# Senpai-sama06/real-time-audio-visual-zooming

Hardware: AMD Instinct MI355X
Metric: beamformed TF-bins/sec (2-ch, 1024-pt STFT) + SIR dB delta vs reference (higher is better)
Workload: dtype f32; 1 GPU; configs[1]: B=256 utterances/GPU, 2 interferers, oracle IBM, 1024-pt STFT hop 512 @16 kHz, 4.0 s utterances; batch_per_gpu=256, global_batch=256, samples=64000, n_fft=1024, hop=512, parallelism=utterance-sharded x1, RCCL metric all-reduce only, input_batches=2, tf_bins_per_utt=64638, mask=ibm, postfilter=ibm, normalize=peak

## Files before the change

include/avz.h:

```cpp
#ifndef AVZ_H_
#define AVZ_H_

#ifdef __cplusplus
extern "C" {
#endif

#define AVZ_OK 0
#define AVZ_ERR_ARG (-1)
#define AVZ_ERR_SHAPE (-2)
#define AVZ_ERR_HIP (-3)
#define AVZ_ERR_UNSUPPORTED (-4)
#define AVZ_ERR_ALIGN (-5)

#define AVZ_MASK_IBM 0
#define AVZ_MASK_IPD 1
#define AVZ_MASK_EXTERNAL 2
#define AVZ_MASK_ONES 3

#define AVZ_PF_NONE 0
#define AVZ_PF_IBM_TARGET 1
#define AVZ_PF_EXT_FLOOR 2
#define AVZ_PF_EXT_MUL 3
#define AVZ_PF_IRM 4

#define AVZ_FALLBACK_MIC0 0
#define AVZ_FALLBACK_MEAN 1
#define AVZ_FALLBACK_BATCH 2

#define AVZ_BF_MVDR 0
#define AVZ_BF_HYBRID_NULL 1

#define AVZ_NORM_NONE 0
#define AVZ_NORM_PEAK 1

typedef struct avz_config {
  int fs;
  int n_fft;
  int hop;
  double sigma;
  double angle_deg;
  double mic_d;
  double c_sound;
  double fmin_hz;
  int mask_mode;
  int postfilter;
  double pf_floor;
  double weight_eps;
  int normalize;
  double norm_eps;
  int max_batch;
  int max_samples;
  int beamformer;
  double bypass_hz;
  double cond_max;
  int singular_fallback;
  double ibm_kappa;
} avz_config;
#define AVZ_IBM_KAPPA 16.0

typedef struct avz_plan avz_plan;

typedef struct avz_batch_args {
  int batch;
  const int* len;
  int max_len;
  const float* mix;
  long long mix_stride;
  long long ch_stride;
  const float* ref_tgt;
  const float* ref_int;
  long long ref_stride;
  const float* ext_mask;
  long long mask_stride_b, mask_stride_f, mask_stride_t;
  float* out;
  long long out_stride;
  float* peak;
  double* cov_out;
  float* w_out;
  int mask_bins;
  int mask_frames;
  void* workspace;
  long long workspace_bytes;
} avz_batch_args;

int avz_plan_create(avz_plan** plan, const avz_config* cfg);
int avz_plan_destroy(avz_plan* plan);
int avz_plan_get_config(const avz_plan* plan, avz_config* cfg);
int avz_num_frames(const avz_plan* plan, int len);
int avz_mvdr_batch(const avz_plan* plan, const avz_batch_args* args, void* hip_stream);
long long avz_mvdr_workspace_bytes(const avz_plan* plan, int batch, int max_len);

int avz_mvdr_covariance(const avz_plan* plan, const avz_batch_args* args, void* hip_stream);
int avz_solve_covariance(const avz_plan* plan, int batch, const double* cov, float* w,
                         const double* steer, int* fallback, void* hip_stream);
int avz_apply_istft(const avz_plan* plan, const avz_batch_args* args, const float* w,
                    void* hip_stream);

typedef struct avz_spectral_args {
  int batch;
  int frames;
  const float* Y;
  long long y_stride_b, y_stride_m, y_stride_f;
  const float* mask;
  long long mask_stride_b, mask_stride_f;
  const double* steer;
  float* S;
  long long s_stride_b, s_stride_f;
  double* cov_out;
  float* w_out;
  int* fallback;
} avz_spectral_args;
int avz_beamform_spectral(const avz_plan* plan, const avz_spectral_args* args, void* hip_stream);

typedef struct avz_wpe_args {
  int batch, bins, frames;
  const int* frames_b;
  int taps, delay, iterations;
  const float* Y;
  long long y_stride_b, y_stride_m, y_stride_f;
  float* Z;
  long long z_stride_b, z_stride_m, z_stride_f;
  int* status;
} avz_wpe_args;
int avz_wpe_spectral(const avz_wpe_args* args, void* hip_stream);

int avz_istft(const avz_plan* plan, int batch, int frames, const float* S, long long s_stride_b,
              long long s_stride_f, float* out, long long out_stride, float* peak,
              void* workspace, long long workspace_bytes, void* hip_stream);

int avz_plan_set_timing(avz_plan* plan, int enable);
int avz_plan_set_timing_period(avz_plan* plan, int period);
int avz_plan_get_timing(avz_plan* plan, double* ms_avg , int* calls);
int avz_plan_set_ibm_stats(avz_plan* plan, unsigned long long* counts);
int avz_plan_set_diagnostics(avz_plan* plan, int synth_variant, int ipf_mode);
int avz_ibm_window(int n, float* out);

int avz_stft(const avz_plan* plan, int batch, int channels, const int* len, int max_len,
             const float* x, long long x_stride, long long ch_stride, float* Y,
             long long y_stride_b, long long y_stride_c, long long y_stride_f,
             void* hip_stream);

int avz_chunk_split(int n_items, int channels, int chunk, const int* item_utt,
                    const int* item_start, const int* len, const float* x, long long x_stride,
                    long long x_ch_stride, float* items, long long item_stride,
                    long long item_ch_stride, void* hip_stream);

int avz_chunk_merge(int batch, int max_len, int hop, int item_out_len, const int* len,
                    const int* item_base, const float* item_out, long long item_out_stride,
                    float* y, long long y_stride, float* peak, int normalize, double norm_eps,
                    void* hip_stream);

#define AVZ_FEAT_LOGMAG_IPD 1
#define AVZ_FEAT_TFLITE 2
int avz_mask_features(const avz_plan* plan, int layout, int batch, const int* len, int max_len,
                      const float* x, long long x_stride, long long ch_stride, float* feat,
                      long long s_b, long long s_c, long long s_f, long long s_t,
                      void* hip_stream);

int avz_mask_training_batch(const avz_plan* plan, int layout, int batch, const int* len,
                            int max_len, const float* mix, long long mix_stride,
                            long long ch_stride, const float* tgt, const float* itf,
                            long long ref_stride, float* feat, long long s_b, long long s_c,
                            long long s_f, long long s_t, float* label, long long l_b,
                            long long l_f, long long l_t, void* hip_stream);

int avz_srp_scan(const avz_plan* plan, int batch, const int* len, int max_len,
                 const float* mix, long long mix_stride, long long ch_stride, int n_angles,
                 double angle_lo, double angle_hi, double f_lo, double f_hi, double* power_db,
                 void* hip_stream);

int avz_projection_metrics(int batch, int max_len, const int* len, const float* est,
                           long long est_stride, const float* tgt, long long tgt_stride,
                           const float* itf, long long itf_stride, double* sums,
                           double* metrics, void* hip_stream);
int avz_projection_metrics_scaled(int batch, int max_len, const int* len, const float* est,
                                  long long est_stride, const float* est_peak, double est_eps,
                                  const float* tgt, long long tgt_stride, const float* itf,
                                  long long itf_stride, double* sums, double* metrics,
                                  void* hip_stream);

typedef struct avz_stoi_args {
  int batch, max_len;
  const int* len;
  double fs;
  const float* clean; long long clean_stride;
  const float* est;   long long est_stride;
  double* stoi;
  int* info;
  float* resampled;
  long long res_stride;
  double* tob;
  long long tob_stride;
  void* workspace; long long workspace_bytes;
} avz_stoi_args;
long long avz_stoi_workspace_bytes(int batch, int max_len, double fs);
int avz_stoi_batch(const avz_stoi_args* args, void* hip_stream);

long long avz_scene_workspace_bytes(int batch, int n_src, int n);
int avz_scene_mix(int batch, int n_src, int n, const float* src, const double* angles_deg,
                  const float* noise, double mic_d, double c_sound, double fs, double sir_db,
                  double snr_db, float* mix, long long mix_stride, long long ch_stride,
                  float* tgt, float* itf, long long ref_stride, void* workspace,
                  long long workspace_bytes, void* hip_stream);

long long avz_scene_generate_workspace_bytes(int batch, int n_interferers, int n);
int avz_scene_generate(int batch, long long start_idx, int n_interferers, int n, unsigned seed,
                       double mic_d, double c_sound, double fs, double sir_db, double snr_db,
                       float* mix, long long mix_stride, long long ch_stride, float* tgt,
                       float* itf, long long ref_stride, void* workspace,
                       long long workspace_bytes, void* hip_stream);

typedef struct avz_room {
  double dim[3];
  double absorption;
  int max_order;
  double mic[2][3];
  double c_sound, fs;
} avz_room;

int avz_room_rir_len(const avz_room* room);

int avz_room_rir(const avz_room* room, int batch, int n_src, const double* src_pos,
                 double* rir, void* hip_stream);

long long avz_scene_reverb_workspace_bytes(const avz_room* room, int batch, int n_src, int n);
int avz_scene_reverb_mix(const avz_room* room, int batch, int n_src, int n, const float* src,
                         const double* src_pos, const float* noise, double sir_db,
                         double snr_db, float* mix, long long mix_stride, long long ch_stride,
                         float* tgt, float* itf, long long ref_stride, void* workspace,
                         long long workspace_bytes, void* hip_stream);

long long avz_scene_reverb_generate_workspace_bytes(const avz_room* room, int batch,
                                                    int n_interferers, int n);
int avz_scene_reverb_generate(const avz_room* room, int batch, long long start_idx,
                              int n_interferers, int n, unsigned seed, const double* target_pos,
                              const double* interferer_pos, double sir_db, double snr_db,
                              float* mix, long long mix_stride, long long ch_stride, float* tgt,
                              float* itf, long long ref_stride, void* workspace,
                              long long workspace_bytes, void* hip_stream);

long long avz_stream_state_bytes(const avz_plan* plan, int streams);
int avz_stream_reset(const avz_plan* plan, void* state, long long state_bytes, int streams,
                     const int* select , void* hip_stream);
int avz_stream_steer(const avz_plan* plan, void* state, long long state_bytes, int streams,
                     const double* angle_deg ,
                     void* hip_stream);
typedef struct avz_stream_args {
  int streams, hops;
  double forget;
  const int* active;
  const int* adapt;
  const float* mix;  long long mix_stride, ch_stride;
  const float* ref_tgt; const float* ref_int; long long ref_stride;
  const float* ext_mask; long long mask_stride_b, mask_stride_f, mask_stride_t;
  float* out; long long out_stride;
  float* w_out;  double* cov_out;
  float* mask_out;
  void* state; long long state_bytes;
} avz_stream_args;
int avz_stream_push(const avz_plan* plan, const avz_stream_args* args, void* hip_stream);

long long avz_wpe_stream_state_bytes(const avz_plan* plan, int streams, int taps, int delay);
int avz_wpe_stream_reset(const avz_plan* plan, void* state, long long state_bytes, int streams,
                         int taps, int delay, double q_init,
                         const int* select ,
                         void* hip_stream);
typedef struct avz_wpe_stream_args {
  int streams, hops, taps, delay;
  double forget, power_floor;
  const int* active;
  const int* adapt;
  const float* mix; long long mix_stride, ch_stride;
  float* out;       long long out_stride, out_ch_stride;
  float* Y_out; float* Z_out;
  double* G_out;
  void* state; long long state_bytes;
} avz_wpe_stream_args;
int avz_wpe_stream_push(const avz_plan* plan, const avz_wpe_stream_args* args, void* hip_stream);

typedef struct avz_delay_mask_args {
  int batch; const int* len; int max_len;
  const float* mix; long long mix_stride, ch_stride;
  const double* angle_deg;
  int hist_bins, smooth, max_peaks;
  double rel_height, min_sep, f_lo_hz;
  float* mask; long long mask_stride_b, mask_stride_f, mask_stride_t;
// ... 39 lines not shown
```

real-time-audio-visual-zooming_amd/avz/_lib.py:

```python
from __future__ import annotations

import ctypes as ct
import os

import torch

_HERE = os.path.dirname(os.path.abspath(__file__))
LIB_PATH = os.environ.get("AVZ_LIB", os.path.join(_HERE, "libavz.so"))

AVZ_OK = 0
AVZ_ERR_ARG = -1
AVZ_ERR_SHAPE = -2
AVZ_ERR_HIP = -3
AVZ_ERR_UNSUPPORTED = -4
AVZ_ERR_ALIGN = -5

MASK_IBM, MASK_IPD, MASK_EXTERNAL, MASK_ONES = 0, 1, 2, 3
PF_NONE, PF_IBM_TARGET, PF_EXT_FLOOR, PF_EXT_MUL, PF_IRM = 0, 1, 2, 3, 4
FALLBACK_MIC0, FALLBACK_MEAN, FALLBACK_BATCH = 0, 1, 2
NORM_NONE, NORM_PEAK = 0, 1
BF_MVDR, BF_HYBRID_NULL = 0, 1
FEAT_LOGMAG_IPD, FEAT_TFLITE = 1, 2

EXPORTED = [
    "avz_plan_create", "avz_plan_destroy", "avz_plan_get_config", "avz_num_frames",
    "avz_mvdr_batch", "avz_plan_set_timing", "avz_plan_get_timing", "avz_stft",
    "avz_plan_set_timing_period",
    "avz_chunk_split", "avz_chunk_merge", "avz_mask_features", "avz_srp_scan",
    "avz_projection_metrics", "avz_scene_workspace_bytes", "avz_scene_mix", "avz_strerror",
    "avz_last_hip_error", "avz_version", "avz_mvdr_workspace_bytes",
    "avz_mvdr_covariance", "avz_solve_covariance", "avz_apply_istft", "avz_beamform_spectral",
    "avz_istft", "avz_scene_generate_workspace_bytes", "avz_scene_generate",
    "avz_projection_metrics_scaled", "avz_plan_set_ibm_stats", "avz_plan_set_diagnostics",
    "avz_ibm_window", "avz_wpe_spectral",
    "avz_room_rir_len", "avz_room_rir", "avz_scene_reverb_workspace_bytes",
    "avz_scene_reverb_mix", "avz_scene_reverb_generate_workspace_bytes",
    "avz_scene_reverb_generate",
    "avz_stoi_workspace_bytes", "avz_stoi_batch",
    "avz_mask_training_batch",
    "avz_stream_state_bytes", "avz_stream_reset", "avz_stream_steer", "avz_stream_push",
    "avz_wpe_stream_state_bytes", "avz_wpe_stream_reset", "avz_wpe_stream_push",
    "avz_delay_mask_workspace_bytes", "avz_delay_mask", "avz_delay_mask_check",
    "avz_delay_stream_state_bytes", "avz_delay_stream_reset", "avz_delay_stream_push",
    "avz_delay_stream_check",
]


class AvzConfig(ct.Structure):
    _fields_ = [
        ("fs", ct.c_int), ("n_fft", ct.c_int), ("hop", ct.c_int),
        ("sigma", ct.c_double), ("angle_deg", ct.c_double), ("mic_d", ct.c_double),
        ("c_sound", ct.c_double), ("fmin_hz", ct.c_double),
        ("mask_mode", ct.c_int), ("postfilter", ct.c_int),
        ("pf_floor", ct.c_double), ("weight_eps", ct.c_double),
        ("normalize", ct.c_int), ("norm_eps", ct.c_double),
        ("max_batch", ct.c_int), ("max_samples", ct.c_int),
        ("beamformer", ct.c_int), ("bypass_hz", ct.c_double), ("cond_max", ct.c_double),
        ("singular_fallback", ct.c_int), ("ibm_kappa", ct.c_double),
    ]


class AvzBatchArgs(ct.Structure):
    _fields_ = [
        ("batch", ct.c_int), ("len", ct.c_void_p), ("max_len", ct.c_int),
        ("mix", ct.c_void_p), ("mix_stride", ct.c_longlong), ("ch_stride", ct.c_longlong),
        ("ref_tgt", ct.c_void_p), ("ref_int", ct.c_void_p), ("ref_stride", ct.c_longlong),
        ("ext_mask", ct.c_void_p), ("mask_stride_b", ct.c_longlong),
        ("mask_stride_f", ct.c_longlong), ("mask_stride_t", ct.c_longlong),
        ("out", ct.c_void_p), ("out_stride", ct.c_longlong), ("peak", ct.c_void_p),
        ("cov_out", ct.c_void_p), ("w_out", ct.c_void_p),
        ("mask_bins", ct.c_int), ("mask_frames", ct.c_int),
        ("workspace", ct.c_void_p), ("workspace_bytes", ct.c_longlong),
    ]


class AvzSpectralArgs(ct.Structure):
    _fields_ = [
        ("batch", ct.c_int), ("frames", ct.c_int),
        ("Y", ct.c_void_p), ("y_stride_b", ct.c_longlong), ("y_stride_m", ct.c_longlong),
        ("y_stride_f", ct.c_longlong),
        ("mask", ct.c_void_p), ("mask_stride_b", ct.c_longlong), ("mask_stride_f", ct.c_longlong),
        ("steer", ct.c_void_p),
        ("S", ct.c_void_p), ("s_stride_b", ct.c_longlong), ("s_stride_f", ct.c_longlong),
        ("cov_out", ct.c_void_p), ("w_out", ct.c_void_p), ("fallback", ct.c_void_p),
    ]


class AvzWpeArgs(ct.Structure):
    _fields_ = [
        ("batch", ct.c_int), ("bins", ct.c_int), ("frames", ct.c_int),
        ("frames_b", ct.c_void_p),
        ("taps", ct.c_int), ("delay", ct.c_int), ("iterations", ct.c_int),
        ("Y", ct.c_void_p), ("y_stride_b", ct.c_longlong), ("y_stride_m", ct.c_longlong),
        ("y_stride_f", ct.c_longlong),
        ("Z", ct.c_void_p), ("z_stride_b", ct.c_longlong), ("z_stride_m", ct.c_longlong),
        ("z_stride_f", ct.c_longlong),
        ("status", ct.c_void_p),
    ]


class AvzStoiArgs(ct.Structure):
    _fields_ = [
        ("batch", ct.c_int), ("max_len", ct.c_int), ("len", ct.c_void_p), ("fs", ct.c_double),
        ("clean", ct.c_void_p), ("clean_stride", ct.c_longlong),
        ("est", ct.c_void_p), ("est_stride", ct.c_longlong),
        ("stoi", ct.c_void_p), ("info", ct.c_void_p),
        ("resampled", ct.c_void_p), ("res_stride", ct.c_longlong),
        ("tob", ct.c_void_p), ("tob_stride", ct.c_longlong),
        ("workspace", ct.c_void_p), ("workspace_bytes", ct.c_longlong),
    ]


class AvzStreamArgs(ct.Structure):
    _fields_ = [
        ("streams", ct.c_int), ("hops", ct.c_int), ("forget", ct.c_double),
        ("active", ct.c_void_p), ("adapt", ct.c_void_p),
        ("mix", ct.c_void_p), ("mix_stride", ct.c_longlong), ("ch_stride", ct.c_longlong),
        ("ref_tgt", ct.c_void_p), ("ref_int", ct.c_void_p), ("ref_stride", ct.c_longlong),
        ("ext_mask", ct.c_void_p), ("mask_stride_b", ct.c_longlong),
        ("mask_stride_f", ct.c_longlong), ("mask_stride_t", ct.c_longlong),
        ("out", ct.c_void_p), ("out_stride", ct.c_longlong),
        ("w_out", ct.c_void_p), ("cov_out", ct.c_void_p), ("mask_out", ct.c_void_p),
        ("state", ct.c_void_p), ("state_bytes", ct.c_longlong),
    ]


class AvzWpeStreamArgs(ct.Structure):
    _fields_ = [
        ("streams", ct.c_int), ("hops", ct.c_int), ("taps", ct.c_int), ("delay", ct.c_int),
        ("forget", ct.c_double), ("power_floor", ct.c_double),
        ("active", ct.c_void_p), ("adapt", ct.c_void_p),
        ("mix", ct.c_void_p), ("mix_stride", ct.c_longlong), ("ch_stride", ct.c_longlong),
        ("out", ct.c_void_p), ("out_stride", ct.c_longlong), ("out_ch_stride", ct.c_longlong),
        ("Y_out", ct.c_void_p), ("Z_out", ct.c_void_p), ("G_out", ct.c_void_p),
        ("state", ct.c_void_p), ("state_bytes", ct.c_longlong),
    ]


class AvzDelayMaskArgs(ct.Structure):
    _fields_ = [
        ("batch", ct.c_int), ("len", ct.c_void_p), ("max_len", ct.c_int),
        ("mix", ct.c_void_p), ("mix_stride", ct.c_longlong), ("ch_stride", ct.c_longlong),
        ("angle_deg", ct.c_void_p),
        ("hist_bins", ct.c_int), ("smooth", ct.c_int), ("max_peaks", ct.c_int),
        ("rel_height", ct.c_double), ("min_sep", ct.c_double), ("f_lo_hz", ct.c_double),
        ("mask", ct.c_void_p), ("mask_stride_b", ct.c_longlong),
        ("mask_stride_f", ct.c_longlong), ("mask_stride_t", ct.c_longlong),
        ("hist_out", ct.c_void_p), ("delays_out", ct.c_void_p), ("n_peaks", ct.c_void_p),
        ("workspace", ct.c_void_p), ("workspace_bytes", ct.c_longlong),
    ]


class AvzDelayStreamArgs(ct.Structure):
    _fields_ = [
        ("streams", ct.c_int), ("hops", ct.c_int), ("forget", ct.c_double),
        ("active", ct.c_void_p), ("adapt", ct.c_void_p),
        ("mix", ct.c_void_p), ("mix_stride", ct.c_longlong), ("ch_stride", ct.c_longlong),
        ("angle_deg", ct.c_void_p),
        ("hist_bins", ct.c_int), ("smooth", ct.c_int), ("max_peaks", ct.c_int),
        ("rel_height", ct.c_double), ("min_sep", ct.c_double), ("f_lo_hz", ct.c_double),
        ("mask", ct.c_void_p), ("mask_stride_b", ct.c_longlong),
        ("mask_stride_f", ct.c_longlong), ("mask_stride_t", ct.c_longlong),
        ("hist_out", ct.c_void_p), ("delays_out", ct.c_void_p), ("n_peaks", ct.c_void_p),
        ("state", ct.c_void_p), ("state_bytes", ct.c_longlong),
    ]


class AvzRoom(ct.Structure):
    _fields_ = [
        ("dim", ct.c_double * 3), ("absorption", ct.c_double), ("max_order", ct.c_int),
        ("mic", (ct.c_double * 3) * 2), ("c_sound", ct.c_double), ("fs", ct.c_double),
    ]


class AvzError(RuntimeError):
    pass


ABI_VERSION = 3


def hip_runtimes_mapped() -> list:
    paths = set()
    try:
        with open("/proc/self/maps") as fh:
            for line in fh:
                if "libamdhip64" in line:
                    paths.add(os.path.realpath(line.split()[-1]))
    except OSError:
        pass
    return sorted(paths)


def _load():
    if not os.path.exists(LIB_PATH):
        raise ImportError(f"libavz.so not found at {LIB_PATH}; run __graft_entry__.build() "
                          "(hipcc --offload-arch=gfx950). There is no CPU fallback.")
    lib = ct.CDLL(LIB_PATH)
    rts = hip_runtimes_mapped()
    if len(rts) > 1:
        raise ImportError(f"two HIP runtimes mapped into the process: {rts}")
    P = ct.c_void_p
    lib.avz_plan_create.argtypes = [ct.POINTER(P), ct.POINTER(AvzConfig)]
    lib.avz_plan_destroy.argtypes = [P]
    lib.avz_plan_get_config.argtypes = [P, ct.POINTER(AvzConfig)]
    lib.avz_num_frames.argtypes = [P, ct.c_int]
    lib.avz_mvdr_batch.argtypes = [P, ct.POINTER(AvzBatchArgs), P]
    lib.avz_mvdr_workspace_bytes.argtypes = [P, ct.c_int, ct.c_int]
    lib.avz_mvdr_workspace_bytes.restype = ct.c_longlong
    lib.avz_mvdr_covariance.argtypes = [P, ct.POINTER(AvzBatchArgs), P]
    lib.avz_solve_covariance.argtypes = [P, ct.c_int, P, P, P, P, P]
    lib.avz_apply_istft.argtypes = [P, ct.POINTER(AvzBatchArgs), P, P]
    lib.avz_beamform_spectral.argtypes = [P, ct.POINTER(AvzSpectralArgs), P]
    lib.avz_istft.argtypes = [P, ct.c_int, ct.c_int, P, ct.c_longlong, ct.c_longlong, P,
                              ct.c_longlong, P, P, ct.c_longlong, P]
    lib.avz_wpe_spectral.argtypes = [ct.POINTER(AvzWpeArgs), P]
    for name in ("avz_mvdr_covariance", "avz_solve_covariance", "avz_apply_istft",
                 "avz_beamform_spectral", "avz_istft", "avz_wpe_spectral"):
        getattr(lib, name).restype = ct.c_int
    lib.avz_stft.argtypes = [P, ct.c_int, ct.c_int, P, ct.c_int, P, ct.c_longlong, ct.c_longlong,
                             P, ct.c_longlong, ct.c_longlong, ct.c_longlong, P]
    I, LL = ct.c_int, ct.c_longlong
    lib.avz_plan_set_timing.argtypes = [P, I]
    lib.avz_plan_set_timing_period.argtypes = [P, I]
    lib.avz_plan_get_timing.argtypes = [P, ct.POINTER(ct.c_double), ct.POINTER(I)]
    lib.avz_plan_set_ibm_stats.argtypes = [P, P]
    lib.avz_plan_set_diagnostics.argtypes = [P, I, I]
    lib.avz_ibm_window.argtypes = [I, ct.POINTER(ct.c_float)]
    lib.avz_chunk_split.argtypes = [I, I, I, P, P, P, P, LL, LL, P, LL, LL, P]
    lib.avz_chunk_merge.argtypes = [I, I, I, I, P, P, P, LL, P, LL, P, I, ct.c_double, P]
    lib.avz_mask_features.argtypes = [P, I, I, P, I, P, LL, LL, P, LL, LL, LL, LL, P]
    D = ct.c_double
    lib.avz_srp_scan.argtypes = [P, I, P, I, P, LL, LL, I, D, D, D, D, P, P]
    lib.avz_projection_metrics.argtypes = [I, I, P, P, LL, P, LL, P, LL, P, P, P]
    lib.avz_projection_metrics_scaled.argtypes = [I, I, P, P, LL, P, D, P, LL, P, LL, P, P, P]
    lib.avz_scene_workspace_bytes.argtypes = [I, I, I]
    lib.avz_scene_workspace_bytes.restype = LL
    lib.avz_scene_mix.argtypes = [I, I, I, P, P, P, D, D, D, D, D, P, LL, LL, P, P, LL, P, LL, P]
    lib.avz_scene_generate_workspace_bytes.argtypes = [I, I, I]
    lib.avz_scene_generate_workspace_bytes.restype = LL
    lib.avz_scene_generate.argtypes = [I, LL, I, I, ct.c_uint, D, D, D, D, D, P, LL, LL, P, P, LL,
                                       P, LL, P]
    R = ct.POINTER(AvzRoom)
    DP = ct.POINTER(ct.c_double)
    lib.avz_room_rir_len.argtypes = [R]
    lib.avz_room_rir.argtypes = [R, I, I, P, P, P]
    lib.avz_scene_reverb_workspace_bytes.argtypes = [R, I, I, I]
    lib.avz_scene_reverb_workspace_bytes.restype = LL
    lib.avz_scene_reverb_mix.argtypes = [R, I, I, I, P, P, P, D, D, P, LL, LL, P, P, LL, P, LL, P]
    lib.avz_scene_reverb_generate_workspace_bytes.argtypes = [R, I, I, I]
    lib.avz_scene_reverb_generate_workspace_bytes.restype = LL
    lib.avz_scene_reverb_generate.argtypes = [R, I, LL, I, I, ct.c_uint, DP, DP, D, D, P, LL, LL,
                                              P, P, LL, P, LL, P]
    for name in ("avz_room_rir_len", "avz_room_rir", "avz_scene_reverb_mix",
                 "avz_scene_reverb_generate"):
        getattr(lib, name).restype = ct.c_int
    lib.avz_stoi_workspace_bytes.argtypes = [I, I, D]
    lib.avz_stoi_workspace_bytes.restype = LL
    lib.avz_stoi_batch.argtypes = [ct.POINTER(AvzStoiArgs), P]
    lib.avz_stoi_batch.restype = ct.c_int
    lib.avz_mask_training_batch.argtypes = [P, I, I, P, I, P, LL, LL, P, P, LL, P, LL, LL, LL, LL,
                                            P, LL, LL, LL, P]
    lib.avz_mask_training_batch.restype = ct.c_int
    SA = ct.POINTER(AvzStreamArgs)
    CP = ct.POINTER(AvzConfig)
    lib.avz_stream_state_bytes.argtypes = [P, I]
    lib.avz_stream_state_bytes.restype = LL
    lib.avz_stream_reset.argtypes = [P, P, LL, I, P, P]
    lib.avz_stream_steer.argtypes = [P, P, LL, I, P, P]
    lib.avz_stream_push.argtypes = [P, SA, P]
    lib.avz_stream_check_state_bytes.argtypes = [CP, I]
    lib.avz_stream_check_state_bytes.restype = LL
    lib.avz_stream_check_state.argtypes = [CP, P, LL, I, P, I]
    lib.avz_stream_check_push.argtypes = [CP, SA]
    for name in ("avz_stream_reset", "avz_stream_steer", "avz_stream_push",
                 "avz_stream_check_state", "avz_stream_check_push"):
        getattr(lib, name).restype = ct.c_int
    WA = ct.POINTER(AvzWpeStreamArgs)
    lib.avz_wpe_stream_state_bytes.argtypes = [P, I, I, I]
    lib.avz_wpe_stream_state_bytes.restype = LL
    lib.avz_wpe_stream_reset.argtypes = [P, P, LL, I, I, I, D, P, P]
    lib.avz_wpe_stream_push.argtypes = [P, WA, P]
    lib.avz_wpe_stream_check_state_bytes.argtypes = [CP, I, I, I]
    lib.avz_wpe_stream_check_state_bytes.restype = LL
    lib.avz_wpe_stream_check_reset.argtypes = [CP, P, LL, I, I, I, D]
    lib.avz_wpe_stream_check_push.argtypes = [CP, WA]
    for name in ("avz_wpe_stream_reset", "avz_wpe_stream_push", "avz_wpe_stream_check_reset",
                 "avz_wpe_stream_check_push"):
        getattr(lib, name).restype = ct.c_int
    DA = ct.POINTER(AvzDelayMaskArgs)
    lib.avz_delay_mask_workspace_bytes.argtypes = [P, I, I, I]
    lib.avz_delay_mask_workspace_bytes.restype = LL
    lib.avz_delay_mask.argtypes = [P, DA, P]
    lib.avz_delay_mask_check.argtypes = [CP, DA]
    lib.avz_delay_mask.restype = lib.avz_delay_mask_check.restype = ct.c_int
    DS = ct.POINTER(AvzDelayStreamArgs)
    lib.avz_delay_stream_state_bytes.argtypes = [P, I, I]
    lib.avz_delay_stream_state_bytes.restype = LL
    lib.avz_delay_stream_reset.argtypes = [P, P, LL, I, I, P, P]
    lib.avz_delay_stream_push.argtypes = [P, DS, P]
    lib.avz_delay_stream_check.argtypes = [CP, DS]
    for name in ("avz_delay_stream_reset", "avz_delay_stream_push", "avz_delay_stream_check"):
        getattr(lib, name).restype = ct.c_int
    lib.avz_stoi_taps.argtypes = [DP]
    lib.avz_stoi_taps.restype = ct.c_int
    lib.avz_strerror.argtypes = [ct.c_int]
    lib.avz_strerror.restype = ct.c_char_p
    lib.avz_last_hip_error.restype = ct.c_char_p
    for name in ("avz_plan_create", "avz_plan_destroy", "avz_plan_get_config", "avz_num_frames",
                 "avz_mvdr_batch", "avz_stft", "avz_chunk_split", "avz_chunk_merge",
                 "avz_plan_set_timing", "avz_plan_get_timing", "avz_mask_features",
                 "avz_plan_set_timing_period",
                 "avz_srp_scan", "avz_projection_metrics", "avz_scene_mix",
                 "avz_scene_generate", "avz_projection_metrics_scaled", "avz_version",
                 "avz_plan_set_ibm_stats", "avz_plan_set_diagnostics", "avz_ibm_window"):
        getattr(lib, name).restype = ct.c_int
    if lib.avz_version() != ABI_VERSION:
        raise ImportError(f"libavz ABI version {lib.avz_version()} != {ABI_VERSION} "
                          "(AvzBatchArgs / AvzSpectralArgs layouts); rebuild")
    return lib


lib = _load()


def check(rc: int, what: str) -> int:
    if rc < 0:
        msg = lib.avz_strerror(rc).decode()
        if rc == AVZ_ERR_HIP:
            msg += ": " + lib.avz_last_hip_error().decode()
        raise AvzError(f"{what} failed ({rc}): {msg}")
    return rc
```

real-time-audio-visual-zooming_amd/avz/engine.py:

```python
from __future__ import annotations

import ctypes as ct
from dataclasses import dataclass, field

import torch

from . import _lib
from ._lib import AvzBatchArgs, AvzConfig, AvzStreamArgs, check, lib

MASKS = {"ibm": _lib.MASK_IBM, "ipd": _lib.MASK_IPD, "external": _lib.MASK_EXTERNAL,
         "ones": _lib.MASK_ONES}
POSTFILTERS = {"none": _lib.PF_NONE, "ibm": _lib.PF_IBM_TARGET, "floor": _lib.PF_EXT_FLOOR,
               "mul": _lib.PF_EXT_MUL, "irm": _lib.PF_IRM}
FALLBACKS = {"mic0": _lib.FALLBACK_MIC0, "mean": _lib.FALLBACK_MEAN,
             "batch": _lib.FALLBACK_BATCH}
NORMS = {"none": _lib.NORM_NONE, "peak": _lib.NORM_PEAK}
BEAMFORMERS = {"mvdr": _lib.BF_MVDR, "hybrid_null": _lib.BF_HYBRID_NULL}


def n_frames(length: int, hop: int) -> int:
    return -(-length // hop) + 1


def out_length(length: int, hop: int) -> int:
    return (n_frames(length, hop) - 1) * hop


@dataclass
class PlanConfig:
    n_fft: int = 1024
    fs: int = 16000
    sigma: float = 1.0
    angle_deg: float = 90.0
    mic_d: float = 0.01
    c_sound: float = 343.0
    fmin_hz: float = 100.0
    mask: str = "ibm"
    postfilter: str = "ibm"
    pf_floor: float = 0.05
    weight_eps: float = 0.0
    normalize: str = "peak"
    norm_eps: float = 0.0
    max_batch: int = 1
    max_samples: int = 64000
    beamformer: str = "mvdr"
    bypass_hz: float = 200.0
    cond_max: float = 10.0
    singular_fallback: str = "mic0"
    ibm_kappa: float = 0.0
    extra: dict = field(default_factory=dict)


def _ptr(t):
    return None if t is None else ct.c_void_p(t.data_ptr())


def _stream_handle(stream):
    s = stream if stream is not None else torch.cuda.current_stream()
    return ct.c_void_p(s.cuda_stream)


class MVDRPlan:

    def __init__(self, cfg: PlanConfig | None = None, **kw):
        cfg = cfg or PlanConfig()
        for k, v in kw.items():
            if not hasattr(cfg, k):
                raise TypeError(f"unknown plan option {k!r}")
            setattr(cfg, k, v)
        self.cfg = cfg
        c = AvzConfig()
        c.fs, c.n_fft, c.hop = cfg.fs, cfg.n_fft, cfg.n_fft // 2
        c.sigma, c.angle_deg, c.mic_d = cfg.sigma, cfg.angle_deg, cfg.mic_d
        c.c_sound, c.fmin_hz = cfg.c_sound, cfg.fmin_hz
        c.mask_mode = MASKS[cfg.mask]
        c.postfilter = POSTFILTERS[cfg.postfilter]
        c.pf_floor, c.weight_eps = cfg.pf_floor, cfg.weight_eps
        c.normalize, c.norm_eps = NORMS[cfg.normalize], cfg.norm_eps
        c.max_batch, c.max_samples = cfg.max_batch, cfg.max_samples
        c.beamformer = BEAMFORMERS[cfg.beamformer]
        c.bypass_hz, c.cond_max = cfg.bypass_hz, cfg.cond_max
        c.singular_fallback = FALLBACKS[cfg.singular_fallback]
        c.ibm_kappa = cfg.ibm_kappa
        h = ct.c_void_p()
        check(lib.avz_plan_create(ct.byref(h), ct.byref(c)), "avz_plan_create")
        self._h = h
        self.hop = cfg.n_fft // 2
        self.F = cfg.n_fft // 2 + 1

    def __del__(self):
        h = getattr(self, "_h", None)
        if h is not None and h.value:
            lib.avz_plan_destroy(h)
            self._h = None

    KERNELS = ("analysis", "solve", "synthesis", "finalize")

    def set_timing(self, enable: bool = True, analysis_only: bool = False,
                   period: int = 1) -> None:
        mode = (2 if analysis_only else 1) if enable else 0
        check(lib.avz_plan_set_timing_period(self._h, int(period)), "avz_plan_set_timing_period")
        check(lib.avz_plan_set_timing(self._h, mode), "avz_plan_set_timing")

    def set_ibm_stats(self, counts) -> None:
        if counts is not None:
            assert counts.dtype == torch.int64 and counts.is_cuda and counts.numel() >= 2
        check(lib.avz_plan_set_ibm_stats(self._h, _ptr(counts)), "avz_plan_set_ibm_stats")
        self._ibm_stats = counts

    def set_diagnostics(self, synth_variant: int = 2, ipf_mode: int = 0) -> None:
        check(lib.avz_plan_set_diagnostics(self._h, int(synth_variant), int(ipf_mode)),
              "avz_plan_set_diagnostics")

    def timing(self) -> dict:
        ms = (ct.c_double * 4)()
        n = ct.c_int()
        check(lib.avz_plan_get_timing(self._h, ms, ct.byref(n)), "avz_plan_get_timing")
        return {"calls": n.value, **{k: ms[i] for i, k in enumerate(self.KERNELS)}}

    def frames(self, length: int) -> int:
        return check(lib.avz_num_frames(self._h, int(length)), "avz_num_frames")

    def out_len(self, length: int) -> int:
        return out_length(length, self.hop)

    def alloc_out(self, batch: int, max_len: int, device) -> torch.Tensor:
        n = self.out_len(max_len)
        return torch.empty((batch, (n + 3) // 4 * 4), dtype=torch.float32, device=device)

    def workspace_bytes(self, batch: int, max_len: int) -> int:
        return check(lib.avz_mvdr_workspace_bytes(self._h, int(batch), int(max_len)),
                     "avz_mvdr_workspace_bytes")

    def alloc_workspace(self, batch: int, max_len: int, device) -> torch.Tensor:
        n = self.workspace_bytes(batch, max_len)
        return torch.empty((max(n, 1) + 255) // 256 * 256, dtype=torch.uint8, device=device)

    def _batch_args(self, mix, lengths, max_len, ref_tgt, ref_int, ext_mask, out, peak,
                    cov_out, w_out, workspace, need_out=True):
        if not mix.is_cuda:
            raise ValueError("mix must be a device tensor")
        if mix.dtype != torch.float32 or mix.dim() != 3 or mix.shape[1] != 2:
            raise ValueError("mix must be float32 [B, 2, S]")
        if mix.stride(2) != 1:
            raise ValueError("mix must be contiguous along samples")
        B, _, S = mix.shape
        dev = mix.device
        if lengths is None:
            lengths = torch.full((B,), S, dtype=torch.int32, device=dev)
            max_len = S
        if lengths.dtype != torch.int32 or not lengths.is_cuda or lengths.dim() != 1 \
                or lengths.shape[0] < B:
            raise ValueError("lengths must be an int32 device tensor of >= B entries")
        if max_len is None:
            max_len = int(lengths[:B].max().item())
        if max_len > S:
            raise ValueError(f"max_len {max_len} exceeds the {S} samples of mix")
        T = self.frames(max_len)
        a = AvzBatchArgs()
        if need_out:
            if out is None:
                out = self.alloc_out(B, max_len, dev)
            if peak is None:
                peak = torch.empty((B,), dtype=torch.float32, device=dev)
            if out.dtype != torch.float32 or out.dim() != 2 or out.shape[0] < B or \
                    out.shape[1] < self.out_len(max_len) or out.stride(1) != 1:
                raise ValueError("out must be float32 [>= B, >= out_len(max_len)]")
            if peak.dtype != torch.float32 or peak.numel() < B or not peak.is_contiguous():
                raise ValueError("peak must be a contiguous float32 tensor of >= B entries")
            a.out = out.data_ptr()
            a.out_stride = out.stride(0)
            a.peak = peak.data_ptr()
        a.batch = B
        a.len = lengths.data_ptr()
        a.max_len = int(max_len)
        a.mix = mix.data_ptr()
        a.mix_stride = mix.stride(0)
        a.ch_stride = mix.stride(1)
        for r in (ref_tgt, ref_int):
            if r is not None and (r.dtype != torch.float32 or r.stride(-1) != 1 or not r.is_cuda
                                  or r.dim() != 2 or r.shape[0] < B or r.shape[1] < max_len):
                raise ValueError("references must be float32 device tensors [B, >= max_len]")
        if ref_tgt is not None:
            a.ref_tgt = ref_tgt.data_ptr()
            a.ref_stride = ref_tgt.stride(0)
        if ref_int is not None:
            a.ref_int = ref_int.data_ptr()
            if ref_tgt is not None and ref_int.stride(0) != ref_tgt.stride(0):
                raise ValueError("ref_tgt and ref_int must share a stride")
        if ext_mask is not None:
            if ext_mask.dtype != torch.float32 or not ext_mask.is_cuda or ext_mask.dim() != 3:
                raise ValueError("ext_mask must be float32 [B, F, T] on the device")
            if ext_mask.shape[0] < B or ext_mask.shape[1] < self.F or ext_mask.shape[2] < T:
                raise ValueError(f"ext_mask {tuple(ext_mask.shape)} does not cover "
                                 f"[B={B}, F={self.F}, T={T}]")
            a.ext_mask = ext_mask.data_ptr()
            a.mask_stride_b, a.mask_stride_f, a.mask_stride_t = ext_mask.stride()
            a.mask_bins, a.mask_frames = ext_mask.shape[1], ext_mask.shape[2]
        for name, t, last in (("cov_out", cov_out, 5), ("w_out", w_out, 4)):
            if t is not None and (not t.is_cuda or not t.is_contiguous() or t.numel() < B * self.F * last
                                  or t.dtype != (torch.float64 if last == 5 else torch.float32)):
                raise ValueError(f"{name} must be a contiguous device tensor of "
                                 f"[B, F, {last}] {'float64' if last == 5 else 'float32'}")
        a.cov_out = 0 if cov_out is None else cov_out.data_ptr()
        a.w_out = 0 if w_out is None else w_out.data_ptr()
        if workspace is not None:
            if workspace.dtype != torch.uint8 or not workspace.is_cuda:
                raise ValueError("workspace must be a uint8 device tensor")
            a.workspace = workspace.data_ptr()
            a.workspace_bytes = workspace.numel()
        return a, out, peak

    def run(self, mix: torch.Tensor, lengths: torch.Tensor | None = None, *,
            max_len: int | None = None, ref_tgt=None, ref_int=None, ext_mask=None,
            out: torch.Tensor | None = None, peak: torch.Tensor | None = None,
            cov_out=None, w_out=None, workspace: torch.Tensor | None = None, stream=None):
        a, out, peak = self._batch_args(mix, lengths, max_len, ref_tgt, ref_int, ext_mask, out,
                                        peak, cov_out, w_out, workspace)
        check(lib.avz_mvdr_batch(self._h, ct.byref(a), _stream_handle(stream)), "avz_mvdr_batch")
        return out, peak

    def covariance(self, mix, lengths=None, *, max_len=None, ref_tgt=None, ref_int=None,
                   ext_mask=None, cov_out=None, workspace=None, stream=None) -> torch.Tensor:
        B = mix.shape[0]
        if cov_out is None:
            cov_out = torch.empty((B, self.F, 5), dtype=torch.float64, device=mix.device)
        a, _, _ = self._batch_args(mix, lengths, max_len, ref_tgt, ref_int, ext_mask, None, None,
                                   cov_out, None, workspace, need_out=False)
        check(lib.avz_mvdr_covariance(self._h, ct.byref(a), _stream_handle(stream)),
              "avz_mvdr_covariance")
        return cov_out

    def solve_covariance(self, cov: torch.Tensor, *, steer=None, w=None, fallback=None,
                         stream=None) -> torch.Tensor:
        if cov.dtype != torch.float64 or cov.dim() != 3 or cov.shape[1:] != (self.F, 5) \
                or not cov.is_contiguous() or not cov.is_cuda:
            raise ValueError("cov must be a contiguous float64 [B, F, 5] device tensor")
        B = cov.shape[0]
        if w is None:
            w = torch.empty((B, self.F, 4), dtype=torch.float32, device=cov.device)
        st = self._steer_ptr(steer)
        fb = self._fallback_ptr(fallback, B)
        check(lib.avz_solve_covariance(self._h, B, ct.c_void_p(cov.data_ptr()),
                                       ct.c_void_p(w.data_ptr()), st, fb, _stream_handle(stream)),
              "avz_solve_covariance")
        return w

    def apply_istft(self, mix, w: torch.Tensor, lengths=None, *, max_len=None, gain=None,
                    out=None, peak=None, workspace=None, stream=None):
        if w.dtype != torch.float32 or not w.is_contiguous() or not w.is_cuda \
                or w.numel() < mix.shape[0] * self.F * 4:
            raise ValueError("w must be a contiguous float32 [B, F, 4] device tensor")
        a, out, peak = self._batch_args(mix, lengths, max_len, None, None, gain, out, peak, None,
                                        None, workspace)
        check(lib.avz_apply_istft(self._h, ct.byref(a), ct.c_void_p(w.data_ptr()),
                                  _stream_handle(stream)), "avz_apply_istft")
        return out, peak

    def _steer_ptr(self, steer):
        if steer is None:
            return None
# ... 447 lines not shown
```

real-time-audio-visual-zooming_amd/csrc/avz_capi.cpp:

```cpp
#include <hip/hip_runtime.h>

#include <algorithm>
#include <cmath>
#include <complex>
#include <limits>
#include <mutex>
#include <cstdlib>
#include <cstring>
#include <new>
#include <string>
#include <unordered_map>
#include <vector>

#include "../../include/avz.h"
#include "avz_internal.h"
#include "avz_delay_mask.hpp"
#include "avz_delay_stream.hpp"

struct Workspace {
  float* part;
  uint32_t* mwords;
  float* coef;
  float* heads;
  float* tails;
  uint32_t* peak_u;
  int* flag;
  float* pf_gain;
  float* tpart;
  int tail_slots;
  float* pheads;
  float* ptails;
  int seam_slots;
  avz::PieceState* pstate;
  uint32_t* xpend;
  uint32_t* xdfr;
  uint32_t* xunc;
  uint32_t* xst;
  size_t xst_bytes;
  long long xst_units;
  float* xres;
};

static int tail_slots(long long B, int nchunk) { return (int)std::min<long long>(B * nchunk * 8, 768); }
static int seam_slots(long long B, int nchunk) {
  return (int)(std::min<long long>(B, 256) * std::min(32, 2 * nchunk));
}

static size_t align256(size_t n) { return (n + 255) & ~size_t(255); }

static size_t ws_layout(const avz_config& c, long long batch, int nchunk, char* base, Workspace* w) {
  const int F = c.n_fft / 2 + 1, H = c.n_fft / 2, CF = avz_chunk_frames();
  const long long B = batch;
  const size_t sz_part = align256(sizeof(float) * B * nchunk * 5 * F);
  const size_t sz_mw = align256(sizeof(uint32_t) * B * nchunk * F);
  const size_t sz_coef = align256(sizeof(float) * B * F * 4);
  const size_t sz_ht = align256(sizeof(float) * B * nchunk * H);
  const size_t sz_b = align256(sizeof(uint32_t) * B);
  const size_t sz_gain =
      c.postfilter == AVZ_PF_IRM ? align256(sizeof(float) * B * nchunk * CF * F) : 0;
  const int ts = tail_slots(B, nchunk), ss = seam_slots(B, nchunk);
  const size_t sz_tpart = align256(sizeof(float) * (size_t)ts * 5 * F);
  const size_t sz_seam = align256(sizeof(float) * (size_t)ss * H);
  const long long units = c.mask_mode == AVZ_MASK_IBM ? B * nchunk + ts : 0;
  const size_t sz_xp = align256(sizeof(uint32_t) * 4 * units);
  const size_t sz_xd = align256(sizeof(uint32_t) * (size_t)F * units);
  const size_t sz_xu = align256(sizeof(uint32_t) * 32 * 32 * (size_t)units);
  const size_t sz_xs = align256(sizeof(uint32_t) * (2 * (size_t)units + (size_t)(units + 31) / 32));
  const size_t sz_xr = align256(sizeof(float) * avz::kXPieces * 5 * (size_t)F * units);

  if (base && w) {
    char* q = base;
    w->part = reinterpret_cast<float*>(q); q += sz_part;
    w->mwords = reinterpret_cast<uint32_t*>(q); q += sz_mw;
    w->coef = reinterpret_cast<float*>(q); q += sz_coef;
    w->heads = reinterpret_cast<float*>(q); q += sz_ht;
    w->tails = reinterpret_cast<float*>(q); q += sz_ht;
    w->peak_u = reinterpret_cast<uint32_t*>(q); q += sz_b;
    w->flag = reinterpret_cast<int*>(q); q += sz_b;
    w->pf_gain = sz_gain ? reinterpret_cast<float*>(q) : nullptr;
    q += sz_gain;
    w->tpart = reinterpret_cast<float*>(q); q += sz_tpart;
    w->tail_slots = ts;
    w->pheads = reinterpret_cast<float*>(q); q += sz_seam;
    w->ptails = reinterpret_cast<float*>(q); q += sz_seam;
    w->seam_slots = ss;
    w->pstate = reinterpret_cast<avz::PieceState*>(q); q += 4 * sz_b;
    w->xpend = units ? reinterpret_cast<uint32_t*>(q) : nullptr; q += sz_xp;
    w->xdfr = units ? reinterpret_cast<uint32_t*>(q) : nullptr; q += sz_xd;
    w->xunc = units ? reinterpret_cast<uint32_t*>(q) : nullptr; q += sz_xu;
    w->xst = units ? reinterpret_cast<uint32_t*>(q) : nullptr; q += sz_xs;
    w->xst_bytes = sz_xs;
    w->xst_units = units;
    w->xres = units ? reinterpret_cast<float*>(q) : nullptr; q += sz_xr;
  }
  return sz_part + sz_mw + sz_coef + 2 * sz_ht + 6 * sz_b + sz_gain + sz_tpart + 2 * sz_seam +
         sz_xp + sz_xd + sz_xu + sz_xs + sz_xr;
}

struct avz_plan {
  avz_config cfg;
  double tau1, tau2;
  int max_frames;
  int nchunk;
  void* arena;
  double* steer;
  double* xtw;
  float* xwin;
  float ibm_cert;
  uint32_t ibm_en_lo, ibm_en_span;
  unsigned long long* xstat;
  int synth_variant;
  int dbg_ipf;
  Workspace ws;
  bool timing;
  int n_k;
  hipEvent_t ev[2][8];
  bool ev_pending[2];
  int ev_kern[2];
  int ev_next;
  int period;
  long long seen;
  double ms_sum[4];
  int ms_calls;
};

static void timing_drain(avz_plan* p, int set) {
  if (!p->ev_pending[set]) return;
  p->ev_pending[set] = false;
  int last = 0;
  for (int i = 0; i < p->n_k; ++i)
    if ((p->ev_kern[set] >> i) & 1) last = i;
  if (hipEventSynchronize(p->ev[set][2 * last + 1]) != hipSuccess) return;
  for (int i = 0; i < p->n_k; ++i) {
    if (!((p->ev_kern[set] >> i) & 1)) continue;
    float ms = 0.f;
    if (hipEventElapsedTime(&ms, p->ev[set][2 * i], p->ev[set][2 * i + 1]) == hipSuccess)
      p->ms_sum[i] += ms;
  }
  p->ms_calls += 1;
}

static void timing_free(avz_plan* p) {
  if (!p->timing) return;
  for (int s = 0; s < 2; ++s)
    for (int i = 0; i < 8; ++i) (void)hipEventDestroy(p->ev[s][i]);
  p->timing = false;
}

static thread_local std::string g_last_hip;

static int hip_fail(hipError_t e) {
  g_last_hip = hipGetErrorString(e);
  return AVZ_ERR_HIP;
}

extern "C" int avz_version(void) { return 3; }

extern "C" const char* avz_last_hip_error(void) { return g_last_hip.c_str(); }

extern "C" const char* avz_strerror(int code) {
  switch (code) {
    case AVZ_OK: return "ok";
    case AVZ_ERR_ARG: return "invalid argument";
    case AVZ_ERR_SHAPE: return "length, stride or batch outside the plan";
    case AVZ_ERR_HIP: return "HIP runtime error";
    case AVZ_ERR_UNSUPPORTED: return "unsupported configuration";
    case AVZ_ERR_ALIGN: return "pointer or stride not aligned to its element / vector size";
    default: return "unknown error";
  }
}

static bool misaligned(const void* ptr, uintptr_t bytes) {
  return (reinterpret_cast<uintptr_t>(ptr) & (bytes - 1)) != 0;
}

static int frames_for(int len, int hop) { return (len + hop - 1) / hop + 1; }

#pragma clang fp contract(off)
static void ref_window_f32(int n, float* out) {
  const double start = -M_PI, step = (M_PI - start) / n;
  for (int i = 0; i < n; ++i) {
    double y = (double)i * step;
    y = y + start;
    const double c = std::cos(y);
    const double w = 0.5 + 0.5 * c;
    out[i] = (float)w;
  }
}
#pragma clang fp contract(on)

extern "C" int avz_ibm_window(int n, float* out) {
  if ((n != 512 && n != 1024) || !out) return AVZ_ERR_ARG;
  ref_window_f32(n, out);
  return AVZ_OK;
}

extern "C" int avz_plan_create(avz_plan** out, const avz_config* cfg) {
  if (!out || !cfg) return AVZ_ERR_ARG;
  *out = nullptr;
  const avz_config& c = *cfg;
  if (c.n_fft != 512 && c.n_fft != 1024) return AVZ_ERR_UNSUPPORTED;
  if (c.hop != c.n_fft / 2) return AVZ_ERR_UNSUPPORTED;
  if (c.fs <= 0 || c.c_sound <= 0 || !(c.sigma >= 0) || c.max_batch <= 0 ||
      c.max_samples < c.n_fft)
    return AVZ_ERR_ARG;
  if (c.mask_mode < AVZ_MASK_IBM || c.mask_mode > AVZ_MASK_ONES) return AVZ_ERR_ARG;
  if (c.postfilter < AVZ_PF_NONE || c.postfilter > AVZ_PF_IRM) return AVZ_ERR_ARG;
  if ((c.postfilter == AVZ_PF_IBM_TARGET || c.postfilter == AVZ_PF_IRM) &&
      c.mask_mode != AVZ_MASK_IBM)
    return AVZ_ERR_ARG;
  if (c.singular_fallback != AVZ_FALLBACK_MIC0 && c.singular_fallback != AVZ_FALLBACK_MEAN &&
      c.singular_fallback != AVZ_FALLBACK_BATCH)
    return AVZ_ERR_ARG;
  if ((c.postfilter == AVZ_PF_EXT_FLOOR || c.postfilter == AVZ_PF_EXT_MUL) &&
      c.mask_mode != AVZ_MASK_EXTERNAL)
    return AVZ_ERR_ARG;
  if (c.normalize != AVZ_NORM_NONE && c.normalize != AVZ_NORM_PEAK) return AVZ_ERR_ARG;
  if (c.beamformer != AVZ_BF_MVDR && c.beamformer != AVZ_BF_HYBRID_NULL) return AVZ_ERR_ARG;
  if (c.beamformer == AVZ_BF_HYBRID_NULL && !(c.cond_max >= 1.0)) return AVZ_ERR_ARG;

  avz_plan* p = new (std::nothrow) avz_plan();
  if (!p) return AVZ_ERR_ARG;
  p->cfg = c;
  const double theta = c.angle_deg * (M_PI / 180.0);
  p->tau1 = (c.mic_d / 2) * std::cos(0.0) * std::cos(theta - 0) / c.c_sound;
  p->tau2 = (c.mic_d / 2) * std::cos(0.0) * std::cos(theta - M_PI) / c.c_sound;
  p->max_frames = frames_for(c.max_samples, c.hop);
  const int F = c.n_fft / 2 + 1;
  {
    p->nchunk = (p->max_frames + avz_chunk_frames() - 1) / avz_chunk_frames();
    const int N = c.n_fft;
    const size_t sz_steer = align256(sizeof(double) * F * 4);
    const size_t sz_xtw = align256(sizeof(double) * N * 2), sz_xwin = align256(sizeof(float) * N);
    const size_t sz_tab = sz_steer + sz_xtw + sz_xwin;
    const size_t sz_ws = ws_layout(c, c.max_batch, p->nchunk, nullptr, nullptr);
    hipError_t e = hipMalloc(&p->arena, sz_tab + sz_ws);
    if (e != hipSuccess) {
      delete p;
      return hip_fail(e);
    }
    char* q = static_cast<char*>(p->arena);
    p->steer = reinterpret_cast<double*>(q);
    p->xtw = reinterpret_cast<double*>(q + sz_steer);
    p->xwin = reinterpret_cast<float*>(q + sz_steer + sz_xtw);
    ws_layout(c, c.max_batch, p->nchunk, q + sz_tab, &p->ws);
    if (p->ws.xst) {
      e = hipMemset(p->ws.xst, 0, p->ws.xst_bytes);
      if (e != hipSuccess) {
        (void)hipFree(p->arena);
        delete p;
        return hip_fail(e);
      }
    }
    const double kappa = c.ibm_kappa == 0.0 ? AVZ_IBM_KAPPA : c.ibm_kappa;
    p->ibm_cert = kappa > 0.0 ? (float)(kappa * 0x1p-24) : 0.0f;
    const bool refbits = c.n_fft == 1024 && c.postfilter != AVZ_PF_IRM;
    avz::ibm_level_range(refbits ? (double)p->ibm_cert * 2.0 / c.n_fft : (double)p->ibm_cert,
                         &p->ibm_en_lo, &p->ibm_en_span);
    p->xstat = nullptr;
    p->synth_variant = 2;
    p->dbg_ipf = 0;
    std::vector<double> xt((size_t)N * 2);
    for (int j = 0; j < N; ++j) {
      const long double a = -2.0L * 3.141592653589793238462643383279502884L * j / N;
      xt[2 * j] = (double)cosl(a);
      xt[2 * j + 1] = (double)sinl(a);
    }
    std::vector<float> xw((size_t)N);
    ref_window_f32(N, xw.data());
    std::vector<double> st((size_t)F * 4);
    const double df = 1.0 / (c.n_fft * (1.0 / c.fs));
    for (int k = 0; k < F; ++k) {
      const double omega = 2 * M_PI * (k * df);
      const std::complex<double> v0 = std::exp(std::complex<double>(0.0, -omega * p->tau1));
      const std::complex<double> v1 = std::exp(std::complex<double>(0.0, -omega * p->tau2));
      std::complex<double> d0 = v0, d1 = v1;
      if (c.beamformer == AVZ_BF_HYBRID_NULL) {
        const std::complex<double> den = v0 + 1e-10;
        d0 = v0 / den;
        d1 = v1 / den;
      }
      st[4 * k + 0] = d0.real();
      st[4 * k + 1] = d0.imag();
      st[4 * k + 2] = d1.real();
      st[4 * k + 3] = d1.imag();
    }
    e = hipMemcpy(p->steer, st.data(), sizeof(double) * st.size(), hipMemcpyHostToDevice);
    if (e == hipSuccess)
      e = hipMemcpy(p->xtw, xt.data(), sizeof(double) * xt.size(), hipMemcpyHostToDevice);
    if (e == hipSuccess)
      e = hipMemcpy(p->xwin, xw.data(), sizeof(float) * xw.size(), hipMemcpyHostToDevice);
    if (e != hipSuccess) {
      (void)hipFree(p->arena);
      delete p;
      return hip_fail(e);
    }
  }
  *out = p;
  return AVZ_OK;
}

extern "C" int avz_plan_destroy(avz_plan* p) {
  if (!p) return AVZ_ERR_ARG;
  timing_free(p);
  if (p->arena) (void)hipFree(p->arena);
  delete p;
  return AVZ_OK;
}

extern "C" int avz_plan_get_config(const avz_plan* p, avz_config* cfg) {
  if (!p || !cfg) return AVZ_ERR_ARG;
  *cfg = p->cfg;
  return AVZ_OK;
}

extern "C" int avz_num_frames(const avz_plan* p, int len) {
  if (!p || len < p->cfg.n_fft) return AVZ_ERR_SHAPE;
  return frames_for(len, p->cfg.hop);
}

static int chunks_for(int max_len, int hop) {
  return (frames_for(max_len, hop) + avz_chunk_frames() - 1) / avz_chunk_frames();
}

extern "C" long long avz_mvdr_workspace_bytes(const avz_plan* p, int batch, int max_len) {
  if (!p || batch < 0 || batch > p->cfg.max_batch) return AVZ_ERR_SHAPE;
  if (max_len < p->cfg.n_fft || max_len > p->cfg.max_samples) return AVZ_ERR_SHAPE;
  return (long long)ws_layout(p->cfg, batch, chunks_for(max_len, p->cfg.hop), nullptr, nullptr);
}

static void plan_params(const avz_plan* p, avz::ChainArgs& k) {
  const avz_config& c = p->cfg;
  k.fs = c.fs;
  k.sigma = c.sigma;
  k.tau1 = p->tau1;
  k.tau2 = p->tau2;
  k.mic_d = c.mic_d;
  k.c_sound = c.c_sound;
  k.fmin_hz = c.fmin_hz;
  k.weight_eps = (float)c.weight_eps;
  k.pf_floor = (float)c.pf_floor;
  k.norm_eps = (float)c.norm_eps;
  k.postfilter = c.postfilter;
  k.normalize = c.normalize;
  k.singular_fallback = c.singular_fallback;
  k.beamformer = c.beamformer;
  k.bypass_hz = c.bypass_hz;
  k.cond_max = c.cond_max;
  k.steer = p->steer;
  k.ibm_cert = p->ibm_cert;
  k.ibm_en_lo = p->ibm_en_lo;
  k.ibm_en_span = p->ibm_en_span;
  k.xwin = p->xwin;
  k.xtw = p->xtw;
  k.xstat = p->xstat;
  k.synth_variant = p->synth_variant;
  k.dbg_ipf = p->dbg_ipf;
}

enum { USE_CHAIN = 0, USE_COVARIANCE = 1, USE_APPLY = 2 };

static int prepare_chain(const avz_plan* p, const avz_batch_args* a, int use, avz::ChainArgs& k) {
  if (!p || !a) return AVZ_ERR_ARG;
  const avz_config& c = p->cfg;
  if (a->batch < 0 || a->batch > c.max_batch) return AVZ_ERR_SHAPE;
  if (!a->len || !a->mix || (use != USE_COVARIANCE && !a->out)) return AVZ_ERR_ARG;
  if (use == USE_COVARIANCE && !a->cov_out) return AVZ_ERR_ARG;
  if (a->max_len < c.n_fft || a->max_len > c.max_samples) return AVZ_ERR_SHAPE;
  if (a->ch_stride < a->max_len) return AVZ_ERR_SHAPE;
  if (a->batch > 1 && a->mix_stride < a->ch_stride + a->max_len) return AVZ_ERR_SHAPE;
  const int T = frames_for(a->max_len, c.hop);
  const int F = c.n_fft / 2 + 1;
  if (use != USE_COVARIANCE) {
    const long long out_len = (long long)(T - 1) * c.hop;
    if (a->batch > 1 && a->out_stride < out_len) return AVZ_ERR_SHAPE;
    if ((a->out_stride & 3) || (reinterpret_cast<uintptr_t>(a->out) & 15)) return AVZ_ERR_ALIGN;
  }
  if (use != USE_APPLY && c.mask_mode == AVZ_MASK_IBM) {
    if (!a->ref_tgt || !a->ref_int) return AVZ_ERR_ARG;
    if (a->batch > 1 && a->ref_stride < a->max_len) return AVZ_ERR_SHAPE;
  }
  const bool needs_mask = use == USE_APPLY ? a->ext_mask != nullptr
                                           : c.mask_mode == AVZ_MASK_EXTERNAL;
  if (use != USE_APPLY && c.mask_mode == AVZ_MASK_EXTERNAL && !a->ext_mask) return AVZ_ERR_ARG;
  if (needs_mask && (a->mask_bins < F || a->mask_frames < T)) return AVZ_ERR_SHAPE;
  Workspace ws = p->ws;
  int nchunk = p->nchunk;
  if (a->workspace) {
    nchunk = chunks_for(a->max_len, c.hop);
    if (reinterpret_cast<uintptr_t>(a->workspace) & 255) return AVZ_ERR_ALIGN;
    if (a->workspace_bytes < (long long)ws_layout(c, a->batch, nchunk, nullptr, nullptr))
      return AVZ_ERR_SHAPE;
    ws_layout(c, a->batch, nchunk, static_cast<char*>(a->workspace), &ws);
  }
  k = avz::ChainArgs{};
  k.xst_reset = (a->workspace && ws.xst) ? (long long)ws.xst_bytes : 0;
  plan_params(p, k);
  k.batch = a->batch;
  k.len = a->len;
  k.max_len = a->max_len;
  k.mix = a->mix;
  k.mix_stride = a->mix_stride;
  k.ch_stride = a->ch_stride;
  k.ref_tgt = a->ref_tgt;
  k.ref_int = a->ref_int;
  k.ref_stride = a->ref_stride;
  k.ext_mask = needs_mask ? a->ext_mask : nullptr;
  k.mask_sb = a->mask_stride_b;
  k.mask_sf = a->mask_stride_f;
  k.mask_st = a->mask_stride_t;
  k.out = a->out;
  k.out_stride = a->out_stride;
  k.peak = a->peak;
  k.cov_out = a->cov_out;
  k.w_out = a->w_out;
  k.max_frames = T;
  k.nchunk = nchunk;
  k.part = ws.part;
  k.mwords = ws.mwords;
  k.coef = ws.coef;
  k.heads = ws.heads;
  k.tails = ws.tails;
  k.peak_u = ws.peak_u;
  k.flag = ws.flag;
  k.pf_gain = ws.pf_gain;
  k.tpart = ws.tpart;
  k.tpart_slots = ws.tail_slots;
  k.pheads = ws.pheads;
  k.ptails = ws.ptails;
  k.pseam_slots = ws.seam_slots;
  k.pstate = ws.pstate;
  k.xpend = ws.xpend;
  k.xdfr = ws.xdfr;
  k.xunc = ws.xunc;
  k.xst = ws.xst;
  k.xres = ws.xres;
  k.xhint = ws.xst ? ws.xst + 2 * (ws.xst_units) : nullptr;
  if (use == USE_COVARIANCE) {
    k.out = nullptr;
    k.peak = nullptr;
    k.w_out = nullptr;
  }
  return AVZ_OK;
}

static int hip_rc(int rc) {
  if (rc == AVZ_ERR_HIP) g_last_hip = hipGetErrorString(hipGetLastError());
  return rc;
}

extern "C" int avz_mvdr_batch(const avz_plan* p, const avz_batch_args* a, void* stream) {
  if (p && a && a->batch == 0) return AVZ_OK;
  avz::ChainArgs k;
  const int e = prepare_chain(p, a, USE_CHAIN, k);
  if (e != AVZ_OK) return e;
  avz_plan* mp = const_cast<avz_plan*>(p);
  void* evs[8];
  int set = -1;
  if (mp->timing && (mp->seen++ % mp->period) == 0) {
    set = mp->ev_next;
    mp->ev_next ^= 1;
    timing_drain(mp, set);
    for (int i = 0; i < 8; ++i) evs[i] = mp->ev[set][i];
    k.events = evs;
    k.n_events = 2 * mp->n_k;
  }
  if (k.xst_reset && hipMemsetAsync(k.xst, 0, (size_t)k.xst_reset, (hipStream_t)stream) != hipSuccess)
    return hip_rc(AVZ_ERR_HIP);
  const int rc = hip_rc(avz_launch_chunked(p->cfg.n_fft, p->cfg.mask_mode, &k, stream));
  if (set >= 0 && rc == AVZ_OK) {
    mp->ev_pending[set] = true;
    mp->ev_kern[set] = avz_chain_kernels(p->cfg.n_fft, &k);
  }
  return rc;
}

extern "C" int avz_mvdr_covariance(const avz_plan* p, const avz_batch_args* a, void* stream) {
  if (p && a && a->batch == 0) return AVZ_OK;
  avz::ChainArgs k;
  const int e = prepare_chain(p, a, USE_COVARIANCE, k);
  if (e != AVZ_OK) return e;
  if (k.xst_reset && hipMemsetAsync(k.xst, 0, (size_t)k.xst_reset, (hipStream_t)stream) != hipSuccess)
    return hip_rc(AVZ_ERR_HIP);
  return hip_rc(avz_launch_covariance(p->cfg.n_fft, p->cfg.mask_mode, &k, stream));
}

extern "C" int avz_apply_istft(const avz_plan* p, const avz_batch_args* a, const float* w,
                               void* stream) {
  if (p && a && a->batch == 0) return AVZ_OK;
  if (!w || (reinterpret_cast<uintptr_t>(w) & 15)) return w ? AVZ_ERR_ALIGN : AVZ_ERR_ARG;
  avz::ChainArgs k;
  const int e = prepare_chain(p, a, USE_APPLY, k);
  if (e != AVZ_OK) return e;
  return hip_rc(avz_launch_apply_istft(p->cfg.n_fft, &k, w, stream));
}

extern "C" int avz_istft(const avz_plan* p, int batch, int frames, const float* S,
                         long long s_stride_b, long long s_stride_f, float* out,
                         long long out_stride, float* peak, void* workspace,
                         long long workspace_bytes, void* stream) {
  if (!p) return AVZ_ERR_ARG;
  const avz_config& c = p->cfg;
  if (batch < 0 || batch > c.max_batch || frames < 0) return AVZ_ERR_SHAPE;
  if (batch == 0) return AVZ_OK;
  if (!S || !out) return AVZ_ERR_ARG;
  if (misaligned(S, 8)) return AVZ_ERR_ALIGN;
  const long long len = (long long)(frames - 1) * c.hop;
  if (len < c.n_fft || len > c.max_samples) return AVZ_ERR_SHAPE;
  const int F = c.n_fft / 2 + 1;
  if (s_stride_f < frames || (batch > 1 && s_stride_b < (long long)F * s_stride_f))
    return AVZ_ERR_SHAPE;
  if (batch > 1 && out_stride < len) return AVZ_ERR_SHAPE;
  if ((out_stride & 3) || (reinterpret_cast<uintptr_t>(out) & 15)) return AVZ_ERR_ALIGN;
  Workspace ws = p->ws;
  int nchunk = p->nchunk;
  if (workspace) {
    nchunk = chunks_for((int)len, c.hop);
    if (reinterpret_cast<uintptr_t>(workspace) & 255) return AVZ_ERR_ALIGN;
    if (workspace_bytes < (long long)ws_layout(c, batch, nchunk, nullptr, nullptr))
      return AVZ_ERR_SHAPE;
    ws_layout(c, batch, nchunk, static_cast<char*>(workspace), &ws);
  }
  avz::ChainArgs k{};
  plan_params(p, k);
  k.postfilter = AVZ_PF_NONE;
  k.batch = batch;
  k.len = nullptr;
  k.max_len = (int)len;
  k.max_frames = frames;
  k.spec = S;
  k.spec_sb = s_stride_b;
  k.spec_sf = s_stride_f;
  k.spec_frames = frames;
  k.out = out;
  k.out_stride = out_stride;
  k.peak = peak;
  k.nchunk = nchunk;
  k.heads = ws.heads;
  k.tails = ws.tails;
  k.peak_u = ws.peak_u;
  return hip_rc(avz_launch_istft(c.n_fft, &k, stream));
}

extern "C" int avz_beamform_spectral(const avz_plan* p, const avz_spectral_args* a, void* stream) {
  if (!p || !a) return AVZ_ERR_ARG;
  const avz_config& c = p->cfg;
  if (a->batch < 0 || a->batch > c.max_batch || a->frames < 1) return AVZ_ERR_SHAPE;
  if (a->batch == 0) return AVZ_OK;
  if (!a->Y || !a->mask || !a->S) return AVZ_ERR_ARG;
  if (misaligned(a->Y, 8) || misaligned(a->S, 8) || misaligned(a->mask, 4))
    return AVZ_ERR_ALIGN;
  if (c.mask_mode != AVZ_MASK_EXTERNAL) return AVZ_ERR_ARG;
  const int F = c.n_fft / 2 + 1;
  if (a->y_stride_f < a->frames || a->y_stride_m < (long long)F * a->y_stride_f ||
      a->mask_stride_f < a->frames || a->s_stride_f < a->frames)
    return AVZ_ERR_SHAPE;
  if (a->batch > 1 && (a->y_stride_b < 2 * a->y_stride_m ||
                       a->mask_stride_b < (long long)F * a->mask_stride_f ||
                       a->s_stride_b < (long long)F * a->s_stride_f))
    return AVZ_ERR_SHAPE;
  avz::ChainArgs k{};
  plan_params(p, k);
  avz::SpecArgs s{};
  s.batch = a->batch;
  s.frames = a->frames;
  s.Y = a->Y;
  s.y_sb = a->y_stride_b;
  s.y_sm = a->y_stride_m;
  s.y_sf = a->y_stride_f;
  s.M = a->mask;
  s.m_sb = a->mask_stride_b;
  s.m_sf = a->mask_stride_f;
  s.steer = a->steer ? a->steer : p->steer;
  s.S = a->S;
  s.s_sb = a->s_stride_b;
  s.s_sf = a->s_stride_f;
  s.cov_out = a->cov_out;
  s.w_out = a->w_out;
  s.flag = a->fallback ? a->fallback : p->ws.flag;
  return hip_rc(avz_launch_spectral(c.n_fft, &s, &k, stream));
}

extern "C" int avz_wpe_spectral(const avz_wpe_args* a, void* stream) {
  if (!a) return AVZ_ERR_ARG;
  if (a->taps < 1 || a->taps > 16 || a->delay < 1 || a->iterations < 1 || a->iterations > 10)
    return AVZ_ERR_ARG;
  if (a->batch < 0 || a->bins < 0 || a->frames < 1 || a->frames > avz_wpe_max_frames())
    return AVZ_ERR_SHAPE;
  if (a->batch == 0 || a->bins == 0) return AVZ_OK;
// ... 16 lines not shown
  w.frames_b = a->frames_b;
  w.taps = a->taps;
  w.delay = a->delay;
  w.iterations = a->iterations;
  w.Y = a->Y;
  w.y_sb = a->y_stride_b;
  w.y_sm = a->y_stride_m;
  w.y_sf = a->y_stride_f;
  w.Z = a->Z;
  w.z_sb = a->z_stride_b;
  w.z_sm = a->z_stride_m;
  w.z_sf = a->z_stride_f;
  w.status = a->status;
  return hip_rc(avz_launch_wpe(&w, stream));
}

struct StoiShape {
  int resample;
  long long n10, nf, jmax;
  size_t sz_res, sz_e, sz_k, sz_i, sz_t;
  size_t bytes() const { return sz_res + sz_e + sz_k + sz_i + sz_t; }
};

static int stoi_shape(int batch, int max_len, double fs, StoiShape* s) {
  if (fs != 16000.0 && fs != 10000.0) return AVZ_ERR_UNSUPPORTED;
  if (batch < 0 || batch > 32767 || max_len < 0 || max_len > 0x3fffffff) return AVZ_ERR_SHAPE;
  s->resample = fs == 16000.0;
  s->n10 = s->resample ? (5LL * max_len + 7) / 8 : max_len;
  s->nf = s->n10 > 256 ? (s->n10 - 256 + 127) / 128 : 0;
  s->jmax = s->nf > 1 ? s->nf - 1 : 0;
  const size_t B = (size_t)batch;
  s->sz_res = s->resample ? align256(sizeof(float) * 2 * B * (size_t)s->n10) : 0;
  s->sz_e = align256(sizeof(double) * B * (size_t)s->nf);
  s->sz_k = align256(sizeof(int) * B * (size_t)s->nf);
  s->sz_i = align256(sizeof(int) * 4 * B);
  s->sz_t = align256(sizeof(double) * 2 * 15 * B * (size_t)s->jmax);
  return AVZ_OK;
}

extern "C" long long avz_stoi_workspace_bytes(int batch, int max_len, double fs) {
  StoiShape s;
  const int e = stoi_shape(batch, max_len, fs, &s);
  return e != AVZ_OK ? e : (long long)s.bytes();
}

extern "C" int avz_stoi_batch(const avz_stoi_args* a, void* stream) {
  if (!a) return AVZ_ERR_ARG;
  StoiShape s;
  const int e = stoi_shape(a->batch, a->max_len, a->fs, &s);
  if (e != AVZ_OK) return e;
  if (a->batch == 0) return AVZ_OK;
  if (!a->clean || !a->est || !a->stoi || !a->workspace) return AVZ_ERR_ARG;
  if (misaligned(a->clean, 4) || misaligned(a->est, 4) || misaligned(a->len, 4) ||
      misaligned(a->stoi, 8) || misaligned(a->info, 4) || misaligned(a->resampled, 4) ||
      misaligned(a->tob, 8) || misaligned(a->workspace, 256))
    return AVZ_ERR_ALIGN;
  if (a->workspace_bytes < (long long)s.bytes()) return AVZ_ERR_SHAPE;
  if (a->batch > 1 && (a->clean_stride < a->max_len || a->est_stride < a->max_len))
    return AVZ_ERR_SHAPE;
  if (a->resampled && a->res_stride < s.n10) return AVZ_ERR_SHAPE;
  if (a->tob && a->tob_stride < s.jmax) return AVZ_ERR_SHAPE;

  char* q = static_cast<char*>(a->workspace);
  float* ws_res = reinterpret_cast<float*>(q); q += s.sz_res;
  double* ws_e = reinterpret_cast<double*>(q); q += s.sz_e;
  int* ws_k = reinterpret_cast<int*>(q); q += s.sz_k;
  int* ws_i = reinterpret_cast<int*>(q); q += s.sz_i;
  double* ws_t = reinterpret_cast<double*>(q);

  avz::StoiArgs k{};
  k.batch = a->batch;
  k.max_len = a->max_len;
  k.len = a->len;
  k.resample = s.resample;
  k.n10_max = (int)s.n10;
  k.nf_max = (int)s.nf;
  k.clean = a->clean;
  k.est = a->est;
  k.clean_stride = a->clean_stride;
  k.est_stride = a->est_stride;
  if (a->resampled) {
    k.res = a->resampled;
    k.res_stride = a->res_stride;
  } else if (s.resample) {
    k.res = ws_res;
    k.res_stride = s.n10;
  }
  if (s.resample) {
    k.x10 = k.res;
    k.y10 = k.res + k.res_stride;
    k.x10_stride = k.y10_stride = 2 * k.res_stride;
  } else {
    k.x10 = a->clean;
    k.y10 = a->est;
    k.x10_stride = a->clean_stride;
    k.y10_stride = a->est_stride;
  }
  k.energy = ws_e;
  k.kept = ws_k;
  k.info = a->info ? a->info : ws_i;
  k.tob = a->tob ? a->tob : ws_t;
  k.tob_stride = a->tob ? a->tob_stride : s.jmax;
  k.stoi = a->stoi;
  return hip_rc(avz_launch_stoi(&k, stream));
}

extern "C" int avz_solve_covariance(const avz_plan* p, int batch, const double* cov, float* w,
                                    const double* steer, int* fallback, void* stream) {
  if (!p) return AVZ_ERR_ARG;
  if (batch < 0 || batch > p->cfg.max_batch) return AVZ_ERR_SHAPE;
  if (batch == 0) return AVZ_OK;
  if (!cov || !w) return AVZ_ERR_ARG;
  if (misaligned(cov, 8) || misaligned(w, 16) || misaligned(steer, 8)) return AVZ_ERR_ALIGN;
  avz::ChainArgs k{};
  plan_params(p, k);
  avz::SpecArgs s{};
  s.batch = batch;
  s.cov_in = cov;
  s.w_out = w;
  s.steer = steer ? steer : p->steer;
  s.flag = fallback ? fallback : p->ws.flag;
  return hip_rc(avz_launch_solve_cov(p->cfg.n_fft, &s, &k, stream));
}

extern "C" int avz_plan_set_timing(avz_plan* p, int enable) {
  if (!p) return AVZ_ERR_ARG;
  timing_free(p);
  p->ev_pending[0] = p->ev_pending[1] = false;
  p->ev_next = 0;
  p->ms_calls = 0;
  p->seen = 0;
  if (p->period < 1) p->period = 1;
  for (double& m : p->ms_sum) m = 0.0;
  if (!enable) return AVZ_OK;
  if (enable != 1 && enable != 2) return AVZ_ERR_ARG;
  p->n_k = enable == 2 ? 1 : 4;
  for (int s = 0; s < 2; ++s)
    for (int i = 0; i < 8; ++i) {
      const hipError_t e = hipEventCreateWithFlags(&p->ev[s][i], hipEventDisableSystemFence);
      if (e != hipSuccess) {
        for (int t = 0; t <= s; ++t)
          for (int j = 0; j < (t < s ? 8 : i); ++j) (void)hipEventDestroy(p->ev[t][j]);
        return hip_fail(e);
      }
    }
  p->timing = true;
  return AVZ_OK;
}

extern "C" int avz_plan_set_ibm_stats(avz_plan* p, unsigned long long* counts) {
  if (!p) return AVZ_ERR_ARG;
  if (misaligned(counts, 8)) return AVZ_ERR_ALIGN;
  p->xstat = counts;
  return AVZ_OK;
}

extern "C" int avz_plan_set_diagnostics(avz_plan* p, int synth_variant, int ipf_mode) {
  if (!p || synth_variant < 0 || synth_variant > 2 || ipf_mode < 0 || ipf_mode > 2)
    return AVZ_ERR_ARG;
  p->synth_variant = synth_variant;
  p->dbg_ipf = ipf_mode;
  return AVZ_OK;
}

extern "C" int avz_plan_set_timing_period(avz_plan* p, int period) {
  if (!p || period < 1) return AVZ_ERR_ARG;
  p->period = period;
  p->seen = 0;
  return AVZ_OK;
}

extern "C" int avz_plan_get_timing(avz_plan* p, double* ms_avg, int* calls) {
  if (!p || !ms_avg) return AVZ_ERR_ARG;
  if (!p->timing) return AVZ_ERR_ARG;
  timing_drain(p, p->ev_next);
  timing_drain(p, p->ev_next ^ 1);
  for (int i = 0; i < 4; ++i)
    ms_avg[i] = i >= p->n_k ? std::numeric_limits<double>::quiet_NaN()
                                 : (p->ms_calls ? p->ms_sum[i] / p->ms_calls : 0.0);
  if (calls) *calls = p->ms_calls;
  return AVZ_OK;
}

extern "C" int avz_stft(const avz_plan* p, int batch, int channels, const int* len, int max_len,
                        const float* x, long long x_stride, long long ch_stride, float* Y,
                        long long y_stride_b, long long y_stride_c, long long y_stride_f,
                        void* stream) {
  if (!p || !len || !x || !Y) return AVZ_ERR_ARG;
  if (channels != 1 && channels != 2) return AVZ_ERR_ARG;
  if (batch < 0) return AVZ_ERR_SHAPE;
  if (batch == 0) return AVZ_OK;
  if (max_len < p->cfg.n_fft) return AVZ_ERR_SHAPE;
  const int T = frames_for(max_len, p->cfg.hop);
  if (y_stride_f < T) return AVZ_ERR_SHAPE;
  avz::StftArgs s{};
  s.batch = batch;
  s.channels = channels;
  s.len = len;
  s.x = x;
  s.x_stride = x_stride;
  s.ch_stride = ch_stride;
  s.Y = Y;
  s.y_stride_b = y_stride_b;
  s.y_stride_c = y_stride_c;
  s.y_stride_f = y_stride_f;
  s.max_frames = T;
  s.max_len = max_len;
  const int rc = avz_launch_stft(p->cfg.n_fft, &s, stream);
  if (rc == AVZ_ERR_HIP) g_last_hip = hipGetErrorString(hipGetLastError());
  return rc;
}

extern "C" int avz_chunk_split(int n_items, int channels, int chunk, const int* item_utt,
                               const int* item_start, const int* len, const float* x,
                               long long x_stride, long long x_ch_stride, float* items,
                               long long item_stride, long long item_ch_stride, void* stream) {
  if (n_items < 0 || chunk <= 0 || (channels != 1 && channels != 2)) return AVZ_ERR_SHAPE;
  if (n_items == 0) return AVZ_OK;
  if (!item_utt || !item_start || !len || !x || !items) return AVZ_ERR_ARG;
  if (item_ch_stride < chunk && channels > 1) return AVZ_ERR_SHAPE;
  if (n_items > 1 && item_stride < (long long)channels * chunk) return AVZ_ERR_SHAPE;
  avz::ChunkSplitArgs s{};
  s.n_items = n_items;
  s.channels = channels;
  s.chunk = chunk;
  s.item_utt = item_utt;
  s.item_start = item_start;
  s.len = len;
  s.x = x;
  s.x_stride = x_stride;
  s.x_ch_stride = x_ch_stride;
  s.items = items;
  s.item_stride = item_stride;
  s.item_ch_stride = item_ch_stride;
  const int rc = avz_launch_chunk_split(&s, stream);
  if (rc == AVZ_ERR_HIP) g_last_hip = hipGetErrorString(hipGetLastError());
  return rc;
}

extern "C" int avz_chunk_merge(int batch, int max_len, int hop, int item_out_len, const int* len,
                               const int* item_base, const float* item_out,
                               long long item_out_stride, float* y, long long y_stride,
                               float* peak, int normalize, double norm_eps, void* stream) {
  if (batch < 0 || max_len < 0 || hop <= 0 || item_out_len <= 0) return AVZ_ERR_SHAPE;
  if (batch == 0 || max_len == 0) return AVZ_OK;
  if (!len || !item_base || !item_out || !y || !peak) return AVZ_ERR_ARG;
  if (item_out_stride < item_out_len || (batch > 1 && y_stride < max_len)) return AVZ_ERR_SHAPE;
  avz::ChunkMergeArgs m{};
  m.batch = batch;
  m.max_len = max_len;
  m.hop = hop;
  m.item_out_len = item_out_len;
  m.len = len;
  m.item_base = item_base;
  m.item_out = item_out;
  m.item_out_stride = item_out_stride;
  m.y = y;
  m.y_stride = y_stride;
  m.peak = peak;
  m.normalize = normalize != 0;
  m.norm_eps = (float)norm_eps;
  const int rc = avz_launch_chunk_merge(&m, stream);
  if (rc == AVZ_ERR_HIP) g_last_hip = hipGetErrorString(hipGetLastError());
  return rc;
}

extern "C" int avz_mask_features(const avz_plan* p, int layout, int batch, const int* len,
                                 int max_len, const float* x, long long x_stride,
                                 long long ch_stride, float* feat, long long s_b, long long s_c,
                                 long long s_f, long long s_t, void* stream) {
  if (!p || !len || !x || !feat) return AVZ_ERR_ARG;
  if (layout != AVZ_FEAT_LOGMAG_IPD && layout != AVZ_FEAT_TFLITE) return AVZ_ERR_ARG;
  if (batch < 0) return AVZ_ERR_SHAPE;
  if (batch == 0) return AVZ_OK;
  if (max_len < p->cfg.n_fft || max_len > p->cfg.max_samples) return AVZ_ERR_SHAPE;
  if (ch_stride < max_len) return AVZ_ERR_SHAPE;
  avz::StftArgs s{};
  s.batch = batch;
  s.channels = 2;
  s.len = len;
  s.x = x;
  s.x_stride = x_stride;
  s.ch_stride = ch_stride;
  s.max_frames = frames_for(max_len, p->cfg.hop);
  s.max_len = max_len;
  s.feat = layout;
  s.F_out = feat;
  s.f_sb = s_b;
  s.f_sc = s_c;
  s.f_sf = s_f;
  s.f_st = s_t;
  const int rc = avz_launch_stft(p->cfg.n_fft, &s, stream);
  if (rc == AVZ_ERR_HIP) g_last_hip = hipGetErrorString(hipGetLastError());
  return rc;
}

extern "C" int avz_mask_training_batch(const avz_plan* p, int layout, int batch, const int* len,
                                       int max_len, const float* mix, long long mix_stride,
                                       long long ch_stride, const float* tgt, const float* itf,
                                       long long ref_stride, float* feat, long long s_b,
                                       long long s_c, long long s_f, long long s_t, float* label,
                                       long long l_b, long long l_f, long long l_t, void* stream) {
  if (!p || !len || !mix || !tgt || !itf || !feat || !label) return AVZ_ERR_ARG;
  if (layout != AVZ_FEAT_LOGMAG_IPD && layout != AVZ_FEAT_TFLITE) return AVZ_ERR_ARG;
  const avz_config& c = p->cfg;
  if (batch < 0 || batch > c.max_batch) return AVZ_ERR_SHAPE;
// ... 843 lines not shown
```

real-time-audio-visual-zooming_amd/csrc/avz_chain_analysis.hpp:

```cpp
#pragma once
#include "avz_chain_common.hpp"
#include "avz_chain_exact.hpp"

namespace avz {
template <int N, int MASK, bool IRM, class TW>
__device__ __forceinline__ void analysis_item(const ChainArgs& A, unsigned char* lds, int c,
                                              int b, int p, int P, int slot, const TW& tw_reg,
                                              const LaneConst<N>& K, int seq) {
  using C = KCfg<N>;
  using G = CGeo<N>;
  constexpr int NT = G::NT, H = G::H, F = G::F, NSLOT = G::NSLOT, BPT = G::BPT, PPL = C::PPL;
  constexpr int FB = (MASK == MASK_IBM) ? NSLOT / 2 : NSLOT;
  static_assert(kChunk % FB == 0, "steps tile the chunk");
  constexpr bool REFBITS = N == 1024 && MASK == MASK_IBM && !IRM && !std::is_same<TW, NoTw>::value;
  constexpr bool SHARE = N == 1024 && MASK != MASK_IPD && !std::is_same<TW, NoTw>::value;
  constexpr bool DLT = MASK == MASK_IBM && !REFBITS;

  const int tid = threadIdx.x;
  const int wave = __builtin_amdgcn_readfirstlane(tid >> 6);
  const int lane = tid & 63;
  const int L = utt_len(A, b);
  const int T = (L + H - 1) / H + 1;
  const int nch = (T + kChunk - 1) / kChunk;
  if (L < N || c >= nch) return;
  if (c == 0 && p == 0 && tid == 0) {
    A.peak_u[b] = 0u;
    if (A.peak && A.normalize != NORM_PEAK) A.peak[b] = 0.0f;
  }
  const int t0 = c * kChunk;
  const int nframes = min(kChunk, T - t0);
  constexpr int SA = kChunk / FB;
  const int s_lo = p * SA / P;
  const int nstep = min((nframes + FB - 1) / FB, (p + 1) * SA / P);
  uint32_t* const pendw = reinterpret_cast<uint32_t*>(lds + G::MISC_OFF + 32 + 12 * (seq & 1));
  if (MASK == MASK_IBM && tid == 0) {
    int z = 0;
    opaque_i(z);
    pendw[0] = (uint32_t)z;
    pendw[1] = (uint32_t)z;
    pendw[2] = (uint32_t)z;
  }

  const typename C::Fft fft = K.fft;
  LaneMap<N> lm;
  {
    int ln = threadIdx.x & 63;
    opaque_i(ln);
    lm.init(ln);
  }
  const float cert_raw = A.ibm_cert * (2.0f / N);
  const WinCoef<N> wc = K.wc;
  const int my_slot = wave * C::FPW + lm.grp;
  cf* my_spec = slot_ptr<N>(lds, my_slot);
  const bool ref = (MASK == MASK_IBM) && (wave * C::FPW >= FB);
  const int my_frame = ref ? my_slot - FB : my_slot;
  const int wave_frame0 = ref ? wave * C::FPW - FB : wave * C::FPW;

  const float* mixb = A.mix + (long long)b * A.mix_stride;
  rsrc_t r_re = make_rsrc(mixb, L), r_im = make_rsrc(mixb + A.ch_stride, L);
  if constexpr (MASK == MASK_IBM) {
    if (ref) {
      r_re = make_rsrc(A.ref_tgt + (long long)b * A.ref_stride, L);
      r_im = make_rsrc(A.ref_int + (long long)b * A.ref_stride, L);
    }
  }
  cf v[PPL];
  auto issue_loads = [&](int step) {
    if constexpr (SHARE) {
      const int sp = (t0 + step * FB + wave_frame0) * H - N / 2 + lm.in0;
      if (t0 + step * FB + wave_frame0 >= 1)
        pair_loads<true>(v, r_re, r_im, sp, lm.grp);
      else
        pair_loads<false>(v, r_re, r_im, sp, lm.grp);
      return;
    }
    const int s0 = (t0 + step * FB + my_frame) * H - N / 2 + lm.in0;
    if (t0 + step * FB + wave_frame0 >= 1) {
      static_for<0, PPL>([&](auto r) {
        v[r].x = bload_nn(r_re, s0 + C::IN_STRIDE * r);
        v[r].y = bload_nn(r_im, s0 + C::IN_STRIDE * r);
      });
    } else {
      static_for<0, PPL>([&](auto r) {
        v[r].x = bload(r_re, s0 + C::IN_STRIDE * r);
        v[r].y = bload(r_im, s0 + C::IN_STRIDE * r);
      });
    }
  };

  constexpr bool IL_LOADS = N == 1024 && !std::is_same<TW, NoTw>::value;
  const rsrc_t r_none = make_rsrc(nullptr, 0);
  rsrc_t rn_re = r_none, rn_im = r_none;
  int sp_next = 0;
  auto load_reg = [&](auto kc) {
    constexpr int k = decltype(kc)::value;
    if constexpr (SHARE) {
      if constexpr (k < 16) {
        const int e = sp_next + 1024 * lm.grp + 32 * k;
        v[k].x = bload_nn(rn_re, e);
        v[k].y = bload_nn(rn_im, e);
      } else if constexpr ((k - 16) % 2 == 0) {
        const int e = sp_next + 512 + 32 * (k - 16) + 32 * lm.grp;
        v[k].x = bload_nn(rn_re, e);
        v[k].y = bload_nn(rn_im, e);
      }
    } else {
      v[k].x = bload_nn(rn_re, sp_next + C::IN_STRIDE * k);
      v[k].y = bload_nn(rn_im, sp_next + C::IN_STRIDE * k);
    }
  };

  Acc32 acc[BPT];
  uint32_t bits[BPT];
  uint32_t dfr[BPT];
  int ipd_clear_n[BPT];
#pragma unroll
  for (int j = 0; j < BPT; ++j) {
    acc[j].zero();
    bits[j] = 0u;
    dfr[j] = 0u;
    ipd_clear_n[j] = 0;
  }
  static_assert(!IRM || MASK == MASK_IBM, "IRM needs the references");
  float* const gain = IRM ? A.pf_gain + ((long long)b * A.nchunk + c) * kChunk * F : nullptr;
  const bool nyq_wave = (wave == G::NWAVE - 1);
  Acc32 an, adc;
  an.zero();
  adc.zero();
  uint32_t nyq_bits = 0u, nyq_dfr = 0u;
  float wone[BPT];
#pragma unroll
  for (int j = 0; j < BPT; ++j) wone[j] = (MASK == MASK_IPD && j == 0 && tid == 0) ? 0.0f : 1.0f;

  AVZ_STAMP_DECL();
  issue_loads(s_lo);
  lds_barrier();
  AVZ_STAMP_INIT();
  for (int step = s_lo; step < nstep; ++step) {
    const int f0 = t0 + step * FB;
    const bool live = f0 + wave_frame0 < T;
#ifdef AVZ_STAMPS
    asm volatile("s_waitcnt vmcnt(0)" ::: "memory");
    AVZ_STAMP(0);
#endif
    if (live) {
      if constexpr (SHARE) pair_finish(v);
      float eg0 = 0.0f, eg1 = eg0;
      if constexpr (REFBITS) {
        if (ref) {
          const float eg = group32_sum(frame_energy(v));
          int e0 = __builtin_amdgcn_readlane(__float_as_int(eg), 0);
          int e1 = __builtin_amdgcn_readlane(__float_as_int(eg), 32);
          const bool o0 = (uint32_t)e0 - A.ibm_en_lo > A.ibm_en_span;
          const bool o1 = (uint32_t)e1 - A.ibm_en_lo > A.ibm_en_span;
          if ((o0 || o1) && A.ibm_cert > 0.0f) {
            uint32_t nz = 0u;
            static_for<0, 32>([&](auto r) { nz |= __float_as_uint(v[r].x) | __float_as_uint(v[r].y); });
            const unsigned long long any = __ballot((nz << 1) != 0u);
            const bool f0 = o0 && (uint32_t)any != 0u, f1 = o1 && (any >> 32) != 0ull;
            if (f0 || f1) {
              const bool mine = lm.grp ? f1 : f0;
              static_for<0, 32>([&](auto r) {
                v[r].x = mine ? 0.0f : v[r].x;
                v[r].y = mine ? 0.0f : v[r].y;
              });
              e0 = f0 ? 0x7f800000 : e0;
              e1 = f1 ? 0x7f800000 : e1;
            }
          }
          eg0 = __int_as_float(e0);
          eg1 = __int_as_float(e1);
        }
      }
      if constexpr (MASK == MASK_IPD) {
        bool same = true;
        static_for<0, PPL>([&](auto r) {
          same &= __float_as_uint(v[r].x) == __float_as_uint(v[r].y);
        });
        const unsigned long long nb = __ballot(!same);
        const bool ident = (C::FPW == 1) ? nb == 0ull : ((nb >> (32 * lm.grp)) & 0xffffffffull) == 0ull;
        if ((lane & (64 / C::FPW - 1)) == 0) lds[G::MISC_OFF + my_slot] = ident ? 1 : 0;
      }
      if constexpr (IL_LOADS) {
        const bool more = step + 1 < nstep;
        rn_re = more ? r_re : r_none;
        rn_im = more ? r_im : r_none;
        sp_next = (t0 + (step + 1) * FB + (SHARE ? wave_frame0 : my_frame)) * H - N / 2 + lm.in0;
      }
      float en = 0.0f;
      if constexpr (!IL_LOADS) {
        window_fft<N>(v, wc, fft, my_spec, lm, NoAfter{}, (DLT && ref) ? &en : nullptr);
      } else if constexpr (REFBITS) {
        uint32_t um = 0u;
        if (step + 1 < nstep) {
          if (ref)
            um = window_fft_reg_ibm_bits(v, wc, fft, my_spec, tw_reg, lm, eg0, eg1, cert_raw, en,
                                         load_reg);
          else
            window_fft_reg(v, wc, fft, my_spec, tw_reg, lm, load_reg);
        } else {
          if (ref)
            um = window_fft_reg_ibm_bits(v, wc, fft, my_spec, tw_reg, lm, eg0, eg1, cert_raw, en);
          else
            window_fft_reg(v, wc, fft, my_spec, tw_reg, lm);
        }
        const unsigned long long ua = __ballot(um != 0u);
        if (ua != 0ull) {
          if ((ua >> (32 * lm.grp)) & 0xffffffffull) {
            KArgs& Ak = kernarg_chain_args();
            const int gxi = (Ak.max_frames + kChunk - 1) / kChunk;
            const int unit = slot < 0 ? b * gxi + c : gxi * Ak.batch + slot;
            Ak.xunc[((long long)unit * kChunk + step * FB + my_frame) * 32 + (lane & 31)] = um;
            int nu = __popc(um);
#pragma unroll
            for (int o = 1; o < 32; o <<= 1) nu += __shfl_xor(nu, o, 64);
            if ((lane & 31) == 0) {
              atomicOr(pendw, 1u << (step * FB + my_frame));
              atomicOr(pendw + 1, 1u << (step * FB + my_frame));
              if (nu >= kSparseMax) atomicOr(pendw + 2, 1u << (step * FB + my_frame));
            }
          }
        }
      } else {
        window_fft_reg(v, wc, fft, my_spec, tw_reg, lm, load_reg, (DLT && ref) ? &en : nullptr);
      }
      if constexpr (DLT) {
        static_assert(C::FPW == 2, "lane groups of 32");
        if (ref) {
          const bool o = ibm_level_out(en, A.ibm_en_lo, A.ibm_en_span);
          if (__ballot(o) != 0ull && A.ibm_cert > 0.0f) {
            const int sf = (t0 + step * FB + my_frame) * H - N / 2 + (lane & 31);
            uint32_t nz = 0u;
#pragma unroll 1
            for (int r = 0; r < N / 32; r += 4) {
#pragma unroll
              for (int q = 0; q < 4; ++q)
                nz |= __float_as_uint(bload(r_re, sf + 32 * (r + q))) |
                      __float_as_uint(bload(r_im, sf + 32 * (r + q)));
            }
            const unsigned long long any = __ballot((nz << 1) != 0u);
            if (o && ((any >> (32 * lm.grp)) & 0xffffffffull) != 0ull) en = __builtin_nanf("");
          }
        }
      }
      if (MASK == MASK_IBM && ref && (lane & 31) == 0)
        reinterpret_cast<float*>(lds + G::MISC_OFF + 16)[my_frame] = REFBITS ? en : A.ibm_cert * sqrtf(en);
    }
    AVZ_STAMP(3);
    if (!IL_LOADS && step + 1 < nstep) issue_loads(step + 1);
    AVZ_STAMP(11);
    lds_barrier();
    AVZ_STAMP(1);
    const int nvalid = min(FB, T - f0);
    uint32_t ipd_fix[BPT];
#pragma unroll
    for (int j = 0; j < BPT; ++j) ipd_fix[j] = 0u;
    const unsigned long long ident_w =
        (MASK == MASK_IPD) ? *reinterpret_cast<const unsigned long long*>(lds + G::MISC_OFF) : 0ull;
    const bool mask_vec = MASK == MASK_EXTERNAL && A.mask_st == 1 && (A.mask_sf & 3) == 0 &&
                          (A.mask_sb & 3) == 0 &&
                          ((reinterpret_cast<uintptr_t>(A.ext_mask) & 15) == 0) && (f0 & 3) == 0;
    float dlt[4] = {0.0f, 0.0f, 0.0f, 0.0f};
    if constexpr (DLT) {
      const float4 q = *reinterpret_cast<const float4*>(lds + G::MISC_OFF + 16);
      dlt[0] = q.x;
      dlt[1] = q.y;
      dlt[2] = q.z;
      dlt[3] = q.w;
    }
    auto bin_phase = [&](auto full, auto vec) {
      constexpr int G = FB < 4 ? FB : 4;
#pragma unroll
      for (int j = 0; j < BPT; ++j) {
        const int kb = tid + j * NT;
        const int kp = (N - kb) & (N - 1);
#pragma unroll
        for (int g0 = 0; g0 < FB; g0 += G) {
          float mv[MASK == MASK_EXTERNAL ? 4 : 1];
          if constexpr (MASK == MASK_EXTERNAL && G == 4 && decltype(vec)::value) {
            const float4 m4 = *reinterpret_cast<const float4*>(
                A.ext_mask + (long long)b * A.mask_sb + (long long)kb * A.mask_sf + f0 + g0);
            mv[0] = m4.x;
            mv[1] = m4.y;
            mv[2] = m4.z;
            mv[3] = m4.w;
          }
          cf zm[G], zmp[G], zr[G], zrp[G];
          uint32_t zw[G];
#pragma unroll
          for (int i = 0; i < G; ++i) {
            if (decltype(full)::value || g0 + i < nvalid) {
              const cf* Zm = slot_ptr<N>(lds, g0 + i);
              zm[i] = Zm[kb];
              zmp[i] = Zm[kp];
              if constexpr (REFBITS) {
                zw[i] = reinterpret_cast<const uint32_t*>(slot_ptr<N>(lds, FB + g0 + i))[kb & 31];
              } else if constexpr (MASK == MASK_IBM) {
                const cf* Zr = slot_ptr<N>(lds, FB + g0 + i);
                zr[i] = Zr[kb];
                zrp[i] = Zr[kp];
              }
            }
          }
#pragma unroll
          for (int i = 0; i < G; ++i) {
            if (decltype(full)::value || g0 + i < nvalid) {
              cf x0, x1;
              split_pair2(zm[i], zmp[i], x0, x1);
              if constexpr (MASK == MASK_IPD) {
                const float p0 = x0.x * x0.x + x0.y * x0.y;
                const float p1 = x1.x * x1.x + x1.y * x1.y;
                const float re = x0.x * x1.x + x0.y * x1.y;
                const float im = x0.y * x1.x - x0.x * x1.y;
                const bool clear = im * im > 1e-10f * (p0 * p1) &&
                                   !((ident_w >> (8 * (g0 + i))) & 1ull);
                ipd_fix[j] |= (clear ? 0u : 1u) << (g0 + i);
                acc[j].c00 = fmaf(wone[j], p0, acc[j].c00);
                acc[j].c11 = fmaf(wone[j], p1, acc[j].c11);
                acc[j].c01r = fmaf(wone[j], re, acc[j].c01r);
                acc[j].c01i = fmaf(wone[j], im, acc[j].c01i);
                continue;
              }
              if constexpr (MASK == MASK_IBM) {
                bool noise;
                if constexpr (REFBITS) {
                  noise = (zw[i] >> (kb >> 5)) & 1u;
                } else {
                  noise = ibm_noise(zr[i], zrp[i]);
                  if (ibm_uncertain(zr[i], zrp[i], dlt[g0 + i])) {
                    noise = false;
                    dfr[j] |= 1u << (step * FB + g0 + i);
                    atomicOr(pendw, 1u << (step * FB + g0 + i));
                  }
                }
                bits[j] |= (noise ? 1u : 0u) << (step * FB + g0 + i);
                acc[j].add_sel(x0, x1, noise);
                if constexpr (IRM) gain[(step * FB + g0 + i) * F + kb] = irm_gain(zr[i], zrp[i]);
                continue;
              }
              bool noise = false;
              float wgt;
              float m;
              if constexpr (MASK == MASK_EXTERNAL && G == 4 && decltype(vec)::value) {
                m = 1.0f - mv[i];
                wgt = m + A.weight_eps;
              } else {
                m = bin_mask<MASK>(A, b, x0, x1, zr[i], zrp[i], kb, f0 + g0 + i, noise, wgt);
              }
              bits[j] |= (noise ? 1u : 0u) << (step * FB + g0 + i);
              acc[j].add(x0, x1, wgt, m);
              if constexpr (IRM) gain[(step * FB + g0 + i) * F + kb] = irm_gain(zr[i], zrp[i]);
            }
          }
        }
      }
    };
    if (nvalid == FB) {
      if constexpr (MASK == MASK_EXTERNAL) {
        if (mask_vec)
          bin_phase(std::true_type{}, std::true_type{});
        else
          bin_phase(std::true_type{}, std::false_type{});
      } else {
        bin_phase(std::true_type{}, std::false_type{});
      }
    } else {
      bin_phase(std::false_type{}, std::false_type{});
    }
    if constexpr (MASK == MASK_IPD) {
#pragma unroll
      for (int j = 0; j < BPT; ++j) {
        const int kb = tid + j * NT;
        const int kp = (N - kb) & (N - 1);
        uint32_t f = ipd_fix[j];
        const bool dc = (j == 0 && tid == 0);
        if (dc) f = 0u;
        ipd_clear_n[j] += dc ? 0 : nvalid - __popc(f);
        while (f) {
          const int i = __builtin_ctz(f);
          f &= f - 1u;
          const cf* Zm = slot_ptr<N>(lds, i);
          cf x0, x1;
          split_pair2(Zm[kb], Zm[kp], x0, x1);
          const float w = ((ident_w >> (8 * i)) & 1ull) ? 0.01f : ipd_weight_exact(x0, x1);
          acc[j].add(x0, x1, w - 1.0f, w);
        }
      }
    }
    if (nyq_wave) {
      bool noise = false, nunc = false;
      if (lane < nvalid) {
        int ln = lane;
        opaque_i(ln);
        const cf* Zm = slot_ptr<N>(lds, ln);
        cf y0, y1, zr{0, 0};
        split_pair2(Zm[N / 2], Zm[N / 2], y0, y1);
        if constexpr (MASK == MASK_IBM) zr = slot_ptr<N>(lds, FB + ln)[N / 2];
        float wn;
        float mn = bin_mask<MASK>(A, b, y0, y1, zr, zr, N / 2, f0 + lane, noise, wn);
        if (MASK == MASK_IPD && ((ident_w >> (8 * lane)) & 1ull)) wn = mn = 0.01f;
        if (MASK == MASK_IBM &&
            ibm_uncertain(zr, zr, reinterpret_cast<const float*>(lds + G::MISC_OFF + 16)[lane])) {
          noise = false;
          wn = mn = 0.0f;
          nunc = true;
          atomicOr(pendw, 1u << (step * FB + lane));
        }
        an.add(y0, y1, wn, mn);
        if constexpr (MASK == MASK_IPD) {
          cf d0, d1;
          const cf z0 = Zm[0];
          split_pair2(z0, z0, d0, d1);
          const float wd = ((ident_w >> (8 * lane)) & 1ull) ? 0.01f : ipd_weight_exact(d0, d1);
          adc.add(d0, d1, wd, wd);
        }
        if constexpr (IRM) gain[(step * FB + lane) * F + N / 2] = irm_gain(zr, zr);
      }
      const unsigned long long bal = __ballot(noise);
      nyq_bits |= ((uint32_t)bal & ((1u << FB) - 1u)) << (step * FB);
      if constexpr (MASK == MASK_IBM)
        nyq_dfr |= ((uint32_t)__ballot(nunc) & ((1u << FB) - 1u)) << (step * FB);
    }
    AVZ_STAMP(12);
    lds_barrier();
    AVZ_STAMP(2);
  }

  if constexpr (MASK == MASK_IBM) {
    const uint32_t pend = pendw[0], full = pendw[1];
    const uint32_t big = REFBITS ? pendw[2] : pend;
    KArgs& Ak = kernarg_chain_args();
    const int gxi = (Ak.max_frames + kChunk - 1) / kChunk;
    const int unit = slot < 0 ? b * gxi + c : gxi * Ak.batch + slot;
    if (nyq_wave && lane == 0) {
      reinterpret_cast<uint4*>(Ak.xpend)[unit] = make_uint4(pend, full, nyq_dfr, big);
      if (pend) *reinterpret_cast<uint32_t*>(lds + G::MISC_OFF + 56) |= 1u << min(seq, 31);
    }
    if (DLT && pend != 0u) {
#pragma unroll
      for (int j = 0; j < BPT; ++j) Ak.xdfr[(long long)unit * F + tid + j * NT] = dfr[j];
    }
  }

  float* Pt = slot < 0 ? A.part + ((long long)b * A.nchunk + c) * 5 * F
                       : A.tpart + (long long)slot * 5 * F;
  uint32_t* MW = A.mwords + ((long long)b * A.nchunk + c) * F;
  const uint32_t rng = (P == 1) ? ~0u : ((1u << (kChunk / P)) - 1u) << (kChunk / P * p);
  auto put_word = [&](int k, uint32_t w) {
    if (slot < 0) {
      MW[k] = w;
    } else {
      atomicAnd(MW + k, ~rng);
      atomicOr(MW + k, w);
    }
  };
  constexpr bool DC_NYQ = MASK == MASK_IPD;
#pragma unroll
  for (int j = 0; j < BPT; ++j) {
    const int kb = tid + j * NT;
    if (DC_NYQ && kb == 0) continue;
    if constexpr (MASK == MASK_IBM) acc[j].cm = (float)__popc(bits[j]);
    if constexpr (MASK == MASK_IPD) acc[j].cm += (float)ipd_clear_n[j];
    Pt[0 * F + kb] = acc[j].c00;
    Pt[1 * F + kb] = acc[j].c11;
    Pt[2 * F + kb] = acc[j].c01r;
    Pt[3 * F + kb] = acc[j].c01i;
    Pt[4 * F + kb] = acc[j].cm;
    if constexpr (MASK == MASK_IBM) put_word(kb, bits[j]);
  }
  if (nyq_wave) {
    for (int o = 1; o < 64; o <<= 1) {
      an.c00 += __shfl_xor(an.c00, o, 64);
      an.c11 += __shfl_xor(an.c11, o, 64);
      an.c01r += __shfl_xor(an.c01r, o, 64);
      an.c01i += __shfl_xor(an.c01i, o, 64);
      an.cm += __shfl_xor(an.cm, o, 64);
      if constexpr (DC_NYQ) {
        adc.c00 += __shfl_xor(adc.c00, o, 64);
        adc.c11 += __shfl_xor(adc.c11, o, 64);
        adc.c01r += __shfl_xor(adc.c01r, o, 64);
        adc.c01i += __shfl_xor(adc.c01i, o, 64);
        adc.cm += __shfl_xor(adc.cm, o, 64);
      }
    }
    if (DC_NYQ && lane == 0) {
      Pt[0 * F] = adc.c00;
      Pt[1 * F] = adc.c11;
      Pt[2 * F] = adc.c01r;
      Pt[3 * F] = adc.c01i;
      Pt[4 * F] = adc.cm;
    }
    if (lane == 0) {
      Pt[0 * F + N / 2] = an.c00;
      Pt[1 * F + N / 2] = an.c11;
      Pt[2 * F + N / 2] = an.c01r;
      Pt[3 * F + N / 2] = an.c01i;
      Pt[4 * F + N / 2] = an.cm;
      if constexpr (MASK == MASK_IBM) put_word(N / 2, nyq_bits);
    }
  }

  if constexpr (MASK == MASK_IBM) {
    const uint32_t big = REFBITS ? pendw[2] : pendw[0];
    if (big != 0u) {
      AVZ_XT_BEGIN(tp);
      __syncthreads();
      if (tid == 0) {
        KArgs& Ak = kernarg_chain_args();
        const int gxi = (Ak.max_frames + kChunk - 1) / kChunk;
        const int unit = slot < 0 ? b * gxi + c : gxi * Ak.batch + slot;
        const XPieces q = x_pieces(pendw[0], big);
        Ak.xst[2 * unit + 1] = 0u;
        __builtin_amdgcn_fence(__ATOMIC_RELEASE, "agent");
        __hip_atomic_store(Ak.xst + 2 * unit, kXOpen | ((uint32_t)q.n << 16), __ATOMIC_RELAXED,
                           __HIP_MEMORY_SCOPE_AGENT);
        __hip_atomic_fetch_or(Ak.xhint + (unit >> 5), 1u << (unit & 31), __ATOMIC_RELAXED,
                              __HIP_MEMORY_SCOPE_AGENT);
#ifdef AVZ_XTRACE
        if (g_stamps) {
          g_stamps[blockIdx.x * 16 + 12] += __builtin_amdgcn_s_memrealtime() - tp;
          g_stamps[blockIdx.x * 16 + 13] += 1 + 256 * q.n;
        }
#endif
      }
    }
  }
}

template <int N, int MASK, bool IRM, bool SPLIT, class TW>
__device__ __forceinline__ void analysis_items(const ChainArgs& A, unsigned char* lds, int gx,
                                               int n_items, const TW& tw_reg,
                                               const LaneConst<N>& K) {
  const int P = SPLIT && A.a_pieces > 1 ? A.a_pieces : 1;
  const int n_whole = P > 1 ? A.a_whole : n_items;
  const int n_end = n_whole + (n_items - n_whole) * P;
  int seq = 0;
  for (int u = blockIdx.x; u < n_end; u += gridDim.x) {
    const bool whole = u < n_whole;
    const int q = u - n_whole, it = whole ? u : n_whole + q / P;
    analysis_item<N, MASK, IRM>(A, lds, it % gx, it / gx, whole ? 0 : q % P, whole ? 1 : P,
                                whole ? -1 : q, tw_reg, K, seq++);
  }
}

template <int N, int MASK, bool IRM, bool SPLIT = false>
__global__ void __launch_bounds__(kCThreads, KCfg<N>::BLOCKS_PER_CU) avz_analysis_kernel(ChainArgs A) {
  using G = CGeo<N>;
  extern __shared__ __align__(16) unsigned char lds[];
  AVZ_XT(0, __builtin_amdgcn_s_memrealtime());
  if (MASK == MASK_IBM && threadIdx.x == 0)
    *reinterpret_cast<uint32_t*>(lds + G::MISC_OFF + 56) = 0u;
  if (A.pstate)
    for (int b = blockIdx.x * kCThreads + threadIdx.x; b < A.batch; b += gridDim.x * kCThreads)
      A.pstate[b] = PieceState{};
  KCfg<N>::Fft::fill_twiddles(reinterpret_cast<cf*>(lds + G::TW_OFF), threadIdx.x, G::NT);
  const int gx = (A.max_frames + kChunk - 1) / kChunk;
  const int n_items = gx * A.batch;
  if constexpr (N == 1024) {
    __syncthreads();
    cf tw_reg[31];
    Fft1024x2 f;
    f.init(threadIdx.x & 63);
    f.load_twiddles(tw_reg, reinterpret_cast<const cf*>(lds + G::TW_OFF));
    if (MASK != MASK_IPD && (threadIdx.x & 32)) {
      static_for<0, 16>([&](auto i) { tw_reg[2 * i] = cf{-tw_reg[2 * i].x, -tw_reg[2 * i].y}; });
    }
    LaneConst<N> K;
    K.init(threadIdx.x);
    if (MASK != MASK_IPD && (threadIdx.x & 32)) {
      K.wc.ac = -K.wc.ac;
      K.wc.as = -K.wc.as;
    }
    analysis_items<N, MASK, IRM, SPLIT>(A, lds, gx, n_items, tw_reg, K);
    if constexpr (MASK == MASK_IBM) ibm_exact_units<N, MASK, IRM, SPLIT, Tw1024>(lds, gx, n_items);
  } else {
    LaneConst<N> K;
    K.init(threadIdx.x);
    analysis_items<N, MASK, IRM, SPLIT>(A, lds, gx, n_items, NoTw{}, K);
    if constexpr (MASK == MASK_IBM) ibm_exact_units<N, MASK, IRM, SPLIT, NoTw>(lds, gx, n_items);
  }
}
}
```

real-time-audio-visual-zooming_amd/csrc/avz_chain_common.hpp:

```cpp
#pragma once
#include <hip/hip_runtime.h>
#include <hip/hip_ext.h>
#include <stdint.h>

#include <algorithm>
#include <atomic>
#include <type_traits>

#include "avz_common.hpp"

namespace avz {

constexpr int kChunk = 32;
constexpr int kSC1 = 16;
typedef int v4i_t __attribute__((ext_vector_type(4)));
constexpr int kCThreads = 256;

template <int N>
struct CGeo {
  using C = KCfg<N>;
  static constexpr int NT = kCThreads;
  static constexpr int NWAVE = NT / 64;
  static constexpr int H = N / 2;
  static constexpr int F = N / 2 + 1;
  static constexpr int NSLOT = NWAVE * C::FPW;
  static constexpr int BPT = (N / 2) / NT;
  static constexpr int SLOT_LDS = NWAVE * C::WAVE_BYTES;
  static constexpr int TW_OFF = SLOT_LDS;
  static constexpr int MISC_OFF = TW_OFF + C::TW_BYTES;
  static constexpr int LDS_BYTES = MISC_OFF + 64;
  static_assert(BPT >= 1 && BPT * NT == N / 2, "bin mapping");
  static constexpr int BLOCKS = C::BLOCKS_PER_CU;
  static_assert(BLOCKS * LDS_BYTES <= 160 * 1024, "resident blocks per CU");
};

template <int N, int PF>
constexpr int kSynR = (N == 512 && (PF == PF_EXT_FLOOR || PF == PF_EXT_MUL)) ? 1 : KCfg<N>::SYN_R;

template <int N, int R_ = KCfg<N>::SYN_R>
struct SGeo {
  using C = KCfg<N>;
  static constexpr int NT = kCThreads;
  static constexpr int NWAVE = NT / 64;
  static constexpr int R = R_;
  static constexpr int H = N / 2;
  static constexpr int F = N / 2 + 1;
  static constexpr int NSLOT = NWAVE * C::FPW * R;
  static constexpr int BPT = (N / 2) / NT;
  static constexpr int SLOT_LDS = NWAVE * C::WAVE_BYTES * R;
  static constexpr int TW_OFF = SLOT_LDS;
  static constexpr int MISC_OFF = TW_OFF + C::TW_BYTES;
  static constexpr int LDS_BYTES = MISC_OFF + 64;
  static constexpr int BLOCKS = C::SYN_BLOCKS_PER_CU;
  static_assert(BLOCKS * LDS_BYTES <= 160 * 1024, "resident synthesis blocks per CU");
};

template <int N>
struct WinCoef {
  float a0, ac, as, s0, sc, ss;
  __device__ __forceinline__ void init(const LaneMap<N>& lm) {
    double s, c;
    sincospi(2.0 * lm.in0 / N, &s, &c);
    const double sca = 2.0 / N;
    a0 = (float)(0.5 * sca);
    ac = (float)(0.5 * sca * c);
    as = (float)(0.5 * sca * s);
    sincospi(2.0 * lm.out0 / N, &s, &c);
    s0 = 0.25f;
    sc = (float)(0.25 * c);
    ss = (float)(0.25 * s);
  }
};

template <int N>
__device__ __forceinline__ float inv_wsum(int m) {
  const float c1 = cospif(2.0f * (float)m / (float)N);
  const float wa = 0.5f - 0.5f * c1, wb = 0.5f + 0.5f * c1;
  return 1.0f / (wa * wa + wb * wb);
}

template <int N>
struct LaneConst {
  typename KCfg<N>::Fft fft;
  LaneMap<N> lm;
  WinCoef<N> wc;
  float inv[4];
  __device__ __forceinline__ void init(int tid) {
    const int lane = tid & 63;
    fft.init(lane);
    lm.init(lane);
    wc.init(lm);
    const int m0 = 4 * (tid % (N / 8));
#pragma unroll
    for (int i = 0; i < 4; ++i) inv[i] = inv_wsum<N>(m0 + i);
  }
};

template <int N = 1024, int PPL>
__device__ __forceinline__ void window_apply(cf (&v)[PPL], float a0, float ac, float as) {
  using C = KCfg<N>;
  static_assert(C::IN_STRIDE * (PPL / 2) == N / 2, "upper-half registers are N/2 later");
  const float a2 = a0 + a0;
  static_for<0, PPL / 2>([&](auto r) {
    constexpr int j = (C::IN_STRIDE * 32 / N) * r;
    constexpr float cr = W32::c[j % 32], sr = -W32::s[j % 32];
    const float w = fmaf(as, sr, fmaf(-ac, cr, a0));
    v[r] = c_scale(v[r], w);
    v[r + PPL / 2] = c_scale(v[r + PPL / 2], a2 - w);
  });
}

__device__ __forceinline__ bool ibm_noise(cf zr, cf zrp) {
  return fmaf(zr.x, zrp.x, -(zr.y * zrp.y)) < 0.0f;
}

__device__ __forceinline__ float group32_sum(float e) {
  e += __int_as_float(__builtin_amdgcn_mov_dpp(__float_as_int(e), 0xB1, 0xF, 0xF, false));
  e += __int_as_float(__builtin_amdgcn_mov_dpp(__float_as_int(e), 0x4E, 0xF, 0xF, false));
  e += __int_as_float(__builtin_amdgcn_mov_dpp(__float_as_int(e), 0x141, 0xF, 0xF, false));
  e += __int_as_float(__builtin_amdgcn_mov_dpp(__float_as_int(e), 0x140, 0xF, 0xF, false));
  float lo, hi;
  xhalf<16>(e, lo, hi);
  return lo + hi;
}
__device__ __forceinline__ float frame_energy(const cf (&v)[32]) {
  float e = 0.0f;
  static_for<0, 32>([&](auto r) {
    e = fmaf(v[r].x, v[r].x, e);
    e = fmaf(v[r].y, v[r].y, e);
  });
  return e;
}
struct NoAfter {
  template <class K>
  __device__ __forceinline__ void operator()(K) const {}
};
template <class After = NoAfter>
__device__ __forceinline__ void window_fft_reg(cf (&v)[32], const WinCoef<1024>& wc,
                                               const Fft1024x2& fft, cf* spec,
                                               const cf (&tw_reg)[31], const LaneMap<1024>& lm,
                                               After&& after = After{}, float* en = nullptr) {
  window_apply(v, wc.a0, wc.ac, wc.as);
  if (en) *en = group32_sum(frame_energy(v));
  fft.stage1_reg_st(v, spec, tw_reg);
  fft.transpose_read(v, spec);
  fft.stage2_emit(v, [&](auto k, cf x) {
    spec[lm.out0 + 32 * k] = x;
    after(k);
  });
}

__device__ __forceinline__ bool ibm_uncertain(cf zr, cf zrp, float dl) {
  const float d = fmaf(zr.x, zrp.x, -(zr.y * zrp.y));
  const float m = fmaxf(fmaxf(fabsf(zr.x), fabsf(zr.y)), fmaxf(fmaxf(fabsf(zrp.x), fabsf(zrp.y)), dl));
  return !(fabsf(d) >= 3.9f * dl * m);
}
__device__ __forceinline__ bool ibm_level_out(float en, uint32_t lo, uint32_t span) {
  return __float_as_uint(en) - lo > span;
}
template <class After = NoAfter>
__device__ __forceinline__ uint32_t window_fft_reg_ibm_bits(cf (&v)[32], const WinCoef<1024>& wc,
                                                        const Fft1024x2& fft, cf* spec,
                                                        const cf (&tw_reg)[31],
                                                        const LaneMap<1024>& lm, float eg0,
                                                        float eg1, float cert, float& dl,
                                                        After&& after = After{}) {
  constexpr int N = 1024;
  window_apply(v, wc.a0, wc.ac, wc.as);
  const int l = lm.out0;
  fft.stage1_reg_st(v, spec, tw_reg);
  fft.transpose_read(v, spec);
  fft.stage2_emit(v, [&](auto k, cf x) {
    if constexpr (decltype(k)::value >= 16) {
      spec[l + 32 * k] = x;
      after(k);
    }
  });
  dl = cert * sqrtf(lm.grp ? eg1 : eg0);
  __builtin_amdgcn_wave_barrier();
  uint32_t w = 0u;
  float slack = __builtin_inff();
  const float dl39 = 3.9f * dl;
  static_for<0, 16>([&](auto kk) {
    constexpr int k = 15 - decltype(kk)::value;
    const int m = l + 32 * k;
    cf zp = spec[(N - m) & (N - 1)];
    if (k == 0 && l == 0) zp = v[0];
    w = (w << 1) | (ibm_noise(v[k], zp) ? 1u : 0u);
    const float d = fmaf(v[k].x, zp.x, -(v[k].y * zp.y));
    const float mm = fmaxf(fmaxf(fabsf(v[k].x), fabsf(v[k].y)),
                           fmaxf(fmaxf(fabsf(zp.x), fabsf(zp.y)), dl));
    slack = fminf(slack, fmaf(-dl39, mm, fabsf(d)));
  });
  const bool unc = slack < 0.0f;
  uint32_t um = 0u;
  if (__ballot(unc) != 0ull) {
    static_for<0, 16>([&](auto kk) {
      constexpr int k = 15 - decltype(kk)::value;
      const int m = l + 32 * k;
      cf zp = spec[(N - m) & (N - 1)];
      if (k == 0 && l == 0) zp = v[0];
      const float d = fmaf(v[k].x, zp.x, -(v[k].y * zp.y));
      const float mm = fmaxf(fmaxf(fabsf(v[k].x), fabsf(v[k].y)),
                             fmaxf(fmaxf(fabsf(zp.x), fabsf(zp.y)), dl));
      um = (um << 1) | (fmaf(-dl39, mm, fabsf(d)) < 0.0f ? 1u : 0u);
    });
    w &= ~um;
  }
  reinterpret_cast<uint32_t*>(spec)[l] = w;
  static_for<0, 16>([&](auto k) { after(k); });
  return um;
}

template <int N, bool IL512 = false, class After = NoAfter>
__device__ __forceinline__ void window_fft(cf (&v)[KCfg<N>::PPL], const WinCoef<N>& wc,
                                           const typename KCfg<N>::Fft& fft, cf* spec,
                                           const LaneMap<N>& lm, After&& after = After{},
                                           float* en = nullptr) {
  using C = KCfg<N>;
  float a0 = wc.a0, ac = wc.ac, as = wc.as;
  opaque(a0);
  opaque(ac);
  opaque(as);
  window_apply<N>(v, a0, ac, as);
  if (en) {
    float e = 0.0f;
    static_for<0, C::PPL>([&](auto r) {
      e = fmaf(v[r].x, v[r].x, e);
      e = fmaf(v[r].y, v[r].y, e);
    });
    *en = group32_sum(e);
  }
  if constexpr (N == 1024) {
    fft.stage1_ab_st(v, spec);
    fft.transpose_read(v, spec);
    fft.stage2_emit(v, [&](auto k, cf x) {
      spec[lm.out0 + C::OUT_STRIDE * k] = x;
      after(k);
    });
  } else if constexpr (IL512) {
    fft.forward_emit(v, spec, [&](auto k, cf x) {
      spec[lm.out0 + C::OUT_STRIDE * k] = x;
      after(k);
    });
  } else {
    fft.forward(v, spec);
    static_for<0, C::PPL>([&](auto k) { spec[lm.out0 + C::OUT_STRIDE * k] = v[k]; });
  }
}

template <bool NONNEG>
__device__ __forceinline__ void pair_loads(cf (&v)[32], rsrc_t r0, rsrc_t r1, int sp, int g) {
  static_for<0, 16>([&](auto j) {
    const int e = sp + 1024 * g + 32 * j;
    v[j].x = NONNEG ? bload_nn(r0, e) : bload(r0, e);
    v[j].y = NONNEG ? bload_nn(r1, e) : bload(r1, e);
  });
  static_for<0, 8>([&](auto i) {
    const int e = sp + 512 + 32 * (2 * i) + 32 * g;
    v[16 + 2 * i].x = NONNEG ? bload_nn(r0, e) : bload(r0, e);
    v[16 + 2 * i].y = NONNEG ? bload_nn(r1, e) : bload(r1, e);
  });
}
__device__ __forceinline__ void pair_finish(cf (&v)[32]) {
  static_for<0, 8>([&](auto i) {
    const auto rx = __builtin_amdgcn_permlane32_swap(__float_as_uint(v[16 + 2 * i].x),
                                                     __float_as_uint(v[16 + 2 * i].x), false, false);
    const auto ry = __builtin_amdgcn_permlane32_swap(__float_as_uint(v[16 + 2 * i].y),
                                                     __float_as_uint(v[16 + 2 * i].y), false, false);
    v[16 + 2 * i] = cf{__uint_as_float(rx[0]), __uint_as_float(ry[0])};
    v[17 + 2 * i] = cf{__uint_as_float(rx[1]), __uint_as_float(ry[1])};
  });
}

__device__ __forceinline__ void store_through(float* row, int n, int i, float4 v) {
  const v4i_t d = {__float_as_int(v.x), __float_as_int(v.y), __float_as_int(v.z),
                   __float_as_int(v.w)};
  __builtin_amdgcn_raw_buffer_store_b128(d, make_rsrc(row, n), 4 * i, 0, kSC1);
}

template <class CA>
__device__ __forceinline__ int utt_len(CA& A, int b) {
  if (!A.len) return A.max_len;
  const __attribute__((address_space(4))) int* lc =
      (const __attribute__((address_space(4))) int*)(A.len);
  return min(lc[b], A.max_len);
}

template <int MASK>
__device__ __forceinline__ float bin_mask(const ChainArgs& A, int b, cf x0, cf x1, cf zr,
                                          cf zrp, int k, int t, bool& noise, float& wgt) {
  if constexpr (MASK == MASK_IBM) {
    noise = ibm_noise(zr, zrp);
    wgt = noise ? 1.0f : 0.0f;
    return wgt;
  } else if constexpr (MASK == MASK_IPD) {
    wgt = ipd_weight(x0, x1);
    return wgt;
  } else if constexpr (MASK == MASK_ONES) {
    wgt = 1.0f;
    return 1.0f;
  } else {
    const float M =
        A.ext_mask[(long long)b * A.mask_sb + (long long)k * A.mask_sf + (long long)t * A.mask_st];
    const float m = 1.0f - M;
    wgt = m + A.weight_eps;
    return m;
  }
}

__device__ __forceinline__ float irm_gain(cf zr, cf zrp) {
  const float tr = zr.x + zrp.x, ti = zr.y - zrp.y;
  const float ir = zr.y + zrp.y, ii = zr.x - zrp.x;
  const float pt = tr * tr + ti * ti, pi = ir * ir + ii * ii;
  return sqrtf(pt / (pt + pi + 4e-10f));
}

using KArgs = const __attribute__((address_space(4))) ChainArgs;
__device__ __forceinline__ KArgs& kernarg_chain_args() {
  uintptr_t u = (uintptr_t)__builtin_amdgcn_kernarg_segment_ptr();
  asm volatile("" : "+s"(u));
  return *(KArgs*)u;
}
struct NoTw {};
using Tw1024 = cf[31];

template <int F, class CA>
__device__ __forceinline__ float* unit_item(CA& A, int u, int gx, int n_items, int n_whole, int P,
                                            int& b, int& c) {
  if (u < n_items) {
    b = u / gx;
    c = u % gx;
    return A.part + ((long long)b * A.nchunk + c) * 5 * F;
  }
  const int q = u - n_items, it = n_whole + q / P;
  b = it / gx;
  c = it % gx;
  return A.tpart + (long long)q * 5 * F;
}
}
```

real-time-audio-visual-zooming_amd/csrc/avz_chain_exact.hpp:

```cpp
#pragma once
#include "avz_chain_common.hpp"
#include "avz_ibm_exact.hpp"

namespace avz {
__device__ __forceinline__ int pick(uint32_t packed, int i) {
  return (int)(signed char)(packed >> (8 * i));
}
template <int N>
struct XLds {
  using C = KCfg<N>;
  using X = XGeo<N>;
  static constexpr int FR = 4;
  static constexpr int MP = N / 2 + 4;
  static constexpr int MIC_BYTES = FR / C::FPW * C::WAVE_BYTES;
  static constexpr int MAG_OFF = (4 * X::SCRATCH > MIC_BYTES) ? 4 * X::SCRATCH : MIC_BYTES;
  static constexpr int TWL_OFF = MAG_OFF + 2 * FR * MP * 4;
  static constexpr int WIN_OFF = TWL_OFF + (N / 2) * 16;
  static constexpr int SLOT_OFF = WIN_OFF + N * 4;
  static constexpr int SCAN_OFF = SLOT_OFF + FR * 32;
  static constexpr int SCAN_INTS = 256;
  static constexpr int WL = 32;
  static constexpr int WL_OFF = SCAN_OFF + 256 * 4;
  static constexpr int CTL_OFF = WL_OFF + WL * 16;
  static constexpr int END = CTL_OFF + 32;
  static_assert(C::FPW == 2 && END <= CGeo<N>::SLOT_LDS, "exact phase LDS");
};

struct XSlot {
  int unit, f, e, b, L, c, flags, pad;
};
__device__ __forceinline__ XSlot slot_u(const XSlot* sl, int g) {
  const XSlot v = sl[g];
  XSlot s;
  s.unit = __builtin_amdgcn_readfirstlane(v.unit);
  s.f = __builtin_amdgcn_readfirstlane(v.f);
  s.e = 0;
  s.b = __builtin_amdgcn_readfirstlane(v.b);
  s.L = __builtin_amdgcn_readfirstlane(v.L);
  s.c = __builtin_amdgcn_readfirstlane(v.c);
  s.flags = __builtin_amdgcn_readfirstlane(v.flags);
  s.pad = 0;
  return s;
}

template <int N, bool PER_BIN>
__device__ __forceinline__ void exact_round(KArgs& A, unsigned char* lds, const XSlot* sl, int ns,
                                            Acc32 (&pacc)[CGeo<N>::BPT + 1],
                                            uint32_t (&pbits)[CGeo<N>::BPT + 1]) {
  using C = KCfg<N>;
  using G = CGeo<N>;
  using X = XGeo<N>;
  using XL = XLds<N>;
  constexpr int NT = G::NT, H = G::H, F = G::F, BPT = G::BPT, PPL = C::PPL, MP = XL::MP;
  const int tid = threadIdx.x, lane = tid & 63;
  const int wave = __builtin_amdgcn_readfirstlane(tid >> 6);
  float* const mag = reinterpret_cast<float*>(lds + XL::MAG_OFF);
  const cd* const twl = reinterpret_cast<const cd*>(lds + XL::TWL_OFF);
  const float* const win = reinterpret_cast<const float*>(lds + XL::WIN_OFF);
  cd* const buf = reinterpret_cast<cd*>(lds + wave * X::SCRATCH);
  AVZ_STAMP_DECL();
  AVZ_STAMP_INIT();
  AVZ_XT_LAP_BEGIN(xr_prev);
  int lane_o = lane;
  opaque_i(lane_o);
  const int ga = wave >> 1, gb = (wave >> 1) + 2;
  const float* const refp = (wave & 1) ? A.ref_int : A.ref_tgt;
  float xa[N / 64], xb[N / 64];
  if (ga < ns) {
    const XSlot s = slot_u(sl, ga);
    ref_frame_load<N>(make_rsrc(refp + (long long)s.b * A.ref_stride, s.L),
                      (s.c * kChunk + s.f) * H - N / 2, lane_o, xa);
  }
  if (gb < ns) {
    const XSlot s = slot_u(sl, gb);
    ref_frame_load<N>(make_rsrc(refp + (long long)s.b * A.ref_stride, s.L),
                      (s.c * kChunk + s.f) * H - N / 2, lane_o, xb);
  }
  if (ga < ns) ref_spectrum_exact<N>(xa, twl, win, buf, mag + (2 * ga + (wave & 1)) * MP, lane_o);
  AVZ_STAMP(4);
  AVZ_XT_LAP(8, xr_prev);
  cf v[PPL];
  LaneMap<N> lm;
  lm.init(lane_o);
  const int gm = C::FPW * wave + lm.grp;
  if (wave < XL::FR / C::FPW) {
    const XSlot s = slot_u(sl, 0);
    const float* mixb = A.mix + (long long)s.b * A.mix_stride;
    const rsrc_t r_m0 = make_rsrc(mixb, s.L), r_m1 = make_rsrc(mixb + A.ch_stride, s.L);
    const bool on = gm < ns;
    const int fm = sl[on ? gm : 0].f;
    const int s0 = (s.c * kChunk + fm) * H - N / 2 + lm.in0;
#pragma unroll
    for (int r = 0; r < PPL; ++r) {
      v[r].x = on ? bload(r_m0, s0 + C::IN_STRIDE * r) : 0.0f;
      v[r].y = on ? bload(r_m1, s0 + C::IN_STRIDE * r) : 0.0f;
    }
  }
  if (gb < ns) {
    int lane_b = lane;
    opaque_i(lane_b);
    ref_spectrum_exact<N>(xb, twl, win, buf, mag + (2 * gb + (wave & 1)) * MP, lane_b);
  }
  AVZ_STAMP(5);
  lds_barrier();
  AVZ_STAMP(6);
  AVZ_XT_LAP(9, xr_prev);
  if (wave < XL::FR / C::FPW) {
    WinCoef<N> wc;
    wc.init(lm);
    cf* const spec = slot_ptr<N>(lds, gm);
    if constexpr (N == 1024) {
      Fft1024x2 f;
      f.l = lm.out0;
      window_apply(v, wc.a0, wc.ac, wc.as);
      f.forward(v, spec, reinterpret_cast<const cf*>(lds + G::TW_OFF));
      static_for<0, 32>([&](auto k) { spec[lm.out0 + 32 * k] = v[k]; });
    } else {
      Fft512x2 f;
      f.init(lane_o);
      window_fft<N>(v, wc, f, spec, lm);
    }
  }
  AVZ_STAMP(7);
  lds_barrier();
  AVZ_STAMP(8);
  AVZ_XT_LAP(10, xr_prev);
  unsigned long long n_exact = 0;
  for (int g = 0; g < ns; ++g) {
    const XSlot s = slot_u(sl, g);
    const cf* Zm = slot_ptr<N>(lds, g);
    auto put = [&](int j, int k, const Acc32& a, bool dfr, bool noise) {
      if (dfr) {
        pacc[j].c00 += a.c00;
        pacc[j].c11 += a.c11;
        pacc[j].c01r += a.c01r;
        pacc[j].c01i += a.c01i;
        pacc[j].cm += a.cm;
        pbits[j] |= (noise ? 1u : 0u) << s.f;
      }
    };
#pragma unroll
    for (int j = 0; j < BPT; ++j) {
      const int kb = tid + j * NT;
      const int kp = (N - kb) & (N - 1);
      const bool dfr =
          PER_BIN ? ((A.xdfr[(long long)s.unit * F + kb] >> s.f) & 1u)
                  : ((s.flags & 1) &&
                     ((A.xunc[((long long)s.unit * kChunk + s.f) * 32 + (kb & 31)] >> (kb >> 5)) & 1u));
      Acc32 a;
      a.zero();
      bool noise = false;
      if (dfr) {
        noise = mag[(2 * g + 1) * MP + kb] > mag[(2 * g) * MP + kb];
        cf x0, x1;
        split_pair2(Zm[kb], Zm[kp], x0, x1);
        a.add_sel(x0, x1, noise);
        a.cm = noise ? 1.0f : 0.0f;
        n_exact += 1;
      }
      put(j, kb, a, dfr, noise);
    }
    if (tid == NT - 1) {
      const bool dfr = (s.flags >> 1) & 1;
      Acc32 a;
      a.zero();
      bool noise = false;
      if (dfr) {
        noise = mag[(2 * g + 1) * MP + N / 2] > mag[(2 * g) * MP + N / 2];
        cf y0, y1;
        split_pair2(Zm[N / 2], Zm[N / 2], y0, y1);
        const float wn = noise ? 1.0f : 0.0f;
        a.add(y0, y1, wn, wn);
        n_exact += 1;
      }
      put(BPT, N / 2, a, dfr, noise);
    }
  }
  if (A.xstat && n_exact) atomicAdd(A.xstat + 1, n_exact);
  AVZ_STAMP(9);
  lds_barrier();
  AVZ_STAMP(10);
  AVZ_XT_LAP(11, xr_prev);
}

constexpr int kSparseMax = 12;

constexpr uint32_t kXOpen = 0x80000000u;
constexpr int kXRound = 2;
struct XPieces {
  uint32_t sp;
  int n_sp, nr, npr, n;
};
__device__ __forceinline__ XPieces x_pieces(uint32_t pend, uint32_t big) {
  XPieces q;
  q.sp = pend & ~big;
  q.n_sp = q.sp ? 1 : 0;
  q.nr = (__popc(big) + kXRound - 1) / kXRound;
  q.npr = min(q.nr, kXPieces - q.n_sp);
  q.n = q.n_sp + q.npr;
  return q;
}
__device__ __forceinline__ bool x_has_piece(uint32_t v) {
  return (v & kXOpen) && (v & 0xffffu) < ((v >> 16) & 0xffu);
}

template <int N>
__device__ __forceinline__ void exact_sparse(KArgs& A, unsigned char* lds, int b, int L, int c,
                                             const int* items, int n,
                                             Acc32 (&pacc)[CGeo<N>::BPT + 1],
                                             uint32_t (&pbits)[CGeo<N>::BPT + 1]) {
  using G = CGeo<N>;
  using XL = XLds<N>;
  constexpr int H = N / 2, NT = G::NT, BPT = G::BPT;
  const int tid = threadIdx.x, lane = tid & 63;
  const int wave = __builtin_amdgcn_readfirstlane(tid >> 6);
  const cd* const twl = reinterpret_cast<const cd*>(lds + XL::TWL_OFF);
  const float* const win = reinterpret_cast<const float*>(lds + XL::WIN_OFF);
  float* const res = reinterpret_cast<float*>(lds);
  const rsrc_t rt = make_rsrc(A.ref_tgt + (long long)b * A.ref_stride, L);
  const rsrc_t ri = make_rsrc(A.ref_int + (long long)b * A.ref_stride, L);
  const float* mixb = A.mix + (long long)b * A.mix_stride;
  const rsrc_t rm0 = make_rsrc(mixb, L), rm1 = make_rsrc(mixb + A.ch_stride, L);
  for (int it = wave; it < n; it += NT / 64) {
    const int item = __builtin_amdgcn_readfirstlane(items[it]);
    const int f = item >> 16, k = item & 0xffff;
    const int s0 = (c * kChunk + f) * H - N / 2;
    float st[N / 64], si[N / 64], sm0[N / 64], sm1[N / 64];
#pragma unroll
    for (int r = 0; r < N / 64; ++r) {
      const int m = lane + 64 * r;
      st[r] = bload(rt, s0 + m);
      si[r] = bload(ri, s0 + m);
      sm0[r] = bload(rm0, s0 + m);
      sm1[r] = bload(rm1, s0 + m);
    }
    double tr = 0.0, ti = 0.0, ir = 0.0, ii = 0.0, ac = 0.0, bs = 0.0, as = 0.0, bc = 0.0;
#pragma unroll
    for (int r = 0; r < N / 64; ++r) {
      const int m = lane + 64 * r;
      const double w = (double)win[m];
      const double xt = w * (double)st[r], xi = w * (double)si[r];
      const double a = w * (double)sm0[r], bb = w * (double)sm1[r];
      const cd tw = xtw_at<N>(twl, (k * m) & (N - 1));
      tr = fma(xt, tw.x, tr);
      ti = fma(xt, tw.y, ti);
      ir = fma(xi, tw.x, ir);
      ii = fma(xi, tw.y, ii);
      ac = fma(a, tw.x, ac);
      bs = fma(bb, tw.y, bs);
      as = fma(a, tw.y, as);
      bc = fma(bb, tw.x, bc);
    }
#pragma unroll
    for (int o = 32; o > 0; o >>= 1) {
      tr += __shfl_xor(tr, o, 64);
      ti += __shfl_xor(ti, o, 64);
      ir += __shfl_xor(ir, o, 64);
      ii += __shfl_xor(ii, o, 64);
      ac += __shfl_xor(ac, o, 64);
      bs += __shfl_xor(bs, o, 64);
      as += __shfl_xor(as, o, 64);
      bc += __shfl_xor(bc, o, 64);
    }
    if (lane == 0) {
      const bool noise = np_abs_c64((float)ir, (float)ii) > np_abs_c64((float)tr, (float)ti);
      constexpr double sc = 2.0 / N;
      const cf zk = {(float)(sc * (ac - bs)), (float)(sc * (as + bc))};
      const cf zp = {(float)(sc * (ac + bs)), (float)(sc * (bc - as))};
      Acc32 t;
      t.zero();
      cf x0, x1;
      split_pair2(zk, zp, x0, x1);
      if (k == N / 2) {
        const float wn = noise ? 1.0f : 0.0f;
        t.add(x0, x1, wn, wn);
      } else {
        t.add_sel(x0, x1, noise);
        t.cm = noise ? 1.0f : 0.0f;
      }
      float* q = res + 6 * it;
      q[0] = noise ? 1.0f : 0.0f;
      q[1] = t.c00;
      q[2] = t.c11;
      q[3] = t.c01r;
      q[4] = t.c01i;
      q[5] = t.cm;
    }
  }
  __syncthreads();
  for (int it = 0; it < n; ++it) {
    const int item = items[it];
    const int f = item >> 16, k = item & 0xffff;
    const int j = k == N / 2 ? BPT : k / NT;
    if (k == N / 2 ? tid == NT - 1 : (k % NT) == tid) {
      const float* q = res + 6 * it;
#pragma unroll
      for (int jj = 0; jj <= BPT; ++jj) {
        if (jj != j) continue;
        pacc[jj].c00 += q[1];
        pacc[jj].c11 += q[2];
        pacc[jj].c01r += q[3];
        pacc[jj].c01i += q[4];
        pacc[jj].cm += q[5];
        pbits[jj] |= (q[0] != 0.0f ? 1u : 0u) << f;
      }
    }
  }
  if (A.xstat && tid == 0) atomicAdd(A.xstat + 1, (unsigned long long)n);
  __syncthreads();
}

template <int N, bool PER_BIN, class CA>
__device__ __forceinline__ void exact_set_slot(CA& A, XSlot* sl, int g, int u, int f, int gx,
                                               int n_items, int n_whole, int P) {
  constexpr int F = N / 2 + 1;
  XSlot s;
  s.unit = u;
  s.f = f;
  s.e = -1;
  unit_item<F>(A, u, gx, n_items, n_whole, P, s.b, s.c);
  s.L = utt_len(A, s.b);
  const uint4 r = reinterpret_cast<const uint4*>(A.xpend)[u];
  s.flags = (PER_BIN ? 0 : (int)((r.y >> f) & 1u)) | (int)(((r.z >> f) & 1u) << 1);
  s.pad = 0;
  sl[g] = s;
}

template <int N, bool PER_BIN>
__device__ __forceinline__ void exact_unit(KArgs& A, unsigned char* lds, int u, int gx, int n_items,
                                           int n_whole, int P) {
  using G = CGeo<N>;
  using XL = XLds<N>;
  constexpr int F = N / 2 + 1, NT = G::NT, BPT = G::BPT, FR = XL::FR;
  const int tid = threadIdx.x;
  XSlot* const sl = reinterpret_cast<XSlot*>(lds + XL::SLOT_OFF);
  const uint4 rec = reinterpret_cast<const uint4*>(A.xpend)[u];
  const uint32_t pend = rec.x;
  if (pend == 0u || rec.w != 0u) return;
  int b, c;
  float* const Pt = unit_item<F>(A, u, gx, n_items, n_whole, P, b, c);
  if (A.xstat && tid == 0) atomicAdd(A.xstat, (unsigned long long)__popc(pend));
  Acc32 pacc[BPT + 1];
  uint32_t pbits[BPT + 1];
#pragma unroll
  for (int j = 0; j <= BPT; ++j) {
    const int kk = j < BPT ? tid + j * NT : N / 2;
    pbits[j] = 0u;
    if (j < BPT || tid == NT - 1) {
      pacc[j].c00 = Pt[0 * F + kk];
      pacc[j].c11 = Pt[1 * F + kk];
      pacc[j].c01r = Pt[2 * F + kk];
      pacc[j].c01i = Pt[3 * F + kk];
      pacc[j].cm = Pt[4 * F + kk];
    } else {
      pacc[j].zero();
    }
  }
  uint32_t rest = pend;
  if constexpr (!PER_BIN) {
    int* const items = reinterpret_cast<int*>(lds + XL::SCAN_OFF);
    int* const ctl = reinterpret_cast<int*>(lds + XL::CTL_OFF);
    uint32_t* const wsm = reinterpret_cast<uint32_t*>(lds + 16384);
    const uint32_t has_words = reinterpret_cast<const uint4*>(A.xpend)[u].y;
#pragma unroll
    for (int i = 0; i < kChunk / (G::NT / 32); ++i) {
      const int f = (tid >> 5) + (G::NT / 32) * i;
      if ((pend >> f) & 1u)
        wsm[f * 32 + (tid & 31)] =
            ((has_words >> f) & 1u) ? A.xunc[((long long)u * kChunk + f) * 32 + (tid & 31)] : 0u;
    }
    __syncthreads();
    if (tid < 64) {
      const uint32_t nyq = reinterpret_cast<const uint4*>(A.xpend)[u].z;
      int base = 0;
      uint32_t sparse = 0u;
      for (uint32_t todo = pend; todo != 0u; todo &= todo - 1u) {
        const int f = __builtin_ctz(todo);
        const uint32_t w = tid < 32 ? wsm[f * 32 + tid] : 0u;
        int inc = __popc(w);
#pragma unroll
        for (int o = 1; o < 32; o <<= 1) {
          const int y = __shfl_up(inc, o, 64);
          if ((tid & 63) >= o) inc += y;
        }
        const int tot = __shfl(inc, 31, 64), ny = (nyq >> f) & 1u;
        if (tot + ny <= kSparseMax && base + tot + ny <= XL::SCAN_INTS) {
          int at = base + inc - __popc(w);
          for (uint32_t x = w; x != 0u; x &= x - 1u) items[at++] = (f << 16) | (tid + 32 * __builtin_ctz(x));
          if (ny && tid == 0) items[base + tot] = (f << 16) | (N / 2);
          base += tot + ny;
          sparse |= 1u << f;
        }
      }
      if (tid == 0) {
        ctl[0] = base;
        ctl[1] = (int)sparse;
      }
    }
    __syncthreads();
    const int n_sp = ctl[0];
    rest &= ~(uint32_t)ctl[1];
    if (n_sp > 0) exact_sparse<N>(A, lds, b, utt_len(A, b), c, items, n_sp, pacc, pbits);
  }
  while (rest != 0u) {
    if (tid < FR) {
      uint32_t x = rest;
      for (int i = 0; i < tid && x; ++i) x &= x - 1u;
      if (x) exact_set_slot<N, PER_BIN>(A, sl, tid, u, __builtin_ctz(x), gx, n_items, n_whole, P);
    }
    const int ns = min(FR, __popc(rest));
    for (int i = 0; i < ns; ++i) rest &= rest - 1u;
    __syncthreads();
    exact_round<N, PER_BIN>(A, lds, sl, ns, pacc, pbits);
  }
  uint32_t* const MW = A.mwords + ((long long)b * A.nchunk + c) * F;
#pragma unroll
  for (int j = 0; j <= BPT; ++j) {
    const int kk = j < BPT ? tid + j * NT : N / 2;
    if (j < BPT || tid == NT - 1) {
      Pt[0 * F + kk] = pacc[j].c00;
      Pt[1 * F + kk] = pacc[j].c11;
      Pt[2 * F + kk] = pacc[j].c01r;
      Pt[3 * F + kk] = pacc[j].c01i;
      Pt[4 * F + kk] = pacc[j].cm;
      if (pbits[j]) atomicOr(MW + kk, pbits[j]);
    }
  }
}

template <int N>
__device__ __forceinline__ void exact_sparse_frames(KArgs& A, unsigned char* lds, int u, int b,
                                                    int c, uint32_t frames,
                                                    Acc32 (&pacc)[CGeo<N>::BPT + 1],
                                                    uint32_t (&pbits)[CGeo<N>::BPT + 1]) {
  using G = CGeo<N>;
  using XL = XLds<N>;
  const int tid = threadIdx.x;
  int* const items = reinterpret_cast<int*>(lds + XL::SCAN_OFF);
  int* const ctl = reinterpret_cast<int*>(lds + XL::CTL_OFF);
  uint32_t* const wsm = reinterpret_cast<uint32_t*>(lds + 16384);
  const uint4 rec = reinterpret_cast<const uint4*>(A.xpend)[u];
#pragma unroll
  for (int i = 0; i < kChunk / (G::NT / 32); ++i) {
    const int f = (tid >> 5) + (G::NT / 32) * i;
    if ((frames >> f) & 1u)
      wsm[f * 32 + (tid & 31)] =
          ((rec.y >> f) & 1u) ? A.xunc[((long long)u * kChunk + f) * 32 + (tid & 31)] : 0u;
  }
  __syncthreads();
  uint32_t todo = frames;
  while (todo != 0u) {
    if (tid < 64) {
      int base = 0;
      uint32_t took = 0u;
      for (uint32_t t = todo; t != 0u; t &= t - 1u) {
        const int f = __builtin_ctz(t);
        const uint32_t w = tid < 32 ? wsm[f * 32 + tid] : 0u;
        int inc = __popc(w);
#pragma unroll
        for (int o = 1; o < 32; o <<= 1) {
          const int y = __shfl_up(inc, o, 64);
          if ((tid & 63) >= o) inc += y;
        }
        const int tot = __shfl(inc, 31, 64), ny = (rec.z >> f) & 1u;
        if (base + tot + ny > XL::SCAN_INTS) break;
        int at = base + inc - __popc(w);
        for (uint32_t x = w; x != 0u; x &= x - 1u) items[at++] = (f << 16) | (tid + 32 * __builtin_ctz(x));
        if (ny && tid == 0) items[base + tot] = (f << 16) | (N / 2);
        base += tot + ny;
        took |= 1u << f;
      }
      if (tid == 0) {
        ctl[0] = base;
        ctl[1] = (int)took;
      }
    }
    __syncthreads();
    const int n = ctl[0];
    todo &= ~(uint32_t)ctl[1];
    exact_sparse<N>(A, lds, b, utt_len(A, b), c, items, n, pacc, pbits);
  }
}

template <int N, bool PER_BIN>
__device__ __forceinline__ void exact_piece(KArgs& A, unsigned char* lds, int u, int p, int gx,
                                            int n_items, int n_whole, int P) {
  using G = CGeo<N>;
  using XL = XLds<N>;
  constexpr int F = N / 2 + 1, NT = G::NT, BPT = G::BPT, FR = XL::FR;
  const int tid = threadIdx.x;
  XSlot* const sl = reinterpret_cast<XSlot*>(lds + XL::SLOT_OFF);
  int* const ctl = reinterpret_cast<int*>(lds + XL::CTL_OFF);
  const uint4 rec = reinterpret_cast<const uint4*>(A.xpend)[u];
  const XPieces q = x_pieces(rec.x, rec.w);
  int b, c;
  float* const Pt = unit_item<F>(A, u, gx, n_items, n_whole, P, b, c);
  Acc32 pacc[BPT + 1];
  uint32_t pbits[BPT + 1];
#pragma unroll
  for (int j = 0; j <= BPT; ++j) {
    pacc[j].zero();
    pbits[j] = 0u;
  }
  if (p < q.n_sp) {
    if (A.xstat && tid == 0) atomicAdd(A.xstat, (unsigned long long)__popc(q.sp));
    if constexpr (!PER_BIN) exact_sparse_frames<N>(A, lds, u, b, c, q.sp, pacc, pbits);
  } else {
    constexpr int R = kXRound;
    static_assert(R <= FR, "round frames");
    const int g = p - q.n_sp, r0 = g * q.nr / q.npr, r1 = (g + 1) * q.nr / q.npr;
    if (A.xstat && tid == 0)
      atomicAdd(A.xstat, (unsigned long long)(min(R * r1, __popc(rec.w)) - R * r0));
    const int L = utt_len(A, b);
    uint32_t rest = rec.w;
    for (int i = 0; i < r0 * R; ++i) rest &= rest - 1u;
    for (int r = r0; r < r1; ++r) {
      if (tid < R) {
        uint32_t x = rest;
        for (int i = 0; i < tid && x; ++i) x &= x - 1u;
        if (x) {
          const int f = __builtin_ctz(x);
          XSlot s;
          s.unit = u;
          s.f = f;
          s.e = -1;
          s.b = b;
          s.L = L;
          s.c = c;
          s.flags = (PER_BIN ? 0 : (int)((rec.y >> f) & 1u)) | (int)(((rec.z >> f) & 1u) << 1);
          s.pad = 0;
          sl[tid] = s;
        }
      }
      const int ns = min(R, __popc(rest));
      for (int i = 0; i < ns; ++i) rest &= rest - 1u;
      __syncthreads();
      exact_round<N, PER_BIN>(A, lds, sl, ns, pacc, pbits);
    }
  }
  uint32_t* const MW = A.mwords + ((long long)b * A.nchunk + c) * F;
  float* const R = A.xres + ((long long)u * kXPieces + p) * 5 * F;
#pragma unroll
  for (int j = 0; j <= BPT; ++j) {
    const int kk = j < BPT ? tid + j * NT : N / 2;
    if (j < BPT || tid == NT - 1) {
      if (pbits[j]) atomicOr(MW + kk, pbits[j]);
      if (q.n == 1) {
        Pt[0 * F + kk] = Pt[0 * F + kk] + pacc[j].c00;
        Pt[1 * F + kk] = Pt[1 * F + kk] + pacc[j].c11;
        Pt[2 * F + kk] = Pt[2 * F + kk] + pacc[j].c01r;
        Pt[3 * F + kk] = Pt[3 * F + kk] + pacc[j].c01i;
        Pt[4 * F + kk] = Pt[4 * F + kk] + pacc[j].cm;
      } else {
        R[0 * F + kk] = pacc[j].c00;
        R[1 * F + kk] = pacc[j].c11;
        R[2 * F + kk] = pacc[j].c01r;
        R[3 * F + kk] = pacc[j].c01i;
        R[4 * F + kk] = pacc[j].cm;
      }
    }
  }
#ifdef AVZ_XTRACE
  const unsigned long long tf = __builtin_amdgcn_s_memrealtime();
#endif
  __syncthreads();
  if (tid == 0) {
    bool last = true;
    if (q.n > 1) {
      __builtin_amdgcn_fence(__ATOMIC_RELEASE, "agent");
      const uint32_t arrived =
          __hip_atomic_fetch_add(A.xst + 2 * u + 1, 1u, __ATOMIC_RELAXED, __HIP_MEMORY_SCOPE_AGENT) + 1u;
      last = arrived == (uint32_t)q.n;
      if (last) __builtin_amdgcn_fence(__ATOMIC_ACQUIRE, "agent");
    }
    ctl[4] = last ? 1 : 0;
  }
  __syncthreads();
#ifdef AVZ_XTRACE
  const unsigned long long tm = __builtin_amdgcn_s_memrealtime();
  if (tid == 0 && g_stamps) g_stamps[blockIdx.x * 16 + 6] += tm - tf;
#endif
  if (ctl[4]) {
    if (q.n > 1) {
      const float* const R0 = A.xres + (long long)u * kXPieces * 5 * F;
      constexpr int M = (5 * F + NT - 1) / NT;
      float v[M];
#pragma unroll
      for (int m = 0; m < M; ++m) v[m] = tid + m * NT < 5 * F ? Pt[tid + m * NT] : 0.0f;
      for (int pp = 0; pp < q.n; ++pp) {
        float t[M];
#pragma unroll
        for (int m = 0; m < M; ++m)
          t[m] = tid + m * NT < 5 * F ? R0[(long long)pp * 5 * F + tid + m * NT] : 0.0f;
#pragma unroll
        for (int m = 0; m < M; ++m) v[m] += t[m];
      }
#pragma unroll
      for (int m = 0; m < M; ++m)
        if (tid + m * NT < 5 * F) Pt[tid + m * NT] = v[m];
    }
    if (tid == 0) {
      __hip_atomic_store(A.xst + 2 * u + 1, 0u, __ATOMIC_RELAXED, __HIP_MEMORY_SCOPE_AGENT);
      __hip_atomic_store(A.xst + 2 * u, 0u, __ATOMIC_RELAXED, __HIP_MEMORY_SCOPE_AGENT);
      __hip_atomic_fetch_and(A.xhint + (u >> 5), ~(1u << (u & 31)), __ATOMIC_RELAXED,
                             __HIP_MEMORY_SCOPE_AGENT);
    }
  }
  __syncthreads();
#ifdef AVZ_XTRACE
  if (tid == 0 && g_stamps) g_stamps[blockIdx.x * 16 + 7] += __builtin_amdgcn_s_memrealtime() - tm;
#endif
}

__device__ __forceinline__ int exact_claim(KArgs& A, int n_units, int* cand) {
  const int lane = threadIdx.x & 63;
  const int nw = (n_units + 31) >> 5;
  const int w_start = (int)(((long long)blockIdx.x * nw) / gridDim.x);
  for (;;) {
    int count = 0;
    for (int w0 = 0; w0 < nw && count < 64; w0 += 64) {
      const int wi = w0 + lane;
      int wid = w_start + wi;
      if (wid >= nw) wid -= nw;
      const uint32_t bits =
          wi < nw ? __hip_atomic_load(A.xhint + wid, __ATOMIC_RELAXED, __HIP_MEMORY_SCOPE_AGENT) : 0u;
      const int cnt = __popc(bits);
      int pre = cnt;
#pragma unroll
      for (int o = 1; o < 64; o <<= 1) {
        const int y = __shfl_up(pre, o, 64);
        if (lane >= o) pre += y;
      }
      const int tot = __shfl(pre, 63, 64);
      int pos = count + pre - cnt;
      for (uint32_t x = bits; x != 0u && pos < 64; x &= x - 1u) cand[pos++] = wid * 32 + __builtin_ctz(x);
      count += tot;
    }
    count = min(count, 64);
    if (count == 0) return -1;
    __builtin_amdgcn_fence(__ATOMIC_RELEASE, "wavefront");
    __builtin_amdgcn_wave_barrier();
    __builtin_amdgcn_fence(__ATOMIC_ACQUIRE, "wavefront");
    const int uid = lane < count ? cand[lane] : -1;
    const uint32_t v =
        uid >= 0 ? __hip_atomic_load(A.xst + 2 * uid, __ATOMIC_RELAXED, __HIP_MEMORY_SCOPE_AGENT) : 0u;
    const unsigned long long m = __ballot(x_has_piece(v));
    if (m == 0ull) return -1;
    int k = (int)(blockIdx.x % (unsigned)__popcll(m));
    unsigned long long mm = m;
    for (; k > 0; --k) mm &= mm - 1ull;
    const int src = __builtin_ctzll(mm);
    int res = -1;
    if (lane == src) {
      const uint32_t old =
          __hip_atomic_fetch_add(A.xst + 2 * uid, 1u, __ATOMIC_RELAXED, __HIP_MEMORY_SCOPE_AGENT);
      if (x_has_piece(old)) {
        __builtin_amdgcn_fence(__ATOMIC_ACQUIRE, "agent");
        res = (uid << 8) | (int)(old & 0xffu);
      }
    }
    res = __shfl(res, src, 64);
    if (res >= 0) return res;
    __builtin_amdgcn_wave_barrier();
  }
}

template <int N, int MASK, bool IRM, bool SPLIT, class TW>
__device__ __forceinline__ void ibm_exact_units(unsigned char* lds, int gx, int n_items) {
  KArgs& A = kernarg_chain_args();
  using G = CGeo<N>;
  using XL = XLds<N>;
  constexpr bool SHARE = N == 1024 && !std::is_same<TW, NoTw>::value;
  constexpr bool PER_BIN = !(N == 1024 && !IRM && SHARE);
  AVZ_XT(1, __builtin_amdgcn_s_memrealtime());
  if (A.ibm_cert <= 0.0f) return;
  const int tid = threadIdx.x;
  const int P = SPLIT && A.a_pieces > 1 ? A.a_pieces : 1;
  const int n_whole = P > 1 ? A.a_whole : n_items;
  __syncthreads();
  const uint32_t mine = *reinterpret_cast<const uint32_t*>(lds + G::MISC_OFF + 56);
  auto tables = [&]() {
    int t = threadIdx.x;
    opaque_i(t);
    xtab_fill<N>(A.xtw, A.xwin, reinterpret_cast<cd*>(lds + XL::TWL_OFF),
                 reinterpret_cast<float*>(lds + XL::WIN_OFF), t, G::NT);
    __syncthreads();
  };
  bool have_tables = false;
  int seq = 0;
  auto one = [&](int u) {
    const int k = seq++;
    if (!((mine >> min(k, 31)) & 1u)) return;
    const uint4 rec = reinterpret_cast<const uint4*>(A.xpend)[u];
    if (rec.x == 0u || rec.w != 0u) return;
    if (k >= 31) {
      int b, c;
      unit_item<G::F>(A, u, gx, n_items, n_whole, P, b, c);
      const int L = utt_len(A, b);
      if (L < N || c >= ((L + G::H - 1) / G::H + 1 + kChunk - 1) / kChunk) return;
    }
    if (!have_tables) {
      tables();
      have_tables = true;
    }
    exact_unit<N, PER_BIN>(A, lds, u, gx, n_items, n_whole, P);
  };
  const int n_end = n_whole + (n_items - n_whole) * P;
  for (int u = blockIdx.x; u < n_end; u += gridDim.x) one(u < n_whole ? u : n_items + u - n_whole);
  AVZ_XT(2, __builtin_amdgcn_s_memrealtime());
  {
    const int n_units = n_items + (n_end - n_whole);
    int* const ctl = reinterpret_cast<int*>(lds + XLds<N>::CTL_OFF);
    for (;;) {
      AVZ_XT_BEGIN(tc);
      if (tid < 64) {
        const int got = exact_claim(A, n_units, reinterpret_cast<int*>(lds + XLds<N>::SCAN_OFF));
        if (tid == 0) ctl[2] = got;
      }
      AVZ_XT_END(14, tc);
      __syncthreads();
      const int got = ctl[2];
      __syncthreads();
      if (got < 0) break;
      if (!have_tables) {
        AVZ_XT_BEGIN(tt);
        tables();
        have_tables = true;
        AVZ_XT_END(15, tt);
      }
      AVZ_XT_BEGIN(t0x);
      exact_piece<N, PER_BIN>(A, lds, got >> 8, got & 0xff, gx, n_items, n_whole, P);
#ifdef AVZ_XTRACE
      if (tid == 0 && g_stamps) {
        unsigned long long* st = g_stamps + blockIdx.x * 16;
        st[4] += 1;
        st[5] += __builtin_amdgcn_s_memrealtime() - t0x;
      }
#endif
    }
  }
  AVZ_XT(3, __builtin_amdgcn_s_memrealtime());
}
}
```

real-time-audio-visual-zooming_amd/csrc/avz_internal.h:

```cpp
#pragma once
#include <stdint.h>
#include <string.h>

namespace avz {

enum : int { MASK_IBM = 0, MASK_IPD = 1, MASK_EXTERNAL = 2, MASK_ONES = 3 };
enum : int { PF_NONE = 0, PF_IBM_TARGET = 1, PF_EXT_FLOOR = 2, PF_EXT_MUL = 3, PF_IRM = 4 };
enum : int { NORM_NONE = 0, NORM_PEAK = 1 };

enum : int { BF_MVDR = 0, BF_HYBRID_NULL = 1 };

struct PieceState {
  uint32_t cnt, fin;
  unsigned long long st;
};
static_assert(sizeof(PieceState) == 16, "one 16-B store resets it");

constexpr int kXPieces = 8;

inline void ibm_level_range(double c, uint32_t* lo_bits, uint32_t* span) {
  auto bits = [](double x) {
    const float f = (float)x;
    uint32_t u;
    memcpy(&u, &f, 4);
    return u;
  };
  auto value = [](uint32_t u) {
    float f;
    memcpy(&f, &u, 4);
    return (double)f;
  };
  double lo = 0x1p-100, hi = 0x1p100;
  if (c > 0.0) {
    if (0x1p-114 / (c * c) > lo) lo = 0x1p-114 / (c * c);
    const double m = c > 64.0 ? c : 64.0;
    if (0x1p124 / (c * m) < hi) hi = 0x1p124 / (c * m);
  }
  if (!(lo <= hi) || !(lo >= 0x1p-126) || !(hi <= 0x1p127)) lo = hi = 1.0;
  uint32_t a = bits(lo), b = bits(hi);
  if (value(a) < lo) ++a;
  if (value(b) > hi) --b;
  if (a > b) a = b = bits(1.0);
  *lo_bits = a;
  *span = b - a;
}

struct ChainArgs {
  int batch;
  const int* len;
  int max_len;
  const float* mix;
  long long mix_stride;
  long long ch_stride;
  const float* ref_tgt;
  const float* ref_int;
  long long ref_stride;
  const float* ext_mask;
  long long mask_sb, mask_sf, mask_st;
  float* out;
  long long out_stride;
  float* peak;
  double* cov_out;
  float* w_out;
  double fs, sigma, tau1, tau2, fmin_hz;
  double mic_d, c_sound;
  float weight_eps, pf_floor, norm_eps;
  int postfilter, normalize;
  int beamformer;
  double bypass_hz, cond_max;
  int max_frames;
  int nchunk;
  float* part;
  uint32_t* mwords;
  const double* steer;
  float* coef;
  float* heads;
  float* tails;
  uint32_t* peak_u;
  float* pf_gain;
  int singular_fallback;
  const float* spec;
  long long spec_sb, spec_sf;
  int spec_frames;
  int cov_only;
  int* flag;
  int a_whole, a_pieces;
  float* tpart;
  int tpart_slots;
  int s_whole, s_pieces, s_steps;
  float* pheads;
  float* ptails;
  int pseam_slots;
  int b_lo;
  int s_ipf;
  PieceState* pstate;
  int dbg_ipf;
  float ibm_cert;
  uint32_t ibm_en_lo, ibm_en_span;
  const float* xwin;
  const double* xtw;
  unsigned long long* xstat;
  uint32_t* xpend;
  uint32_t* xdfr;
  uint32_t* xunc;
  uint32_t* xst;
  float* xres;
  uint32_t* xhint;
  long long xst_reset;
  int synth_variant;
  void* const* events;
  int n_events;
};

struct SpecArgs {
  int batch, frames;
  const float* Y;
  long long y_sb, y_sm, y_sf;
  const float* M;
  long long m_sb, m_sf;
  const double* steer;
  float* S;
  long long s_sb, s_sf;
  double* cov_out;
  float* w_out;
  const double* cov_in;
  int* flag;
};

struct WpeArgs {
  int batch, bins, frames;
  const int* frames_b;
  int taps, delay, iterations;
  const float* Y;
  long long y_sb, y_sm, y_sf;
  float* Z;
  long long z_sb, z_sm, z_sf;
  int* status;
};

struct StoiArgs {
  int batch, max_len;
  const int* len;
  int resample;
  int n10_max, nf_max;
  const float* clean;
  const float* est;
  long long clean_stride, est_stride;
  float* res;
  long long res_stride;
  const float* x10;
  const float* y10;
  long long x10_stride, y10_stride;
  double* energy;
  int* kept;
  int* info;
  double* tob;
  long long tob_stride;
  double* stoi;
};

struct StftArgs {
  int batch, channels;
  const int* len;
  int max_len;
  const float* x;
  long long x_stride, ch_stride;
  float* Y;
  long long y_stride_b, y_stride_c, y_stride_f;
  int max_frames;
  int feat;
  float* F_out;
  long long f_sb, f_sc, f_sf, f_st;
};
enum : int { FEAT_NONE = 0, FEAT_LOGMAG_IPD = 1, FEAT_TFLITE = 2 };

struct TrainArgs {
  StftArgs s;
  const float* tgt;
  const float* itf;
  long long ref_stride;
  float* label;
  long long l_sb, l_sf, l_st;
};

struct StreamArgs {
  int streams, hops;
  double forget;
  const int* active;
  const int* adapt;
  const float* mix;
  long long mix_stride, ch_stride;
  const float* ref_tgt;
  const float* ref_int;
  long long ref_stride;
  const float* ext_mask;
  long long mask_sb, mask_sf, mask_st;
  float* out;
  long long out_stride;
  float* w_out;
  double* cov_out;
  float* mask_out;
  unsigned char* state;
  long long state_stride;
  const int* select;
  const double* angle_deg;
};

struct StreamLayout {
  long long prev_off = 0, tail_off = 0, cov_off = 0, steer_off = 0, stride = 0;
  constexpr explicit StreamLayout(int n_fft) {
    const long long H = n_fft / 2, F = H + 1;
    prev_off = 64;
    tail_off = prev_off + 4 * H * 4;
    cov_off = tail_off + H * 4;
    steer_off = cov_off + F * 5 * 8;
    stride = (steer_off + F * 4 * 8 + 255) & ~255LL;
  }
};

struct WpeStreamArgs {
  int streams, hops, taps, delay;
  double forget, inv_forget, power_floor, q_init;
  const int* active;
  const int* adapt;
  const float* mix;
  long long mix_stride, ch_stride;
  float* out;
  long long out_stride, out_ch_stride;
  float* Y_out;
  float* Z_out;
  double* G_out;
  unsigned char* state;
  long long state_stride;
  const int* select;
  int j0, nf;
};

constexpr int kWpeStreamRound = 8;

struct WpeStreamLayout {
  long long prev_off = 0, tail_off = 0, ring_off = 0, zr_off = 0, g_off = 0, q_off = 0, stride = 0;
  int n = 0, W = 0, R = 0, tri = 0;
  constexpr WpeStreamLayout(int n_fft, int taps, int delay) {
    const long long H = n_fft / 2, F = H + 1;
    auto up = [](long long v) { return (v + 255) & ~255LL; };
    n = 2 * taps;
    W = taps + delay + 1;
    R = W + kWpeStreamRound;
    tri = n * (n + 1) / 2;
    prev_off = 256;
    tail_off = up(prev_off + 2 * H * 4);
    ring_off = up(tail_off + 2 * H * 4);
    zr_off = up(ring_off + F * R * 16);
    g_off = up(zr_off + kWpeStreamRound * F * 16);
    q_off = up(g_off + F * n * 32);
    stride = up(q_off + F * tri * 16);
  }
};

struct SrpArgs {
// ... 114 lines not shown
```

Baseline: 79.64 billion TF-bins/s.

## Speculate IBM polarity for dense uncertain frames and verify exactly in parallel

For frames with many uncertain IBM bins, the analysis pass now guesses the mask polarity from the summed sign of the difference, applies it immediately, and records the frame as speculative instead of pending. The exact path gains verify pieces that recheck speculative bins and a fix-up pass that subtracts wrong contributions and re-adds corrected ones, plus flips the stored mask words. The aim is to take dense uncertain frames off the critical exact-recompute path and spread verification over more pieces. Exact-path twiddle and window tables are also prefetched into registers before the claim. This adds complexity, extra workspace, and a sign-cancellation fix-up path whose correctness is delicate.

```diff
diff --git a/include/avz.h b/include/avz.h
--- a/include/avz.h
+++ b/include/avz.h
@@ -132,6 +132,8 @@
 int avz_plan_set_timing_period(avz_plan* plan, int period);
 int avz_plan_get_timing(avz_plan* plan, double* ms_avg , int* calls);
 int avz_plan_set_ibm_stats(avz_plan* plan, unsigned long long* counts);
+int avz_plan_set_ibm_speculation(avz_plan* plan, unsigned long long* counts, int invert_polarity,
+                                 double bound_factor);
 int avz_plan_set_diagnostics(avz_plan* plan, int synth_variant, int ipf_mode);
 int avz_ibm_window(int n, float* out);
 
diff --git a/real-time-audio-visual-zooming_amd/avz/_lib.py b/real-time-audio-visual-zooming_amd/avz/_lib.py
--- a/real-time-audio-visual-zooming_amd/avz/_lib.py
+++ b/real-time-audio-visual-zooming_amd/avz/_lib.py
@@ -32,7 +32,7 @@
     "avz_mvdr_covariance", "avz_solve_covariance", "avz_apply_istft", "avz_beamform_spectral",
     "avz_istft", "avz_scene_generate_workspace_bytes", "avz_scene_generate",
     "avz_projection_metrics_scaled", "avz_plan_set_ibm_stats", "avz_plan_set_diagnostics",
-    "avz_ibm_window", "avz_wpe_spectral",
+    "avz_ibm_window", "avz_wpe_spectral", "avz_plan_set_ibm_speculation",
     "avz_room_rir_len", "avz_room_rir", "avz_scene_reverb_workspace_bytes",
     "avz_scene_reverb_mix", "avz_scene_reverb_generate_workspace_bytes",
     "avz_scene_reverb_generate",
@@ -226,6 +226,8 @@
     lib.avz_plan_get_timing.argtypes = [P, ct.POINTER(ct.c_double), ct.POINTER(I)]
     lib.avz_plan_set_ibm_stats.argtypes = [P, P]
     lib.avz_plan_set_diagnostics.argtypes = [P, I, I]
+    lib.avz_plan_set_ibm_speculation.argtypes = [P, P, I, ct.c_double]
+    lib.avz_plan_set_ibm_speculation.restype = ct.c_int
     lib.avz_ibm_window.argtypes = [I, ct.POINTER(ct.c_float)]
     lib.avz_chunk_split.argtypes = [I, I, I, P, P, P, P, LL, LL, P, LL, LL, P]
     lib.avz_chunk_merge.argtypes = [I, I, I, I, P, P, P, LL, P, LL, P, I, ct.c_double, P]
diff --git a/real-time-audio-visual-zooming_amd/avz/engine.py b/real-time-audio-visual-zooming_amd/avz/engine.py
--- a/real-time-audio-visual-zooming_amd/avz/engine.py
+++ b/real-time-audio-visual-zooming_amd/avz/engine.py
@@ -107,6 +107,15 @@
             assert counts.dtype == torch.int64 and counts.is_cuda and counts.numel() >= 2
         check(lib.avz_plan_set_ibm_stats(self._h, _ptr(counts)), "avz_plan_set_ibm_stats")
         self._ibm_stats = counts
+
+    def set_ibm_speculation(self, counts=None, invert_polarity: bool = False,
+                            bound_factor: float = 1.0) -> None:
+        if counts is not None:
+            assert counts.dtype == torch.int64 and counts.is_cuda and counts.numel() >= 4
+        check(lib.avz_plan_set_ibm_speculation(self._h, _ptr(counts), int(bool(invert_polarity)),
+                                               float(bound_factor)),
+              "avz_plan_set_ibm_speculation")
+        self._ibm_spec_stats = counts
 
     def set_diagnostics(self, synth_variant: int = 2, ipf_mode: int = 0) -> None:
         check(lib.avz_plan_set_diagnostics(self._h, int(synth_variant), int(ipf_mode)),
diff --git a/real-time-audio-visual-zooming_amd/csrc/avz_capi.cpp b/real-time-audio-visual-zooming_amd/csrc/avz_capi.cpp
--- a/real-time-audio-visual-zooming_amd/csrc/avz_capi.cpp
+++ b/real-time-audio-visual-zooming_amd/csrc/avz_capi.cpp
@@ -39,6 +39,7 @@
   size_t xst_bytes;
   long long xst_units;
   float* xres;
+  uint32_t* xspec;
 };
 
 static int tail_slots(long long B, int nchunk) { return (int)std::min<long long>(B * nchunk * 8, 768); }
@@ -67,6 +68,7 @@
   const size_t sz_xu = align256(sizeof(uint32_t) * 32 * 32 * (size_t)units);
   const size_t sz_xs = align256(sizeof(uint32_t) * (2 * (size_t)units + (size_t)(units + 31) / 32));
   const size_t sz_xr = align256(sizeof(float) * avz::kXPieces * 5 * (size_t)F * units);
+  const size_t sz_xc = align256(sizeof(uint32_t) * 4 * units);
 
   if (base && w) {
     char* q = base;
@@ -92,9 +94,10 @@
     w->xst_bytes = sz_xs;
     w->xst_units = units;
     w->xres = units ? reinterpret_cast<float*>(q) : nullptr; q += sz_xr;
+    w->xspec = units ? reinterpret_cast<uint32_t*>(q) : nullptr; q += sz_xc;
   }
   return sz_part + sz_mw + sz_coef + 2 * sz_ht + 6 * sz_b + sz_gain + sz_tpart + 2 * sz_seam +
-         sz_xp + sz_xd + sz_xu + sz_xs + sz_xr;
+         sz_xp + sz_xd + sz_xu + sz_xs + sz_xr + sz_xc;
 }
 
 struct avz_plan {
@@ -109,6 +112,9 @@
   float ibm_cert;
   uint32_t ibm_en_lo, ibm_en_span;
   unsigned long long* xstat;
+  unsigned long long* xspstat;
+  int ibm_spec_flip;
+  double ibm_bq_scale;
   int synth_variant;
   int dbg_ipf;
   Workspace ws;
@@ -258,6 +264,9 @@
     avz::ibm_level_range(refbits ? (double)p->ibm_cert * 2.0 / c.n_fft : (double)p->ibm_cert,
                          &p->ibm_en_lo, &p->ibm_en_span);
     p->xstat = nullptr;
+    p->xspstat = nullptr;
+    p->ibm_spec_flip = 0;
+    p->ibm_bq_scale = 1.0;
     p->synth_variant = 2;
     p->dbg_ipf = 0;
     std::vector<double> xt((size_t)N * 2);
@@ -354,6 +363,9 @@
   k.xwin = p->xwin;
   k.xtw = p->xtw;
   k.xstat = p->xstat;
+  k.xspstat = p->xspstat;
+  k.ibm_spec_flip = p->ibm_spec_flip;
+  k.ibm_bq_scale = p->ibm_bq_scale;
   k.synth_variant = p->synth_variant;
   k.dbg_ipf = p->dbg_ipf;
 }
@@ -435,6 +447,7 @@
   k.xunc = ws.xunc;
   k.xst = ws.xst;
   k.xres = ws.xres;
+  k.xspec = ws.xspec;
   k.xhint = ws.xst ? ws.xst + 2 * (ws.xst_units) : nullptr;
   if (use == USE_COVARIANCE) {
     k.out = nullptr;
@@ -757,6 +770,18 @@
   if (!p) return AVZ_ERR_ARG;
   if (misaligned(counts, 8)) return AVZ_ERR_ALIGN;
   p->xstat = counts;
+  return AVZ_OK;
+}
+
+extern "C" int avz_plan_set_ibm_speculation(avz_plan* p, unsigned long long* counts,
+                                            int invert_polarity, double bound_factor) {
+  if (!p || invert_polarity < 0 || invert_polarity > 1 || !(bound_factor > 0.0) ||
+      !std::isfinite(bound_factor))
+    return AVZ_ERR_ARG;
+  if (misaligned(counts, 8)) return AVZ_ERR_ALIGN;
+  p->xspstat = counts;
+  p->ibm_spec_flip = invert_polarity;
+  p->ibm_bq_scale = bound_factor;
   return AVZ_OK;
 }
 
diff --git a/real-time-audio-visual-zooming_amd/csrc/avz_chain_analysis.hpp b/real-time-audio-visual-zooming_amd/csrc/avz_chain_analysis.hpp
--- a/real-time-audio-visual-zooming_amd/csrc/avz_chain_analysis.hpp
+++ b/real-time-audio-visual-zooming_amd/csrc/avz_chain_analysis.hpp
@@ -33,12 +33,17 @@
   const int s_lo = p * SA / P;
   const int nstep = min((nframes + FB - 1) / FB, (p + 1) * SA / P);
   uint32_t* const pendw = reinterpret_cast<uint32_t*>(lds + G::MISC_OFF + 32 + 12 * (seq & 1));
+  uint32_t* const specw = reinterpret_cast<uint32_t*>(lds + G::MISC_OFF + 8 * (seq & 1));
   if (MASK == MASK_IBM && tid == 0) {
     int z = 0;
     opaque_i(z);
     pendw[0] = (uint32_t)z;
     pendw[1] = (uint32_t)z;
     pendw[2] = (uint32_t)z;
+    if constexpr (REFBITS) {
+      specw[0] = (uint32_t)z;
+      specw[1] = (uint32_t)z;
+    }
   }
 
   const typename C::Fft fft = K.fft;
@@ -210,14 +215,20 @@
             KArgs& Ak = kernarg_chain_args();
             const int gxi = (Ak.max_frames + kChunk - 1) / kChunk;
             const int unit = slot < 0 ? b * gxi + c : gxi * Ak.batch + slot;
-            Ak.xunc[((long long)unit * kChunk + step * FB + my_frame) * 32 + (lane & 31)] = um;
-            int nu = __popc(um);
+            Ak.xunc[((long long)unit * kChunk + step * FB + my_frame) * 32 + (lane & 31)] =
+                um & 0xffffu;
+            int nu = __popc(um & 0xffffu);
 #pragma unroll
             for (int o = 1; o < 32; o <<= 1) nu += __shfl_xor(nu, o, 64);
             if ((lane & 31) == 0) {
-              atomicOr(pendw, 1u << (step * FB + my_frame));
-              atomicOr(pendw + 1, 1u << (step * FB + my_frame));
-              if (nu >= kSparseMax) atomicOr(pendw + 2, 1u << (step * FB + my_frame));
+              if (um & 0x10000u) {
+                atomicOr(specw, 1u << (step * FB + my_frame));
+                if (um & 0x20000u) atomicOr(specw + 1, 1u << (step * FB + my_frame));
+              } else {
+                atomicOr(pendw, 1u << (step * FB + my_frame));
+                atomicOr(pendw + 1, 1u << (step * FB + my_frame));
+                if (nu >= kSparseMax) atomicOr(pendw + 2, 1u << (step * FB + my_frame));
+              }
             }
           }
         }
@@ -401,10 +412,15 @@
         if (MASK == MASK_IPD && ((ident_w >> (8 * lane)) & 1ull)) wn = mn = 0.01f;
         if (MASK == MASK_IBM &&
             ibm_uncertain(zr, zr, reinterpret_cast<const float*>(lds + G::MISC_OFF + 16)[lane])) {
-          noise = false;
-          wn = mn = 0.0f;
           nunc = true;
-          atomicOr(pendw, 1u << (step * FB + lane));
+          if (REFBITS && ((specw[0] >> (step * FB + lane)) & 1u)) {
+            noise = (specw[1] >> (step * FB + lane)) & 1u;
+            wn = mn = noise ? 1.0f : 0.0f;
+          } else {
+            noise = false;
+            wn = mn = 0.0f;
+            atomicOr(pendw, 1u << (step * FB + lane));
+          }
         }
         an.add(y0, y1, wn, mn);
         if constexpr (MASK == MASK_IPD) {
@@ -428,13 +444,16 @@
 
   if constexpr (MASK == MASK_IBM) {
     const uint32_t pend = pendw[0], full = pendw[1];
+    const uint32_t spec = REFBITS ? specw[0] : 0u;
     const uint32_t big = REFBITS ? pendw[2] : pend;
     KArgs& Ak = kernarg_chain_args();
     const int gxi = (Ak.max_frames + kChunk - 1) / kChunk;
     const int unit = slot < 0 ? b * gxi + c : gxi * Ak.batch + slot;
     if (nyq_wave && lane == 0) {
       reinterpret_cast<uint4*>(Ak.xpend)[unit] = make_uint4(pend, full, nyq_dfr, big);
-      if (pend) *reinterpret_cast<uint32_t*>(lds + G::MISC_OFF + 56) |= 1u << min(seq, 31);
+      if constexpr (REFBITS)
+        reinterpret_cast<uint4*>(Ak.xspec)[unit] = make_uint4(spec, specw[1], 0u, 0u);
+      if (pend | spec) *reinterpret_cast<uint32_t*>(lds + G::MISC_OFF + 56) |= 1u << min(seq, 31);
     }
     if (DLT && pend != 0u) {
 #pragma unroll
@@ -502,14 +521,15 @@
 
   if constexpr (MASK == MASK_IBM) {
     const uint32_t big = REFBITS ? pendw[2] : pendw[0];
-    if (big != 0u) {
+    const uint32_t spec = REFBITS ? specw[0] : 0u;
+    if (x_published(big, spec)) {
       AVZ_XT_BEGIN(tp);
       __syncthreads();
       if (tid == 0) {
         KArgs& Ak = kernarg_chain_args();
         const int gxi = (Ak.max_frames + kChunk - 1) / kChunk;
         const int unit = slot < 0 ? b * gxi + c : gxi * Ak.batch + slot;
-        const XPieces q = x_pieces(pendw[0], big);
+        const XPieces q = x_pieces(pendw[0], big, spec);
         Ak.xst[2 * unit + 1] = 0u;
         __builtin_amdgcn_fence(__ATOMIC_RELEASE, "agent");
         __hip_atomic_store(Ak.xst + 2 * unit, kXOpen | ((uint32_t)q.n << 16), __ATOMIC_RELAXED,
diff --git a/real-time-audio-visual-zooming_amd/csrc/avz_chain_common.hpp b/real-time-audio-visual-zooming_amd/csrc/avz_chain_common.hpp
--- a/real-time-audio-visual-zooming_amd/csrc/avz_chain_common.hpp
+++ b/real-time-audio-visual-zooming_amd/csrc/avz_chain_common.hpp
@@ -15,6 +15,7 @@
 constexpr int kSC1 = 16;
 typedef int v4i_t __attribute__((ext_vector_type(4)));
 constexpr int kCThreads = 256;
+constexpr int kSparseMax = 12;
 
 template <int N>
 struct CGeo {
@@ -130,6 +131,12 @@
     e = fmaf(v[r].y, v[r].y, e);
   });
   return e;
+}
+using KArgs = const __attribute__((address_space(4))) ChainArgs;
+__device__ __forceinline__ KArgs& kernarg_chain_args() {
+  uintptr_t u = (uintptr_t)__builtin_amdgcn_kernarg_segment_ptr();
+  asm volatile("" : "+s"(u));
+  return *(KArgs*)u;
 }
 struct NoAfter {
   template <class K>
@@ -195,6 +202,7 @@
   const bool unc = slack < 0.0f;
   uint32_t um = 0u;
   if (__ballot(unc) != 0ull) {
+    float ds = 0.0f;
     static_for<0, 16>([&](auto kk) {
       constexpr int k = 15 - decltype(kk)::value;
       const int m = l + 32 * k;
@@ -204,8 +212,18 @@
       const float mm = fmaxf(fmaxf(fabsf(v[k].x), fabsf(v[k].y)),
                              fmaxf(fmaxf(fabsf(zp.x), fabsf(zp.y)), dl));
       um = (um << 1) | (fmaf(-dl39, mm, fabsf(d)) < 0.0f ? 1u : 0u);
+      ds += d;
     });
     w &= ~um;
+    int nu = __popc(um);
+#pragma unroll
+    for (int o = 1; o < 32; o <<= 1) nu += __shfl_xor(nu, o, 64);
+    const float dg = group32_sum(ds);
+    if (nu >= kSparseMax && dl < __builtin_inff()) {
+      const uint32_t pol = (dg < 0.0f ? 1u : 0u) ^ (uint32_t)kernarg_chain_args().ibm_spec_flip;
+      w |= pol ? um : 0u;
+      um |= 0x10000u | (pol << 17);
+    }
   }
   reinterpret_cast<uint32_t*>(spec)[l] = w;
   static_for<0, 16>([&](auto k) { after(k); });
@@ -316,12 +334,6 @@
   return sqrtf(pt / (pt + pi + 4e-10f));
 }
 
-using KArgs = const __attribute__((address_space(4))) ChainArgs;
-__device__ __forceinline__ KArgs& kernarg_chain_args() {
-  uintptr_t u = (uintptr_t)__builtin_amdgcn_kernarg_segment_ptr();
-  asm volatile("" : "+s"(u));
-  return *(KArgs*)u;
-}
 struct NoTw {};
 using Tw1024 = cf[31];
 
diff --git a/real-time-audio-visual-zooming_amd/csrc/avz_chain_exact.hpp b/real-time-audio-visual-zooming_amd/csrc/avz_chain_exact.hpp
--- a/real-time-audio-visual-zooming_amd/csrc/avz_chain_exact.hpp
+++ b/real-time-audio-visual-zooming_amd/csrc/avz_chain_exact.hpp
@@ -43,7 +43,7 @@
   return s;
 }
 
-template <int N, bool PER_BIN>
+template <int N, bool PER_BIN, bool FIX = false>
 __device__ __forceinline__ void exact_round(KArgs& A, unsigned char* lds, const XSlot* sl, int ns,
                                             Acc32 (&pacc)[CGeo<N>::BPT + 1],
                                             uint32_t (&pbits)[CGeo<N>::BPT + 1]) {
@@ -154,9 +154,24 @@
         noise = mag[(2 * g + 1) * MP + kb] > mag[(2 * g) * MP + kb];
         cf x0, x1;
         split_pair2(Zm[kb], Zm[kp], x0, x1);
-        a.add_sel(x0, x1, noise);
-        a.cm = noise ? 1.0f : 0.0f;
-        n_exact += 1;
+        if constexpr (FIX) {
+          const bool flip = noise != (bool)((s.flags >> 2) & 1);
+          a.add_sel(x0, x1, flip);
+          a.cm = flip ? 1.0f : 0.0f;
+          if (!noise) {
+            a.c00 = -a.c00;
+            a.c11 = -a.c11;
+            a.c01r = -a.c01r;
+            a.c01i = -a.c01i;
+            a.cm = -a.cm;
+          }
+          n_exact += flip ? 1 : 0;
+          noise = flip;
+        } else {
+          a.add_sel(x0, x1, noise);
+          a.cm = noise ? 1.0f : 0.0f;
+          n_exact += 1;
+        }
       }
       put(j, kb, a, dfr, noise);
     }
@@ -169,36 +184,54 @@
         noise = mag[(2 * g + 1) * MP + N / 2] > mag[(2 * g) * MP + N / 2];
         cf y0, y1;
         split_pair2(Zm[N / 2], Zm[N / 2], y0, y1);
-        const float wn = noise ? 1.0f : 0.0f;
-        a.add(y0, y1, wn, wn);
-        n_exact += 1;
+        if constexpr (FIX) {
+          const bool flip = noise != (bool)((s.flags >> 2) & 1);
+          const float wn = flip ? (noise ? 1.0f : -1.0f) : 0.0f;
+          a.add(y0, y1, wn, wn);
+          n_exact += flip ? 1 : 0;
+          noise = flip;
+        } else {
+          const float wn = noise ? 1.0f : 0.0f;
+          a.add(y0, y1, wn, wn);
+          n_exact += 1;
+        }
       }
       put(BPT, N / 2, a, dfr, noise);
     }
   }
-  if (A.xstat && n_exact) atomicAdd(A.xstat + 1, n_exact);
+  if constexpr (FIX) {
+    if (A.xspstat && n_exact) atomicAdd(A.xspstat + 3, n_exact);
+  } else {
+    if (A.xstat && n_exact) atomicAdd(A.xstat + 1, n_exact);
+  }
   AVZ_STAMP(9);
   lds_barrier();
   AVZ_STAMP(10);
   AVZ_XT_LAP(11, xr_prev);
 }
 
-constexpr int kSparseMax = 12;
 
 constexpr uint32_t kXOpen = 0x80000000u;
 constexpr int kXRound = 2;
+constexpr int kXVerify = 4;
 struct XPieces {
   uint32_t sp;
   int n_sp, nr, npr, n;
+  int nv, nvp;
 };
-__device__ __forceinline__ XPieces x_pieces(uint32_t pend, uint32_t big) {
+__device__ __forceinline__ XPieces x_pieces(uint32_t pend, uint32_t big, uint32_t spec) {
   XPieces q;
   q.sp = pend & ~big;
   q.n_sp = q.sp ? 1 : 0;
   q.nr = (__popc(big) + kXRound - 1) / kXRound;
-  q.npr = min(q.nr, kXPieces - q.n_sp);
-  q.n = q.n_sp + q.npr;
+  q.nv = __popc(spec);
+  q.nvp = min((q.nv + kXVerify - 1) / kXVerify, kXPieces - q.n_sp - (q.nr ? 1 : 0));
+  q.npr = min(q.nr, kXPieces - q.n_sp - q.nvp);
+  q.n = q.n_sp + q.npr + q.nvp;
   return q;
+}
+__device__ __forceinline__ bool x_published(uint32_t big, uint32_t spec) {
+  return (big | spec) != 0u;
 }
 __device__ __forceinline__ bool x_has_piece(uint32_t v) {
   return (v & kXOpen) && (v & 0xffffu) < ((v >> 16) & 0xffu);
@@ -332,7 +365,8 @@
   using G = CGeo<N>;
   using XL = XLds<N>;
   constexpr int F = N / 2 + 1, NT = G::NT, BPT = G::BPT, FR = XL::FR;
-  const int tid = threadIdx.x;
+  int tid = threadIdx.x;
+  opaque_i(tid);
   XSlot* const sl = reinterpret_cast<XSlot*>(lds + XL::SLOT_OFF);
   const uint4 rec = reinterpret_cast<const uint4*>(A.xpend)[u];
   const uint32_t pend = rec.x;
@@ -435,7 +469,8 @@
                                                     uint32_t (&pbits)[CGeo<N>::BPT + 1]) {
   using G = CGeo<N>;
   using XL = XLds<N>;
-  const int tid = threadIdx.x;
+  int tid = threadIdx.x;
+  opaque_i(tid);
   int* const items = reinterpret_cast<int*>(lds + XL::SCAN_OFF);
   int* const ctl = reinterpret_cast<int*>(lds + XL::CTL_OFF);
   uint32_t* const wsm = reinterpret_cast<uint32_t*>(lds + 16384);
@@ -482,17 +517,190 @@
   }
 }
 
+template <int N>
+__device__ __forceinline__ uint32_t exact_verify(KArgs& A, unsigned char* lds, int u, int b, int c,
+                                                 uint32_t spec, uint32_t pol, uint32_t nyq) {
+  using G = CGeo<N>;
+  using X = XGeo<N>;
+  using XL = XLds<N>;
+  constexpr int NT = G::NT, FR = XL::FR, H = G::H, MP = XL::MP;
+  static_assert(NT / 64 == FR, "a frame per wave");
+  const int tid = threadIdx.x;
+  const int wave = __builtin_amdgcn_readfirstlane(tid >> 6);
+  int lane = tid & 63;
+  opaque_i(lane);
+  const cd* const twl = reinterpret_cast<const cd*>(lds + XL::TWL_OFF);
+  const float* const win = reinterpret_cast<const float*>(lds + XL::WIN_OFF);
+  float* const mag = reinterpret_cast<float*>(lds + XL::MAG_OFF) + wave * MP;
+  cd* const buf = reinterpret_cast<cd*>(lds + wave * X::SCRATCH);
+  int* const ctl = reinterpret_cast<int*>(lds + XL::CTL_OFF);
+  const int L = utt_len(A, b);
+  if (tid == 0) ctl[5] = 0;
+  __syncthreads();
+  const rsrc_t rt = make_rsrc(A.ref_tgt + (long long)b * A.ref_stride, L);
+  const rsrc_t ri = make_rsrc(A.ref_int + (long long)b * A.ref_stride, L);
+  const double bq = A.ibm_bq_scale;
+  uint32_t fixw = 0u;
+  unsigned long long n_ver = 0, n_fall = 0, n_fr = 0;
+  const int lane_o = lane;
+  uint32_t mine = spec;
+  for (int i = 0; i < wave && mine; ++i) mine &= mine - 1u;
+  float xa[N / 64], xb[N / 64];
+  uint32_t uw = 0u;
+  auto loads = [&](int f) {
+    const int s0 = (c * kChunk + f) * H - N / 2;
+    ref_frame_load<N>(rt, s0, lane_o, xa);
+    ref_frame_load<N>(ri, s0, lane_o, xb);
+    uw = A.xunc[((long long)u * kChunk + f) * 32 + (lane & 31)];
+  };
+  if (mine) loads(__builtin_ctz(mine));
+  while (mine != 0u) {
+    const int f = __builtin_ctz(mine);
+    for (int i = 0; i < FR && mine; ++i) mine &= mine - 1u;
+    double st = 0.0, si = 0.0;
+#pragma unroll
+    for (int r = 0; r < X::RX; ++r) {
+      const float2 w = reinterpret_cast<const float2*>(win)[lane_o + 64 * r];
+      st += fabs((double)w.x * (double)xa[2 * r]) + fabs((double)w.y * (double)xa[2 * r + 1]);
+      si += fabs((double)w.x * (double)xb[2 * r]) + fabs((double)w.y * (double)xb[2 * r + 1]);
+    }
+#pragma unroll
+    for (int o = 32; o > 0; o >>= 1) {
+      st += __shfl_xor(st, o, 64);
+      si += __shfl_xor(si, o, 64);
+    }
+    st = __shfl(st, 0, 64);
+    si = __shfl(si, 0, 64);
+    const bool tq = st <= si;
+    float xl[N / 64];
+#pragma unroll
+    for (int i = 0; i < N / 64; ++i) xl[i] = tq ? xb[i] : xa[i];
+    const uint32_t uwf = uw;
+    if (mine) loads(__builtin_ctz(mine));
+    ref_spectrum_exact<N>(xl, twl, win, buf, mag, lane_o);
+    const double thr = (tq ? st : si) * bq * (1.0 + 0x1p-18) + 0x1p-139;
+    int nv = 0, nf = 0;
+#pragma unroll
+    for (int q = 0; q < X::RX; ++q) {
+      const int k = lane + 64 * q;
+      if ((uwf >> (k >> 5)) & 1u) {
+        const bool ok = (double)mag[k] > thr;
+        nv += ok ? 1 : 0;
+        nf += ok ? 0 : 1;
+      }
+    }
+    if (lane == 0 && ((nyq >> f) & 1u)) {
+      const bool ok = (double)mag[N / 2] > thr;
+      nv += ok ? 1 : 0;
+      nf += ok ? 0 : 1;
+    }
+#pragma unroll
+    for (int o = 32; o > 0; o >>= 1) {
+      nv += __shfl_xor(nv, o, 64);
+      nf += __shfl_xor(nf, o, 64);
+    }
+    if (nf != 0 || (tq ? 1u : 0u) != ((pol >> f) & 1u)) fixw |= 1u << f;
+    n_ver += nv;
+    n_fall += nf;
+    n_fr += 1;
+  }
+  if (lane == 0) {
+    if (fixw) atomicOr(reinterpret_cast<uint32_t*>(ctl + 5), fixw);
+    if (A.xstat && n_fr) {
+      atomicAdd(A.xstat, n_fr);
+      atomicAdd(A.xstat + 1, n_ver + n_fall);
+    }
+    if (A.xspstat && n_fr) {
+      atomicAdd(A.xspstat, n_fr);
+      atomicAdd(A.xspstat + 1, n_ver);
+      atomicAdd(A.xspstat + 2, n_fall);
+    }
+  }
+  __syncthreads();
+  const uint32_t fix = (uint32_t)ctl[5];
+  __syncthreads();
+  return fix;
+}
+
+template <int N>
+__device__ __forceinline__ void exact_fix(KArgs& A, unsigned char* lds, int u, float* Pt, int b,
+                                          int c, uint32_t fix, uint32_t pol, uint32_t nyq) {
+  using G = CGeo<N>;
+  using XL = XLds<N>;
+  constexpr int F = N / 2 + 1, NT = G::NT, BPT = G::BPT, FR = XL::FR;
+  int tid = threadIdx.x;
+  opaque_i(tid);
+  XSlot* const sl = reinterpret_cast<XSlot*>(lds + XL::SLOT_OFF);
+  const int L = utt_len(A, b);
+  Acc32 pacc[BPT + 1];
+  uint32_t pflip[BPT + 1];
+#pragma unroll
+  for (int j = 0; j <= BPT; ++j) {
+    const int kk = j < BPT ? tid + j * NT : N / 2;
+    pflip[j] = 0u;
+    if (j < BPT || tid == NT - 1) {
+      pacc[j].c00 = Pt[0 * F + kk];
+      pacc[j].c11 = Pt[1 * F + kk];
+      pacc[j].c01r = Pt[2 * F + kk];
+      pacc[j].c01i = Pt[3 * F + kk];
+      pacc[j].cm = Pt[4 * F + kk];
+    } else {
+      pacc[j].zero();
+    }
+  }
+  while (fix != 0u) {
+    if (tid < FR) {
+      uint32_t x = fix;
+      for (int i = 0; i < tid && x; ++i) x &= x - 1u;
+      if (x) {
+        const int f = __builtin_ctz(x);
+        XSlot s;
+        s.unit = u;
+        s.f = f;
+        s.e = -1;
+        s.b = b;
+        s.L = L;
+        s.c = c;
+        s.flags = 1 | (int)(((nyq >> f) & 1u) << 1) | (int)(((pol >> f) & 1u) << 2);
+        s.pad = 0;
+        sl[tid] = s;
+      }
+    }
+    const int ns = min(FR, __popc(fix));
+    for (int i = 0; i < ns; ++i) fix &= fix - 1u;
+    __syncthreads();
+    exact_round<N, false, true>(A, lds, sl, ns, pacc, pflip);
+  }
+  uint32_t* const MW = A.mwords + ((long long)b * A.nchunk + c) * F;
+#pragma unroll
+  for (int j = 0; j <= BPT; ++j) {
+    const int kk = j < BPT ? tid + j * NT : N / 2;
+    if (j < BPT || tid == NT - 1) {
+      Pt[0 * F + kk] = pacc[j].c00;
+      Pt[1 * F + kk] = pacc[j].c11;
+      Pt[2 * F + kk] = pacc[j].c01r;
+      Pt[3 * F + kk] = pacc[j].c01i;
+      Pt[4 * F + kk] = pacc[j].cm;
+      if (pflip[j]) atomicXor(MW + kk, pflip[j]);
+    }
+  }
+}
+
 template <int N, bool PER_BIN>
 __device__ __forceinline__ void exact_piece(KArgs& A, unsigned char* lds, int u, int p, int gx,
                                             int n_items, int n_whole, int P) {
   using G = CGeo<N>;
   using XL = XLds<N>;
   constexpr int F = N / 2 + 1, NT = G::NT, BPT = G::BPT, FR = XL::FR;
-  const int tid = threadIdx.x;
+  int tid = threadIdx.x;
+  opaque_i(tid);
   XSlot* const sl = reinterpret_cast<XSlot*>(lds + XL::SLOT_OFF);
   int* const ctl = reinterpret_cast<int*>(lds + XL::CTL_OFF);
   const uint4 rec = reinterpret_cast<const uint4*>(A.xpend)[u];
-  const XPieces q = x_pieces(rec.x, rec.w);
+  uint4 sp = make_uint4(0u, 0u, 0u, 0u);
+  if constexpr (!PER_BIN) sp = reinterpret_cast<const uint4*>(A.xspec)[u];
+  const XPieces q = x_pieces(rec.x, rec.w, sp.x);
+  const bool vp = p >= q.n_sp + q.npr;
   int b, c;
   float* const Pt = unit_item<F>(A, u, gx, n_items, n_whole, P, b, c);
   Acc32 pacc[BPT + 1];
@@ -502,7 +710,18 @@
     pacc[j].zero();
     pbits[j] = 0u;
   }
-  if (p < q.n_sp) {
+  uint32_t vfix = 0u;
+  if (vp) {
+    if constexpr (!PER_BIN) {
+      const int g = p - q.n_sp - q.npr, f0 = g * q.nv / q.nvp, f1 = (g + 1) * q.nv / q.nvp;
+      uint32_t fr = sp.x, keep = 0u;
+      for (int i = 0; i < f1; ++i) {
+        if (i >= f0) keep |= fr & (0u - fr);
+        fr &= fr - 1u;
+      }
+      vfix = exact_verify<N>(A, lds, u, b, c, keep, sp.y, rec.z);
+    }
+  } else if (p < q.n_sp) {
     if (A.xstat && tid == 0) atomicAdd(A.xstat, (unsigned long long)__popc(q.sp));
     if constexpr (!PER_BIN) exact_sparse_frames<N>(A, lds, u, b, c, q.sp, pacc, pbits);
   } else {
@@ -543,7 +762,7 @@
 #pragma unroll
   for (int j = 0; j <= BPT; ++j) {
     const int kk = j < BPT ? tid + j * NT : N / 2;
-    if (j < BPT || tid == NT - 1) {
+    if ((j < BPT || tid == NT - 1) && !vp) {
       if (pbits[j]) atomicOr(MW + kk, pbits[j]);
       if (q.n == 1) {
         Pt[0 * F + kk] = Pt[0 * F + kk] + pacc[j].c00;
@@ -566,6 +785,10 @@
   __syncthreads();
   if (tid == 0) {
     bool last = true;
+    if constexpr (!PER_BIN) {
+      if (vfix)
+        __hip_atomic_fetch_or(A.xspec + 4 * u + 2, vfix, __ATOMIC_RELAXED, __HIP_MEMORY_SCOPE_AGENT);
+    }
     if (q.n > 1) {
       __builtin_amdgcn_fence(__ATOMIC_RELEASE, "agent");
       const uint32_t arrived =
@@ -574,6 +797,12 @@
       if (last) __builtin_amdgcn_fence(__ATOMIC_ACQUIRE, "agent");
     }
     ctl[4] = last ? 1 : 0;
+    if constexpr (!PER_BIN) {
+      if (last && q.nvp)
+        ctl[6] = (int)__hip_atomic_load(A.xspec + 4 * u + 2, __ATOMIC_RELAXED, __HIP_MEMORY_SCOPE_AGENT);
+      else
+        ctl[6] = 0;
+    }
   }
   __syncthreads();
 #ifdef AVZ_XTRACE
@@ -581,13 +810,14 @@
   if (tid == 0 && g_stamps) g_stamps[blockIdx.x * 16 + 6] += tm - tf;
 #endif
   if (ctl[4]) {
-    if (q.n > 1) {
+    const int n_sum = q.n_sp + q.npr;
+    if (q.n > 1 && n_sum > 0) {
       const float* const R0 = A.xres + (long long)u * kXPieces * 5 * F;
       constexpr int M = (5 * F + NT - 1) / NT;
       float v[M];
 #pragma unroll
       for (int m = 0; m < M; ++m) v[m] = tid + m * NT < 5 * F ? Pt[tid + m * NT] : 0.0f;
-      for (int pp = 0; pp < q.n; ++pp) {
+      for (int pp = 0; pp < n_sum; ++pp) {
         float t[M];
 #pragma unroll
         for (int m = 0; m < M; ++m)
@@ -598,6 +828,13 @@
 #pragma unroll
       for (int m = 0; m < M; ++m)
         if (tid + m * NT < 5 * F) Pt[tid + m * NT] = v[m];
+    }
+    if constexpr (!PER_BIN) {
+      const uint32_t fix = (uint32_t)ctl[6];
+      if (fix != 0u) {
+        __syncthreads();
+        exact_fix<N>(A, lds, u, Pt, b, c, fix, sp.y, rec.z);
+      }
     }
     if (tid == 0) {
       __hip_atomic_store(A.xst + 2 * u + 1, 0u, __ATOMIC_RELAXED, __HIP_MEMORY_SCOPE_AGENT);
@@ -692,7 +929,9 @@
     const int k = seq++;
     if (!((mine >> min(k, 31)) & 1u)) return;
     const uint4 rec = reinterpret_cast<const uint4*>(A.xpend)[u];
-    if (rec.x == 0u || rec.w != 0u) return;
+    uint32_t spec = 0u;
+    if constexpr (!PER_BIN) spec = A.xspec[4 * u];
+    if (rec.x == 0u || x_published(rec.w, spec)) return;
     if (k >= 31) {
       int b, c;
       unit_item<G::F>(A, u, gx, n_items, n_whole, P, b, c);
@@ -711,7 +950,19 @@
   {
     const int n_units = n_items + (n_end - n_whole);
     int* const ctl = reinterpret_cast<int*>(lds + XLds<N>::CTL_OFF);
+    constexpr int TWN = (N / 2) / G::NT, WNN = N / G::NT;
+    static_assert(TWN * G::NT == N / 2 && WNN * G::NT == N, "tables tile the block");
     for (;;) {
+      double2 tpre[TWN];
+      float wpre[WNN];
+      int tt_ = threadIdx.x;
+      opaque_i(tt_);
+      if (!have_tables) {
+#pragma unroll
+        for (int i = 0; i < TWN; ++i) tpre[i] = reinterpret_cast<const double2*>(A.xtw)[tt_ + i * G::NT];
+#pragma unroll
+        for (int i = 0; i < WNN; ++i) wpre[i] = A.xwin[tt_ + i * G::NT];
+      }
       AVZ_XT_BEGIN(tc);
       if (tid < 64) {
         const int got = exact_claim(A, n_units, reinterpret_cast<int*>(lds + XLds<N>::SCAN_OFF));
@@ -724,7 +975,13 @@
       if (got < 0) break;
       if (!have_tables) {
         AVZ_XT_BEGIN(tt);
-        tables();
+        cd* const twl = reinterpret_cast<cd*>(lds + XL::TWL_OFF);
+        float* const win = reinterpret_cast<float*>(lds + XL::WIN_OFF);
+#pragma unroll
+        for (int i = 0; i < TWN; ++i) twl[tt_ + i * G::NT] = {tpre[i].x, tpre[i].y};
+#pragma unroll
+        for (int i = 0; i < WNN; ++i) win[tt_ + i * G::NT] = wpre[i];
+        __syncthreads();
         have_tables = true;
         AVZ_XT_END(15, tt);
       }
diff --git a/real-time-audio-visual-zooming_amd/csrc/avz_internal.h b/real-time-audio-visual-zooming_amd/csrc/avz_internal.h
--- a/real-time-audio-visual-zooming_amd/csrc/avz_internal.h
+++ b/real-time-audio-visual-zooming_amd/csrc/avz_internal.h
@@ -106,6 +106,10 @@
   uint32_t* xst;
   float* xres;
   uint32_t* xhint;
+  uint32_t* xspec;
+  unsigned long long* xspstat;
+  int ibm_spec_flip;
+  double ibm_bq_scale;
   long long xst_reset;
   int synth_variant;
   void* const* events;
```

Result: no change. 79.92 billion TF-bins/s, median of 6 (+0.3%).
